# nv-tlabs/LION

Measured on AMD Instinct MI355X. Metric: shapes/sec @1000-step DDIM, Bx2048pts, higher is better.
Workload: dtype f32 (operands of the 3x3x3 voxel convolutions and of the long 1x1 convolutions cut into fp16 hi/lo pairs on the 16-bi...

## Files before the change

### include/lion_hip.h

```cpp
#ifndef LION_HIP_H_
#define LION_HIP_H_

#include <stddef.h>
#include <stdint.h>

#ifdef __cplusplus
extern "C" {
#endif

typedef void *lionStream_t;

#define LION_OK 0
#define LION_EINVAL (-1)
#define LION_EUNSUPPORTED (-2)
#define LION_EWORKSPACE (-3)

int lion_abi_version(void);

size_t lion_avg_voxelize_workspace_bytes(int B, int C, int N, int r);
int lion_avg_voxelize_forward(const float *feat, const int32_t *coords, int B, int C, int N,
                              int r, float *out, int32_t *ind, int32_t *cnt, void *ws,
                              size_t ws_bytes, lionStream_t stream);

int lion_voxelize_points_forward(const float *feat, const float *coords, int B, int C, int N,
                                 int r, int normalize, float eps, float *out,
                                 float *norm_coords, int32_t *ind, int32_t *cnt, void *ws,
                                 size_t ws_bytes, lionStream_t stream);

size_t lion_voxel_plan_bytes(int B, int N, int r);
int lion_voxel_index(const float *coords, int B, int N, int r, int normalize, float eps,
                     float *norm_coords, int32_t *ind, int32_t *cnt, void *plan, size_t plan_bytes,
                     lionStream_t stream);
int lion_voxel_scatter(const float *feat, const void *plan, size_t plan_bytes, int B, int C, int N,
                       int r, float *out, lionStream_t stream);
int lion_voxel_scatter_read(const float *feat, const void *plan, size_t plan_bytes, int B, int C, int N, int r,
                            const int32_t *occ_m1, float *out, lionStream_t stream);

int lion_avg_voxelize_backward(const float *gy, const int32_t *ind, const int32_t *cnt, int B,
                               int C, int N, int r3, float *gx, lionStream_t stream);

int lion_trilinear_devoxelize_forward(const float *coords, const float *feat, int B, int C,
                                      int N, int r, int training, float *out, int32_t *inds,
                                      float *wgts, lionStream_t stream);

int lion_trilinear_devoxelize_backward(const float *gy, const int32_t *inds, const float *wgts,
                                       int B, int C, int N, int r3, float *gx,
                                       lionStream_t stream);

int lion_ball_query(const float *centers, const float *points, int B, int M, int N,
                    float radius, int U, int32_t *idx, lionStream_t stream);

int lion_grouping_forward(const float *feat, const int32_t *idx, int B, int C, int N, int M,
                          int U, float *out, lionStream_t stream);
int lion_group_points_forward(const float *coords, const float *centers, const float *feat, const int32_t *idx,
                              int B, int C, int N, int M, int U, float *out, lionStream_t stream);
int lion_grouping_backward(const float *gy, const int32_t *idx, int B, int C, int N, int M,
                           int U, float *gx, lionStream_t stream);

int lion_furthest_point_sampling(const float *coords, int B, int N, int M, int32_t *idx,
                                 lionStream_t stream);

int lion_gather_features_forward(const float *feat, const int32_t *idx, int B, int C, int N,
                                 int M, float *out, lionStream_t stream);
int lion_gather_features_backward(const float *gy, const int32_t *idx, int B, int C, int N,
                                  int M, float *gx, lionStream_t stream);

int lion_three_nn_interpolate_forward(const float *points, const float *centers,
                                      const float *cfeat, int B, int C, int N, int M,
                                      float *out, int32_t *idx, float *wgt,
                                      lionStream_t stream);
int lion_three_nn_interpolate_cat_forward(const float *points, const float *centers, const float *cfeat, const float *temb,
                                          int ld_t, const float *skip, int B, int C1, int C2, int C3, int N, int M,
                                          float *out, int32_t *idx, float *wgt, lionStream_t stream);
int lion_three_nn_interpolate_backward(const float *gy, const int32_t *idx, const float *wgt,
                                       int B, int C, int N, int M, float *gx,
                                       lionStream_t stream);

int lion_chamfer_forward(const float *xyz1, const float *xyz2, int B, int N, int M,
                         float *dist1, float *dist2, int32_t *idx1, int32_t *idx2,
                         lionStream_t stream);
int lion_chamfer_backward(const float *xyz1, const float *xyz2, const float *gdist1,
                          const float *gdist2, const int32_t *idx1, const int32_t *idx2, int B,
                          int N, int M, float *gxyz1, float *gxyz2, lionStream_t stream);

size_t lion_emd_workspace_bytes(int B, int N, int M);
int lion_emd_approxmatch(const float *xyz1, const float *xyz2, int B, int N, int M,
                         float *match, void *ws, size_t ws_bytes, lionStream_t stream);
int lion_emd_cost(const float *xyz1, const float *xyz2, int B, int N, int M, float *cost, void *ws,
                  size_t ws_bytes, lionStream_t stream);
int lion_emd_matchcost(const float *xyz1, const float *xyz2, const float *match, int B, int N,
                       int M, float *cost, void *ws, size_t ws_bytes, lionStream_t stream);
int lion_emd_matchcost_backward(const float *grad_cost, const float *xyz1, const float *xyz2,
                                const float *match, int B, int N, int M, float *grad1,
                                float *grad2, lionStream_t stream);

int lion_ddim_update(const float *x, const float *eps, const float *z, size_t numel, float s,
                     float c, float sigma, float *out, lionStream_t stream);
int lion_ddpm_update(const float *x, const float *eps, const float *z, size_t numel,
                     int t_is_zero, float k_outer, float k_a, float k_b, float scale,
                     float temp, float *out, lionStream_t stream);
int lion_chain_begin_step(const float *table, int n_steps, int32_t *counter, float *t_out, int B, float *cur,
                          lionStream_t stream);
int lion_chain_update_noise(int mode, const float *x, const float *eps, size_t numel, const float *cur,
                            const uint32_t *seed , uint32_t stream_id, float *out,
                            float *z_out, lionStream_t stream);
int lion_chain_begin_step_temb(const float *table, int n_steps, int32_t *counter, float *t_out, int B, float *cur,
                               const float *temb_table, int temb_width, float *temb_out, lionStream_t stream);
int lion_chain_update_noise_cm(int mode, const float *x, const float *eps_cm, int B, int N, const float *cur,
                               const uint32_t *seed, uint32_t stream_id, float *out, float *z_out, lionStream_t stream);
int lion_latent_unpack(const float *x, int B, int N, int D, float *all, float *coords, float *rest, lionStream_t stream);
int lion_concat_broadcast(const float *a, const float *t, int B, int Ca, int Ct, int N, int ld_t, float *out,
                          lionStream_t stream);

size_t lion_conv3d_packed_floats(int Cout, int Cin);
int lion_conv3d_pack_weights(const float *w, int Cout, int Cin, float *wp, lionStream_t stream);
int lion_conv3d_k3_forward(const float *x, const float *wp, const float *bias, int B, int Cin,
                           int Cout, int r, float *y, lionStream_t stream);
size_t lion_conv3d_wgrad_workspace_floats(int B, int Cin, int Cout, int r);
int lion_conv3d_k3_wgrad(const float *x, const float *gy, int B, int Cin, int Cout, int r, float *gw, float *ws,
                         size_t ws_floats, lionStream_t stream);
int lion_conv3d_k3_wgrad_split(const float *x, const float *gy, int B, int Cin, int Cout, int r, float *gw, float *ws,
                               size_t ws_floats, lionStream_t stream);
size_t lion_conv3d_wgrad_sparse_workspace_floats(int B, int Cin, int Cout, int r);
int lion_conv3d_k3_wgrad_split_sparse(const float *x, const float *gy, const int32_t *cnt, int B, int Cin, int Cout, int r,
                                      float *gw, float *ws, size_t ws_floats, lionStream_t stream);

int lion_conv3d_stat_tiles(int r, int Cout, int B, int sparse);
int lion_conv3d_k3_fused_forward(const float *x, const float *wp, const float *bias, int B, int Cin,
                                 int Cout, int r, const float *pro_a, const float *pro_b, const float *pro_bias,
                                 const float *tconst, float *y, float *stats, int32_t *occ, lionStream_t stream);
size_t lion_conv3d_occupancy_ints(int r, int Cout, int B);
int lion_conv3d_const_response(const float *wsum, const float *bias2, const float *bias1, const float *pro_a,
                               const float *pro_b, int B, int Cin, int Cout, float *tconst, lionStream_t stream);
int lion_conv3d_tile_occupancy(const int32_t *cnt, int B, int r, int Cout, int32_t *occ_m1, int32_t *occ_m2,
                               lionStream_t stream);
int lion_conv3d_tile_occupancy_aware(const int32_t *cnt, int B, int r, int Cout, int32_t *occ_m1, int32_t *occ_m2,
                                     int consumer_aware, lionStream_t stream);
int lion_groupnorm_fold(const float *stats, int B, int C, int T, int G, int voxels, const float *gamma,
                        const float *beta, const float *fac, const float *gbias, int ld_fg, float eps,
                        float *A, float *Bs, float *chmean, lionStream_t stream);
size_t lion_conv3d_split_packed_halfs(int Cout, int Cin);
int lion_conv3d_split_pack_weights(const float *w, int Cout, int Cin, uint16_t *wp, lionStream_t stream);
int lion_conv3d_split_stat_tiles(int r, int Cout);
int lion_conv3d_k3_split_forward(const float *x, const uint16_t *wp, const float *bias, int B, int Cin, int Cout,
                                 int r, const float *pro_a, const float *pro_b, const float *pro_bias,
                                 const float *tconst, float *y, float *stats, int32_t *occ, lionStream_t stream);
size_t lion_skinny_packed_floats(int Cout, int Cin);
int lion_skinny_pack_weights(const float *w, int Cout, int Cin, float *wp, lionStream_t stream);
int lion_skinny_splits(int Cin, int Cout);
int lion_skinny_gemm(const float *pin, int ks_in, const float *bias_in, int act_in, const float *addT,
                     const float *wp, int nb, int Cin, int Cout, float *pout, lionStream_t stream);
int lion_skinny_finish(const float *A, int ks_a, const float *bias_a, const float *Bp, int ks_b, const float *resid,
                       int nb, int C, int mode, float *y, lionStream_t stream);
int lion_skinny_gemm_se_finish(const float *pin, int ks_in, const float *bias_in, int act_in, const float *wp, int nb, int Cin,
                               int Cout, const float *A, int ks_a, const float *bias_a, const float *resid, float *y,
                               lionStream_t stream);
int lion_to_channel_major(const float *a, int lda, int Ca, float *oa, const float *b, int ldb, int Cb, float *ob, int B,
                          lionStream_t stream);
int lion_from_channel_major(const float *x, int B, int C, float *y, lionStream_t stream);
int lion_groupnorm_fold_se(const float *stats, int B, int C, int T, int G, int voxels, const float *gamma,
                           const float *beta, const float *fac, const float *gbias, int ld_fg, float eps, const float *w1,
                           const float *w2, int H, float *A, float *Bs, lionStream_t stream);
int lion_se_gate(const float *chmean, const float *w1, const float *w2, int B, int C, int H, float *A,
                 float *Bs, lionStream_t stream);
int lion_trilinear_devoxelize_affine_forward(const float *coords, const float *feat, const float *scale,
                                             const float *shift, int B, int C, int N, int r, float *out,
                                             lionStream_t stream);
size_t lion_devoxelize_plan_bytes(int B, int N, int r);
int lion_trilinear_devoxelize_plan(const float *coords, int B, int N, int r, void *plan, size_t plan_bytes,
                                   lionStream_t stream);
int lion_trilinear_devoxelize_planned_forward(const void *plan, size_t plan_bytes, const float *coords, const float *feat,
                                              const float *scale, const float *shift, int B, int C, int N, int r,
                                              float *out, lionStream_t stream);

int lion_row_stats(const float *x, int rows, int L, float *stats, lionStream_t stream);
size_t lion_pwconv_packed_floats(int Cout, int Cin);
int lion_pwconv_pack_weights(const float *w, int Cout, int Cin, float *wp, lionStream_t stream);
int lion_pwconv_stat_tiles(int Cout, int Cin, int L);
int lion_pwconv_forward(const float *x, const float *wp, const float *bias, int B, int Cin, int Cout, int L,
                        const float *pro_a, const float *pro_b, float *y, float *stats, lionStream_t stream);
int lion_pwconv_forward_max(const float *x, const float *wp, const float *bias, int B, int Cin, int Cout, int L,
                            const float *pro_a, const float *pro_b, const float *out_a, const float *out_b,
                            float *stats, float *ymax, lionStream_t stream);
size_t lion_pwconv_split_packed_halfs(int Cout, int Cin);
int lion_pwconv_split_pack_weights(const float *w, int Cout, int Cin, uint16_t *wp, lionStream_t stream);
int lion_pwconv_split_pack_weights_t(const float *w, int Cout, int Cin, const uint16_t *wp, uint16_t *wpt, lionStream_t stream);
int lion_pwconv_split_stat_tiles(int Cout, int Cin, int L);
int lion_pwconv_split_forward(const float *x, const uint16_t *wp, const float *bias, int B, int Cin, int Cout, int L,
                              const float *pro_a, const float *pro_b, float *y, float *stats, lionStream_t stream);
int lion_linear_attention_core(const float *qkv, int B, int H, int D, int N, float *out, lionStream_t stream);
int lion_linear_attention_core_backward(const float *qkv, const float *gout, int B, int H, int D, int N, float *gqkv,
                                        lionStream_t stream);
int lion_linear_forward(const float *x, const float *wp, const float *bias, int B, int K, int O, int act, float slope,
                        float *y, lionStream_t stream);
int lion_affine_swish(const float *x, const float *A, const float *Bs, int rows, int L, float *y,
                      lionStream_t stream);
int lion_affine_swish_max(const float *x, const float *A, const float *Bs, int rows, int M, int U,
                          float *y, lionStream_t stream);
int lion_timestep_embedding(const float *t, const float *row, float scale, int B, int half, int D, float *emb,
                            lionStream_t stream);
int lion_affine_swish_add(const float *x, const float *A, const float *Bs, const float *addend, int rows, int L, float *y,
                          lionStream_t stream);

size_t lion_scatter_csr_workspace_bytes(int B, int E, int bins);
int lion_scatter_csr(const float *gy, const int32_t *idx, const float *w, int B, int C, int S, int E, int bins, void *ws,
                     size_t ws_bytes, float *gx, lionStream_t stream);

size_t lion_pwconv_wgrad_workspace_bytes(int B, int Cin, int Cout, int L);
int lion_pwconv_wgrad(const float *x, const float *gy, int B, int Cin, int Cout, int L, void *ws, size_t ws_bytes,
                      float *gw, float *gb, lionStream_t stream);

int lion_gn_train_fold(const float *stats, const float *gw, const float *gb, const float *fac, int fac_stride,
                       const float *bias, int bias_stride, int B, int C, int G, int L, float eps, float *A, float *Bs,
                       float *mean, float *rstd, lionStream_t stream);
int lion_row_stats64(const float *x, int rows, int L, double *stats, lionStream_t stream);
int lion_gn_train_fold64(const double *stats, const float *gw, const float *gb, const float *fac, int fac_stride,
                         const float *bias, int bias_stride, int B, int C, int G, int L, float eps, float *A,
                         float *Bs, float *mean, float *rstd, lionStream_t stream);
int lion_gn_train_bwd_fold(const float *S, const float *mean, const float *rstd, const float *gw, const float *gb,
                           const float *fac, int fac_stride, int B, int C, int G, int L, float *Q, float *R, float *dfac,
                           float *dbias, int d_stride, float *pw, const float *A, const double *xstats, const float *gate,
                           const float *qse, float *Aout, lionStream_t stream);
int lion_gn_train_param_grads(const float *pw, int B, int C, float *dgw, float *dgb, float *dxs, lionStream_t stream);
int lion_se_gate_fwd(const float *stats, const float *w1, const float *w2, int B, int C, int Cr, int L, float *mean, float *h,
                     float *g, float *zero, lionStream_t stream);
int lion_se_gate_bwd(const float *S, const float *g, const float *h, const float *mean, const float *w1, const float *w2, int B,
                     int C, int Cr, int L, float *dpre2, float *dpre1, float *Q, float *dw1, float *dw2, lionStream_t stream);
int lion_rows_dot2(const float *g, const float *v, const float *ws, int B, int C, int N, float *S, lionStream_t stream);
int lion_trilinear_devoxelize_backward_affine(const float *gy, const int32_t *inds, const float *wgts, const float *x,
                                              const float *Ap, const float *Q, const float *R, int B, int C, int N, int r3,
                                              float *dx, lionStream_t stream);
int lion_gn_se_gate_fwd(const double *xstats, const float *A, const float *Bs, const float *w1, const float *w2, int B, int C, int Cr,
                        int L, float *mean, float *h, float *g, float *A2, float *B2, lionStream_t stream);
int lion_gn_se_gate_bwd(const float *S, const double *xstats, const float *A, const float *Bs, const float *g, const float *h,
                        const float *mean, const float *w1, const float *w2, int B, int C, int Cr, int L, float *Sp, float *dpre2,
                        float *dpre1, float *Qse, float *dw1, float *dw2, lionStream_t stream);
int lion_affine_act(const float *x, const float *A, const float *Bs, int rows, int L, int act, float *y,
                    lionStream_t stream);
int lion_affine_act_bwd_stats(const float *x, const float *gy, const float *A, const float *Bs, int rows, int L, int act,
                              float *S, lionStream_t stream);
int lion_affine_act_bwd_apply(const float *x, const float *gy, const float *A, const float *Bs, const float *Q,
                              const float *R, int rows, int L, int act, float *dx, lionStream_t stream);
int lion_affine_act_dropout(const float *x, const float *A, const float *Bs, int rows, int L, int act, const uint64_t *seed,
                            float keep, float *y, lionStream_t stream);
int lion_affine_act_dropout_bwd_stats(const float *x, const float *gy, const float *A, const float *Bs, int rows, int L, int act,
                                      const uint64_t *seed, float keep, float *S, lionStream_t stream);
int lion_affine_act_dropout_bwd_apply(const float *x, const float *gy, const float *A, const float *Bs, const float *Q,
                                      const float *R, int rows, int L, int act, const uint64_t *seed, float keep, float *dx,
                                      lionStream_t stream);
int lion_affine_act_max(const float *x, const float *A, const float *Bs, int rows, int M, int U, int act, float *y,
                        lionStream_t stream);
int lion_affine_act_max_bwd_stats(const float *x, const float *gy, const float *A, const float *Bs, int rows, int M, int U,
                                  int act, float *S, lionStream_t stream);
int lion_affine_act_max_bwd_apply(const float *x, const float *gy, const float *A, const float *Bs, const float *Q,
                                  const float *R, int rows, int M, int U, int act, float *dx, lionStream_t stream);

int lion_adam_chunk(void);
int lion_adam_row(void);
int lion_adam_step(const uint64_t *table, const int32_t *numel, const int32_t *blockmap, int blocks, int tensors, const float *lr,
                   float beta1, float beta2, float eps, float weight_decay, float ema_decay, lionStream_t stream);

#define LION_ODE_RUNNING 0
#define LION_ODE_FINISHED 1
#define LION_ODE_TOO_SMALL_STEP (-1)
typedef struct lion_ode_ctrl {
  double t, h_abs, t_bound, direction, rtol, atol;
  double h, t_new, err_norm, h0, d1, sign;
  int32_t stage, cur, status, step_rejected;
  int32_t yslot, fslot, nfe, n_accepted;
  int32_t n_rejected, accepted, pad0, pad1;
} lion_ode_ctrl;
size_t lion_ode_partials_bytes(size_t n);
int lion_ode_stage(double *Y, const double *K, size_t n, lion_ode_ctrl *ctrl, float *x32, float *t_model, int B,
                   lionStream_t stream);
int lion_ode_drift(const float *eps, int cm_points, const float *x32, size_t n, const float *t_model, float beta_start,
                   float beta_delta, float neg_beta_start, float half_beta_delta, float one_minus_sigma2_0,
                   const float *mix_a, const float *mix_b, int mix_len, double *K, lion_ode_ctrl *ctrl,
                   lionStream_t stream);
int lion_ode_error_partials(const double *Y, const double *K, size_t n, const lion_ode_ctrl *ctrl, double *partials,
                            lionStream_t stream);
int lion_ode_control(const double *partials, size_t n, lion_ode_ctrl *ctrl, lionStream_t stream);

#ifdef __cplusplus
}
#endif
#endif
```

### lion_amd/_lib.py

```python
from __future__ import annotations

import ctypes as C
import os

_HERE = os.path.dirname(os.path.abspath(__file__))
SO_PATH = os.environ.get("LION_HIP_SO") or os.path.join(_HERE, "csrc", "liblion_hip.so")

_vp, _i, _f, _sz = C.c_void_p, C.c_int, C.c_float, C.c_size_t

SIGNATURES = {
    "lion_abi_version": (_i, []),
    "lion_avg_voxelize_workspace_bytes": (_sz, [_i, _i, _i, _i]),
    "lion_avg_voxelize_forward": (_i, [_vp, _vp, _i, _i, _i, _i, _vp, _vp, _vp, _vp, _sz, _vp]),
    "lion_voxelize_points_forward": (_i, [_vp, _vp, _i, _i, _i, _i, _i, _f, _vp, _vp, _vp, _vp,
                                          _vp, _sz, _vp]),
    "lion_voxel_plan_bytes": (_sz, [_i, _i, _i]),
    "lion_voxel_index": (_i, [_vp, _i, _i, _i, _i, _f, _vp, _vp, _vp, _vp, _sz, _vp]),
    "lion_voxel_scatter": (_i, [_vp, _vp, _sz, _i, _i, _i, _i, _vp, _vp]),
    "lion_voxel_scatter_read": (_i, [_vp, _vp, _sz, _i, _i, _i, _i, _vp, _vp, _vp]),
    "lion_avg_voxelize_backward": (_i, [_vp, _vp, _vp, _i, _i, _i, _i, _vp, _vp]),
    "lion_trilinear_devoxelize_forward": (_i, [_vp, _vp, _i, _i, _i, _i, _i, _vp, _vp, _vp, _vp]),
    "lion_trilinear_devoxelize_backward": (_i, [_vp, _vp, _vp, _i, _i, _i, _i, _vp, _vp]),
    "lion_ball_query": (_i, [_vp, _vp, _i, _i, _i, _f, _i, _vp, _vp]),
    "lion_grouping_forward": (_i, [_vp, _vp, _i, _i, _i, _i, _i, _vp, _vp]),
    "lion_group_points_forward": (_i, [_vp, _vp, _vp, _vp, _i, _i, _i, _i, _i, _vp, _vp]),
    "lion_grouping_backward": (_i, [_vp, _vp, _i, _i, _i, _i, _i, _vp, _vp]),
    "lion_furthest_point_sampling": (_i, [_vp, _i, _i, _i, _vp, _vp]),
    "lion_gather_features_forward": (_i, [_vp, _vp, _i, _i, _i, _i, _vp, _vp]),
    "lion_gather_features_backward": (_i, [_vp, _vp, _i, _i, _i, _i, _vp, _vp]),
    "lion_three_nn_interpolate_forward": (_i, [_vp, _vp, _vp, _i, _i, _i, _i, _vp, _vp, _vp, _vp]),
    "lion_three_nn_interpolate_backward": (_i, [_vp, _vp, _vp, _i, _i, _i, _i, _vp, _vp]),
    "lion_chamfer_forward": (_i, [_vp, _vp, _i, _i, _i, _vp, _vp, _vp, _vp, _vp]),
    "lion_chamfer_backward": (_i, [_vp, _vp, _vp, _vp, _vp, _vp, _i, _i, _i, _vp, _vp, _vp]),
    "lion_emd_workspace_bytes": (_sz, [_i, _i, _i]),
    "lion_emd_approxmatch": (_i, [_vp, _vp, _i, _i, _i, _vp, _vp, _sz, _vp]),
    "lion_emd_cost": (_i, [_vp, _vp, _i, _i, _i, _vp, _vp, _sz, _vp]),
    "lion_emd_matchcost": (_i, [_vp, _vp, _vp, _i, _i, _i, _vp, _vp, _sz, _vp]),
    "lion_emd_matchcost_backward": (_i, [_vp, _vp, _vp, _vp, _i, _i, _i, _vp, _vp, _vp]),
    "lion_conv3d_packed_floats": (_sz, [_i, _i]),
    "lion_conv3d_pack_weights": (_i, [_vp, _i, _i, _vp, _vp]),
    "lion_conv3d_k3_forward": (_i, [_vp, _vp, _vp, _i, _i, _i, _i, _vp, _vp]),
    "lion_conv3d_wgrad_workspace_floats": (_sz, [_i, _i, _i, _i]),
    "lion_conv3d_k3_wgrad": (_i, [_vp, _vp, _i, _i, _i, _i, _vp, _vp, _sz, _vp]),
    "lion_conv3d_k3_wgrad_split": (_i, [_vp, _vp, _i, _i, _i, _i, _vp, _vp, _sz, _vp]),
    "lion_conv3d_wgrad_sparse_workspace_floats": (_sz, [_i, _i, _i, _i]),
    "lion_conv3d_k3_wgrad_split_sparse": (_i, [_vp, _vp, _vp, _i, _i, _i, _i, _vp, _vp, _sz, _vp]),
    "lion_conv3d_stat_tiles": (_i, [_i, _i, _i, _i]),
    "lion_conv3d_k3_fused_forward": (_i, [_vp, _vp, _vp, _i, _i, _i, _i, _vp, _vp, _vp, _vp, _vp, _vp, _vp, _vp]),
    "lion_conv3d_const_response": (_i, [_vp, _vp, _vp, _vp, _vp, _i, _i, _i, _vp, _vp]),
    "lion_conv3d_occupancy_ints": (_sz, [_i, _i, _i]),
    "lion_conv3d_tile_occupancy": (_i, [_vp, _i, _i, _i, _vp, _vp, _vp]),
    "lion_conv3d_tile_occupancy_aware": (_i, [_vp, _i, _i, _i, _vp, _vp, _i, _vp]),
    "lion_conv3d_split_packed_halfs": (_sz, [_i, _i]),
    "lion_conv3d_split_pack_weights": (_i, [_vp, _i, _i, _vp, _vp]),
    "lion_conv3d_split_stat_tiles": (_i, [_i, _i]),
    "lion_conv3d_k3_split_forward": (_i, [_vp, _vp, _vp, _i, _i, _i, _i, _vp, _vp, _vp, _vp, _vp, _vp, _vp, _vp]),
    "lion_groupnorm_fold": (_i, [_vp, _i, _i, _i, _i, _i, _vp, _vp, _vp, _vp, _i, _f, _vp, _vp, _vp, _vp]),
    "lion_groupnorm_fold_se": (_i, [_vp, _i, _i, _i, _i, _i, _vp, _vp, _vp, _vp, _i, _f, _vp, _vp, _i, _vp, _vp, _vp]),
    "lion_skinny_packed_floats": (_sz, [_i, _i]),
    "lion_skinny_pack_weights": (_i, [_vp, _i, _i, _vp, _vp]),
    "lion_skinny_splits": (_i, [_i, _i]),
    "lion_skinny_gemm": (_i, [_vp, _i, _vp, _i, _vp, _vp, _i, _i, _i, _vp, _vp]),
    "lion_skinny_gemm_se_finish": (_i, [_vp, _i, _vp, _i, _vp, _i, _i, _i, _vp, _i, _vp, _vp, _vp, _vp]),
    "lion_skinny_finish": (_i, [_vp, _i, _vp, _vp, _i, _vp, _i, _i, _i, _vp, _vp]),
    "lion_to_channel_major": (_i, [_vp, _i, _i, _vp, _vp, _i, _i, _vp, _i, _vp]),
    "lion_from_channel_major": (_i, [_vp, _i, _i, _vp, _vp]),
    "lion_se_gate": (_i, [_vp, _vp, _vp, _i, _i, _i, _vp, _vp, _vp]),
    "lion_trilinear_devoxelize_affine_forward": (_i, [_vp, _vp, _vp, _vp, _i, _i, _i, _i, _vp, _vp]),
    "lion_devoxelize_plan_bytes": (_sz, [_i, _i, _i]),
    "lion_trilinear_devoxelize_plan": (_i, [_vp, _i, _i, _i, _vp, _sz, _vp]),
    "lion_trilinear_devoxelize_planned_forward": (_i, [_vp, _sz, _vp, _vp, _vp, _vp, _i, _i, _i, _i, _vp, _vp]),
    "lion_row_stats": (_i, [_vp, _i, _i, _vp, _vp]),
    "lion_pwconv_packed_floats": (_sz, [_i, _i]),
    "lion_pwconv_pack_weights": (_i, [_vp, _i, _i, _vp, _vp]),
    "lion_pwconv_stat_tiles": (_i, [_i, _i, _i]),
    "lion_pwconv_forward": (_i, [_vp, _vp, _vp, _i, _i, _i, _i, _vp, _vp, _vp, _vp, _vp]),
    "lion_pwconv_forward_max": (_i, [_vp, _vp, _vp, _i, _i, _i, _i, _vp, _vp, _vp, _vp, _vp, _vp, _vp]),
    "lion_pwconv_split_packed_halfs": (_sz, [_i, _i]),
    "lion_pwconv_split_pack_weights": (_i, [_vp, _i, _i, _vp, _vp]),
    "lion_pwconv_split_pack_weights_t": (_i, [_vp, _i, _i, _vp, _vp, _vp]),
    "lion_pwconv_split_stat_tiles": (_i, [_i, _i, _i]),
    "lion_pwconv_split_forward": (_i, [_vp, _vp, _vp, _i, _i, _i, _i, _vp, _vp, _vp, _vp, _vp]),
    "lion_linear_attention_core": (_i, [_vp, _i, _i, _i, _i, _vp, _vp]),
    "lion_linear_attention_core_backward": (_i, [_vp, _vp, _i, _i, _i, _i, _vp, _vp]),
    "lion_linear_forward": (_i, [_vp, _vp, _vp, _i, _i, _i, _i, _f, _vp, _vp]),
    "lion_affine_swish": (_i, [_vp, _vp, _vp, _i, _i, _vp, _vp]),
    "lion_affine_swish_max": (_i, [_vp, _vp, _vp, _i, _i, _i, _vp, _vp]),
    "lion_timestep_embedding": (_i, [_vp, _vp, _f, _i, _i, _i, _vp, _vp]),
    "lion_affine_swish_add": (_i, [_vp, _vp, _vp, _vp, _i, _i, _vp, _vp]),
    "lion_scatter_csr_workspace_bytes": (_sz, [_i, _i, _i]),
    "lion_scatter_csr": (_i, [_vp, _vp, _vp, _i, _i, _i, _i, _i, _vp, _sz, _vp, _vp]),
    "lion_pwconv_wgrad_workspace_bytes": (_sz, [_i, _i, _i, _i]),
    "lion_pwconv_wgrad": (_i, [_vp, _vp, _i, _i, _i, _i, _vp, _sz, _vp, _vp, _vp]),
    "lion_gn_train_fold": (_i, [_vp, _vp, _vp, _vp, _i, _vp, _i, _i, _i, _i, _i, _f, _vp, _vp, _vp, _vp, _vp]),
    "lion_row_stats64": (_i, [_vp, _i, _i, _vp, _vp]),
    "lion_gn_train_fold64": (_i, [_vp, _vp, _vp, _vp, _i, _vp, _i, _i, _i, _i, _i, _f, _vp, _vp, _vp, _vp, _vp]),
    "lion_gn_train_bwd_fold": (_i, [_vp, _vp, _vp, _vp, _vp, _vp, _i, _i, _i, _i, _i, _vp, _vp, _vp, _vp, _i, _vp, _vp, _vp, _vp, _vp,
                                    _vp, _vp]),
    "lion_gn_train_param_grads": (_i, [_vp, _i, _i, _vp, _vp, _vp, _vp]),
    "lion_adam_chunk": (_i, []),
    "lion_adam_row": (_i, []),
    "lion_adam_step": (_i, [_vp, _vp, _vp, _i, _i, _vp, _f, _f, _f, _f, _f, _vp]),
    "lion_se_gate_fwd": (_i, [_vp, _vp, _vp, _i, _i, _i, _i, _vp, _vp, _vp, _vp, _vp]),
    "lion_se_gate_bwd": (_i, [_vp, _vp, _vp, _vp, _vp, _vp, _i, _i, _i, _i, _vp, _vp, _vp, _vp, _vp, _vp]),
    "lion_rows_dot2": (_i, [_vp, _vp, _vp, _i, _i, _i, _vp, _vp]),
    "lion_trilinear_devoxelize_backward_affine": (_i, [_vp, _vp, _vp, _vp, _vp, _vp, _vp, _i, _i, _i, _i, _vp, _vp]),
    "lion_gn_se_gate_fwd": (_i, [_vp, _vp, _vp, _vp, _vp, _i, _i, _i, _i, _vp, _vp, _vp, _vp, _vp, _vp]),
    "lion_gn_se_gate_bwd": (_i, [_vp, _vp, _vp, _vp, _vp, _vp, _vp, _vp, _vp, _i, _i, _i, _i, _vp, _vp, _vp, _vp, _vp, _vp, _vp]),
    "lion_affine_act": (_i, [_vp, _vp, _vp, _i, _i, _i, _vp, _vp]),
    "lion_affine_act_bwd_stats": (_i, [_vp, _vp, _vp, _vp, _i, _i, _i, _vp, _vp]),
    "lion_affine_act_bwd_apply": (_i, [_vp, _vp, _vp, _vp, _vp, _vp, _i, _i, _i, _vp, _vp]),
    "lion_affine_act_dropout": (_i, [_vp, _vp, _vp, _i, _i, _i, _vp, _f, _vp, _vp]),
    "lion_affine_act_dropout_bwd_stats": (_i, [_vp, _vp, _vp, _vp, _i, _i, _i, _vp, _f, _vp, _vp]),
    "lion_affine_act_dropout_bwd_apply": (_i, [_vp, _vp, _vp, _vp, _vp, _vp, _i, _i, _i, _vp, _f, _vp, _vp]),
    "lion_affine_act_max": (_i, [_vp, _vp, _vp, _i, _i, _i, _i, _vp, _vp]),
    "lion_affine_act_max_bwd_stats": (_i, [_vp, _vp, _vp, _vp, _i, _i, _i, _i, _vp, _vp]),
    "lion_affine_act_max_bwd_apply": (_i, [_vp, _vp, _vp, _vp, _vp, _vp, _i, _i, _i, _i, _vp, _vp]),
    "lion_ddim_update": (_i, [_vp, _vp, _vp, _sz, _f, _f, _f, _vp, _vp]),
    "lion_ddpm_update": (_i, [_vp, _vp, _vp, _sz, _i, _f, _f, _f, _f, _f, _vp, _vp]),
    "lion_chain_begin_step": (_i, [_vp, _i, _vp, _vp, _i, _vp, _vp]),
    "lion_chain_update_noise": (_i, [_i, _vp, _vp, _sz, _vp, _vp, C.c_uint32, _vp, _vp, _vp]),
    "lion_chain_begin_step_temb": (_i, [_vp, _i, _vp, _vp, _i, _vp, _vp, _i, _vp, _vp]),
    "lion_chain_update_noise_cm": (_i, [_i, _vp, _vp, _i, _i, _vp, _vp, C.c_uint32, _vp, _vp, _vp]),
    "lion_latent_unpack": (_i, [_vp, _i, _i, _i, _vp, _vp, _vp, _vp]),
    "lion_concat_broadcast": (_i, [_vp, _vp, _i, _i, _i, _i, _i, _vp, _vp]),
    "lion_three_nn_interpolate_cat_forward": (_i, [_vp, _vp, _vp, _vp, _i, _vp, _i, _i, _i, _i, _i, _i, _vp, _vp, _vp, _vp]),
    "lion_ode_partials_bytes": (_sz, [_sz]),
    "lion_ode_stage": (_i, [_vp, _vp, _sz, _vp, _vp, _vp, _i, _vp]),
    "lion_ode_drift": (_i, [_vp, _i, _vp, _sz, _vp, _f, _f, _f, _f, _f, _vp, _vp, _i, _vp, _vp, _vp]),
    "lion_ode_error_partials": (_i, [_vp, _vp, _sz, _vp, _vp, _vp]),
    "lion_ode_control": (_i, [_vp, _sz, _vp, _vp]),
}



_ERR = {-1: "LION_EINVAL (bad shape / null pointer)",
        -2: "LION_EUNSUPPORTED (shape outside what the kernels implement)",
        -3: "LION_EWORKSPACE (workspace too small)"}

_lib = None


def load() -> C.CDLL:
    global _lib
    if _lib is not None:
        return _lib
    if not os.path.exists(SO_PATH):
        raise RuntimeError(
            f"lion_amd: HIP extension not built: {SO_PATH} is missing. Run "
            f"`python -c 'import __graft_entry__ as g; g.build()'` or lion_amd/csrc/build.sh. "
            f"There is no CPU fallback.")
    lib = C.CDLL(SO_PATH)
    for name, (res, args) in SIGNATURES.items():
        try:
            fn = getattr(lib, name)
        except AttributeError as e:
            raise RuntimeError(f"lion_amd: {SO_PATH} does not export {name}") from e
        fn.restype = res
        fn.argtypes = args
    _lib = lib
    return lib


def check(code: int, what: str) -> None:
    if code != 0:
        msg = _ERR.get(code, f"hipError {code}" if code > 0 else f"error {code}")
        raise RuntimeError(f"lion_amd: {what} failed: {msg}")


def call(name: str, *args, unsupported_ok: bool = False) -> bool:
    import torch
    if len(args) + 1 != len(SIGNATURES[name][1]):
        raise TypeError(f"lion_amd: {name} takes {len(SIGNATURES[name][1]) - 1} arguments before the stream, got {len(args)}")
    dev, argv = None, list(args)
    for i, a in enumerate(args):
        if isinstance(a, torch.Tensor):
            d = a.get_device()
            if d != dev:
                if d < 0:
                    raise RuntimeError("lion_amd: expected a CUDA(HIP) tensor; there is no CPU path")
                if dev is not None:
                    raise RuntimeError(f"lion_amd: {name}: operands on different devices (cuda:{dev} and cuda:{d})")
                dev = d
            argv[i] = a.data_ptr()
    rc = getattr(load(), name)(*argv, torch._C._cuda_getCurrentRawStream(torch.cuda.current_device() if dev is None else dev))
    if rc == -2 and unsupported_ok:
        return False
    check(rc, name)
    return True


def ptr(t):
    return None if t is None else C.c_void_p(t.data_ptr())


def stream_ptr(device=None):
    import torch
    return C.c_void_p(torch.cuda.current_stream(device).cuda_stream)


def require_cuda(*tensors):
    for t in tensors:
        if t is None:
            continue
        if not t.is_cuda:
            raise RuntimeError("lion_amd: expected a CUDA(HIP) tensor; there is no CPU path")
        if not t.is_contiguous():
            raise RuntimeError("lion_amd: expected a contiguous tensor")
```

### lion_amd/chain.py

```python
from __future__ import annotations

import numpy as np
import torch

from . import _lib, _wcache

DDIM, DDPM = 0, 1
RECORD = None
TEMB_TABLE = __import__("os").environ.get("LION_TEMB_TABLE", "1") != "0"
CHANNEL_MAJOR_EPS = __import__("os").environ.get("LION_CHAIN_CM_EPS", "1") != "0"

def policy_key() -> tuple:
    from . import conv_ops, fused_ops, geometry
    from .models import pvcnn2_ada
    return (pvcnn2_ada.SPARSE_CONV1, pvcnn2_ada.FUSE_INFERENCE, pvcnn2_ada.OVERLAP_POINT_BRANCH, geometry.ENABLED,
            geometry.SPLIT_GRAPH, conv_ops.SPLIT, fused_ops.PW_SPLIT, pvcnn2_ada.VOX_PLAN, TEMB_TABLE, fused_ops.MAX_RECOMPUTE,
            pvcnn2_ada.SKIP_UNREAD, pvcnn2_ada.SKIP_UNREAD_LEVEL2, CHANNEL_MAJOR_EPS)


class GraphedChain:
    def __init__(self, model, num_samples, shape, condition_input, clip_feat, device, mode, capacity, warmup=2,
                 record_noise=False, step_fn=None):
        self.model, self.mode, self.capacity = model, mode, int(capacity)
        self.fingerprint = _wcache.fingerprint(model)
        dev = torch.device(device)
        size = [num_samples] + list(shape)
        self.x = torch.zeros(size, device=dev)
        self.t = torch.zeros(num_samples, device=dev)
        self.cond = None if condition_input is None else condition_input.detach().clone().contiguous()
        self.clip = None if clip_feat is None else clip_feat.detach().clone().contiguous()
        self.table = torch.zeros(self.capacity, 8, device=dev)
        self.counter = torch.zeros(1, dtype=torch.int32, device=dev)
        self.seed = torch.zeros(2, dtype=torch.int32, device=dev)
        self.cur = torch.zeros(8, device=dev)
        self.z = torch.zeros(size, device=dev) if record_noise else None
        self.table[:, 0] = 1.0
        self.table[:, 1] = 1.0
        self.table[:, 3] = 1.0
        self.temb_table = None
        self.use_temb_table = step_fn is None and TEMB_TABLE and hasattr(model, "time_embedding") and not getattr(model, "embed_dim", 1) == 0
        self.policy = policy_key()
        self.pinned = []

        n_pts, n_cls = getattr(model, "num_points", 0), getattr(model, "num_classes", 0)
        self.cm_out = (CHANNEL_MAJOR_EPS and hasattr(model, "geometry_source") and n_cls == 4
                       and int(np.prod(shape)) == n_pts * n_cls and not getattr(model, "mixed_prediction", False))

        def step():
            if step_fn is not None:
                step_fn(self)
                return
            extra = {}
            if self.temb_table is not None:
                _lib.call("lion_chain_begin_step_temb", self.table, self.capacity, self.counter, self.t, num_samples, self.cur,
                          self.temb_table, self.temb_row.numel(), self.temb_row)
                extra["temb"] = self.temb_row
            else:
                _lib.call("lion_chain_begin_step", self.table, self.capacity, self.counter, self.t, num_samples, self.cur)
            if self.cm_out:
                pred = model(x=self.x, t=self.t, condition_input=self.cond, clip_feat=self.clip, channel_major_out=True,
                             **extra)
                eps = pred.float().contiguous()
                assert tuple(eps.shape) == (num_samples, n_cls, n_pts)
                _lib.call("lion_chain_update_noise_cm", mode, self.x, eps, num_samples, n_pts, self.cur, self.seed, 0, self.x,
                          self.z)
                return
            pred = model(x=self.x, t=self.t, condition_input=self.cond, clip_feat=self.clip, **extra)
            eps = pred.float().contiguous()
            _lib.call("lion_chain_update_noise", mode, self.x, eps, self.x.numel(), self.cur, self.seed, 0, self.x, self.z)

        from . import geometry
        src = getattr(model, "geometry_source", None)
        self.geo_graphs = self.graph_b = None
        self.geo_plan = None
        split = geometry.SPLIT_GRAPH and src is not None and not geometry.ENABLED
        if self.use_temb_table:
            with torch.no_grad():
                row = model.time_embedding(torch.ones(1, device=dev))
            self.temb_table = torch.zeros((self.capacity,) + tuple(row.shape[1:]), device=dev)
            self.temb_row = torch.zeros((1,) + tuple(row.shape[1:]), device=dev)
        main = torch.cuda.current_stream(dev)
        side = torch.cuda.Stream(device=dev)
        side.wait_stream(main)
        with _wcache.pinning(self.pinned):
            with torch.no_grad(), torch.cuda.stream(side):
                for _ in range(warmup):
                    step()
            main.wait_stream(side)
            if split:
                self.geo_stream = torch.cuda.Stream(device=dev)
                self.ev_step = torch.cuda.Event()

                def geo(boundary=None):
                    mods, coords = src(self.x)
                    return geometry.compute_chain(mods, coords, boundary=boundary)
                self.geo_stream.wait_stream(main)
                with torch.no_grad(), torch.cuda.stream(self.geo_stream):
                    geo()
                main.wait_stream(self.geo_stream)
                torch.cuda.synchronize(dev)
                self.geo_graphs = [torch.cuda.CUDAGraph()]
                gs = torch.cuda.Stream(device=dev)
                gs.wait_stream(main)

                def geo_cut(i):
                    if i == 1:
                        self.geo_graphs[-1].capture_end()
                        self.geo_graphs.append(torch.cuda.CUDAGraph())
                        self.geo_graphs[-1].capture_begin(pool=self.geo_graphs[0].pool())
                with torch.no_grad(), torch.cuda.stream(gs):
                    self.geo_graphs[0].capture_begin()
                    try:
                        self.geo_plan = geo(geo_cut)
                    finally:
                        self.geo_graphs[-1].capture_end()
                main.wait_stream(gs)
                torch.cuda.synchronize(dev)
                self.geo_stage_of_graph = [0, self.geo_plan["stages"] - 1][:len(self.geo_graphs)]
                self.ev_geo = [torch.cuda.Event() for _ in self.geo_graphs]
                graphs, waits = [torch.cuda.CUDAGraph()], []

                def on_use(first, last):
                    need = [g for g, st_ in enumerate(self.geo_stage_of_graph)
                            if st_ >= first and (g == 0 or self.geo_stage_of_graph[g - 1] < last)]
                    need = [g for g in need if not any(g in w for w in waits)]
                    if not need:
                        return
                    graphs[-1].capture_end()
                    waits.append(need)
                    graphs.append(torch.cuda.CUDAGraph())
                    graphs[-1].capture_begin(pool=graphs[0].pool())
                cap = torch.cuda.Stream(device=dev)
                cap.wait_stream(main)
                with torch.no_grad(), torch.cuda.stream(cap), geometry.external(self.geo_plan, on_use):
                    graphs[0].capture_begin()
                    try:
                        step()
                    finally:
                        graphs[-1].capture_end()
                main.wait_stream(cap)
                self.graph = graphs[0]
                if waits:
                    self.graphs, self.waits = graphs, waits
                    self.graph_b = graphs[1]
                else:
                    self.geo_graphs = self.geo_plan = None
            else:
                self.graph = torch.cuda.CUDAGraph()
                with torch.no_grad(), torch.cuda.graph(self.graph):
                    step()
        self.pinned = list({id(v): v for v in self.pinned}.values())

    def replay(self):
        if self.graph_b is None:
            self.graph.replay()
            return
        main = torch.cuda.current_stream(self.x.device)
        self.ev_step.record(main)
        self.geo_stream.wait_event(self.ev_step)
        with torch.cuda.stream(self.geo_stream):
            for g, ev in zip(self.geo_graphs, self.ev_geo):
                g.replay()
                ev.record(self.geo_stream)
        self.graphs[0].replay()
        for k, need in enumerate(self.waits):
            for g in need:
                main.wait_event(self.ev_geo[g])
            self.graphs[k + 1].replay()

    def matches(self, condition_input, clip_feat):
# ... 84 lines not shown
```

### lion_amd/csrc/common.h

```cpp
#pragma once
#include <hip/hip_runtime.h>
#include <stdint.h>
#include <stddef.h>

#include "lion_hip.h"

#define LION_WAVE 64

#define LION_LAUNCH_CHECK()                         \
  do {                                              \
    hipError_t e__ = hipGetLastError();             \
    if (e__ != hipSuccess) return (int)e__;         \
  } while (0)

static inline int lion_cdiv(int a, int b) { return (a + b - 1) / b; }

__attribute__((visibility("hidden"))) int lion_internal_sparse_tile_dims(int r, int *td, int *th);

#define LION_MAX_DEVICES 32
struct LionLdsLimit {
  size_t bytes[LION_MAX_DEVICES];
};
static inline int lion_current_device(int *dev) {
  if (hipGetDevice(dev) != hipSuccess || *dev < 0 || *dev >= LION_MAX_DEVICES) return LION_EINVAL;
  return 0;
}
template <typename K>
static inline int lion_dynamic_lds(K kernel, size_t bytes, LionLdsLimit &limit) {
  int dev = 0;
  if (int e = lion_current_device(&dev)) return e;
  if (bytes > limit.bytes[dev]) {
    hipError_t e = hipFuncSetAttribute(reinterpret_cast<const void *>(kernel),
                                       hipFuncAttributeMaxDynamicSharedMemorySize, (int)bytes);
    if (e != hipSuccess) return (int)e;
    limit.bytes[dev] = bytes;
  }
  return 0;
}

__device__ __forceinline__ float mul_rn(float a, float b) { return __fmul_rn(a, b); }
__device__ __forceinline__ float add_rn(float a, float b) { return __fadd_rn(a, b); }
__device__ __forceinline__ float sub_rn(float a, float b) { return __fsub_rn(a, b); }
__device__ __forceinline__ float div_rn(float a, float b) { return __fdiv_rn(a, b); }
__device__ __forceinline__ float sqrt_rn(float a) { return sqrtf(a); }
__device__ __forceinline__ void philox4x32_10(uint32_t c0, uint32_t c1, uint32_t c2, uint32_t c3, uint32_t k0,
                                              uint32_t k1, uint32_t out[4]) {
#pragma unroll
  for (int r = 0; r < 10; ++r) {
    const uint64_t p0 = (uint64_t)0xD2511F53u * c0, p1 = (uint64_t)0xCD9E8D57u * c2;
    const uint32_t n0 = (uint32_t)(p1 >> 32) ^ c1 ^ k0, n2 = (uint32_t)(p0 >> 32) ^ c3 ^ k1;
    c1 = (uint32_t)p1; c3 = (uint32_t)p0; c0 = n0; c2 = n2;
    k0 += 0x9E3779B9u; k1 += 0xBB67AE85u;
  }
  out[0] = c0; out[1] = c1; out[2] = c2; out[3] = c3;
}

__device__ __forceinline__ float swish_fast(float t) { return t * __builtin_amdgcn_rcpf(1.0f + __expf(-t)); }

__device__ __forceinline__ float sqdist3(float ax, float ay, float az, float bx, float by,
                                         float bz) {
  const float dx = sub_rn(ax, bx), dy = sub_rn(ay, by), dz = sub_rn(az, bz);
  return add_rn(add_rn(mul_rn(dx, dx), mul_rn(dy, dy)), mul_rn(dz, dz));
}

#define LION_DPP_F32(v, ctrl) __builtin_bit_cast(float, __builtin_amdgcn_update_dpp(0, __builtin_bit_cast(int, (v)), (ctrl), 0xf, 0xf, true))
__device__ __forceinline__ float row16_sum_rn(float v) {
  v = __fadd_rn(v, LION_DPP_F32(v, 0xB1));
  v = __fadd_rn(v, LION_DPP_F32(v, 0x4E));
  v = __fadd_rn(v, LION_DPP_F32(v, 0x141));
  v = __fadd_rn(v, LION_DPP_F32(v, 0x140));
  return v;
}
__device__ __forceinline__ unsigned wave_max_u32_lane63(unsigned v) {
#define LION_DPP_U32(x, ctrl, rmask) ((unsigned)__builtin_amdgcn_update_dpp(0, (int)(x), (ctrl), (rmask), 0xf, true))
  unsigned o;
  o = LION_DPP_U32(v, 0xB1, 0xf); v = o > v ? o : v;
  o = LION_DPP_U32(v, 0x4E, 0xf); v = o > v ? o : v;
  o = LION_DPP_U32(v, 0x141, 0xf); v = o > v ? o : v;
  o = LION_DPP_U32(v, 0x140, 0xf); v = o > v ? o : v;
  o = LION_DPP_U32(v, 0x142, 0xa); v = o > v ? o : v;
  o = LION_DPP_U32(v, 0x143, 0xc); v = o > v ? o : v;
#undef LION_DPP_U32
  return v;
}
__device__ __forceinline__ float row_pair_sum_odd_rows(float v) {
  return __fadd_rn(v, __builtin_bit_cast(float, __builtin_amdgcn_update_dpp(0, __builtin_bit_cast(int, v), 0x142, 0xa, 0xf, true)));
}
#define LION_DPP_F32_ROWS(x, ctrl, rmask) \
  __builtin_bit_cast(float, __builtin_amdgcn_update_dpp(0, __builtin_bit_cast(int, (x)), (ctrl), (rmask), 0xf, true))
__device__ __forceinline__ float row16_max(float v) {
  float o;
  o = LION_DPP_F32(v, 0xB1); v = o > v ? o : v;
  o = LION_DPP_F32(v, 0x4E); v = o > v ? o : v;
  o = LION_DPP_F32(v, 0x141); v = o > v ? o : v;
  o = LION_DPP_F32(v, 0x140); v = o > v ? o : v;
  return v;
}

__device__ __forceinline__ int wave_incl_scan(int v, int lane) {
#pragma unroll
  for (int d = 1; d < LION_WAVE; d <<= 1) {
    const int t = __shfl_up(v, d, LION_WAVE);
    if (lane >= d) v += t;
  }
  return v;
}
```

### lion_amd/csrc/conv3d.hip

```cpp
#include "common.h"

namespace {

typedef float f32x16 __attribute__((ext_vector_type(16)));
#ifndef LION_CONV_KC
#define LION_CONV_KC 4
#endif
#ifndef LION_CONV_WAVES
#define LION_CONV_WAVES 2
#endif
constexpr int KC = LION_CONV_KC;

__device__ __forceinline__ float pro_act(float v, float pa, float pb) {
  const float t = v * pa + pb;
  return swish_fast(t);
}

template <int TD, int TH, int TW, int COT, int VB, bool PRO, bool STATS>
__global__ __launch_bounds__(256, LION_CONV_WAVES) void conv3d_k3_kernel(const float *__restrict__ x,
                                                                const float *__restrict__ wp,
                                                                const float *__restrict__ bias,
                                                                float *__restrict__ y, int Cin,
                                                                int Cout, int r,
                                                                const float *__restrict__ pro_a,
// ... 72 lines not shown
  for (int vb = 0; vb < VB; ++vb) {
    const int v = (wave * VB + vb) * 32 + (lane & 31);
    const int d = v / (TH * TW), h = (v / TW) % TH, w = v % TW;
    boff[vb] = (lane >> 5) * HALO + (d * HH + h) * HW + w;
  }
  const int aoff = (lane >> 5) * 27 * COT + (lane & 31);

  f32x16 acc[CB][VB];
#pragma unroll
  for (int cb = 0; cb < CB; ++cb)
#pragma unroll
    for (int vb = 0; vb < VB; ++vb)
#pragma unroll
      for (int i = 0; i < 16; ++i) acc[cb][vb][i] = 0.f;

  const __amdgpu_buffer_rsrc_t xrs = __builtin_amdgcn_make_buffer_rsrc(
      const_cast<float *>(x + (size_t)b * Cin * r3), 0, Cin * r3 * 4, 0x00020000);
  float rx[KC][NJ];
  typedef __attribute__((address_space(3))) float lds_float;
  const uint32_t sw_lds = (uint32_t)(uintptr_t)(lds_float *)sw;
  auto load_chunk = [&](int q) {
#pragma unroll
    for (int i = 0; i < NWV; ++i) {
      const int e0 = wave * 64 + i * TM;
      if (e0 < WV4) {
        const int e = min(e0 + lane, WV4 - 1);
        const int row = e / (COT / 4), j4 = e - row * (COT / 4);
        const float *g = wp + ((size_t)q * KC * 27 + row) * Cout + co0 + j4 * 4;
        const uint32_t dst = __builtin_amdgcn_readfirstlane(sw_lds + (uint32_t)(((q & 1) * SWS + e0 * 4) * 4));
        unsigned keep;
        asm volatile("s_mov_b32 %0, m0\n\ts_mov_b32 m0, %2\n\ts_nop 0\n\tglobal_load_lds_dwordx4 %1, off\n\ts_mov_b32 m0, %0"
                     : "=&s"(keep) : "v"(g), "s"(dst) : "memory");
      }
    }
#pragma unroll
    for (int c = 0; c < KC; ++c)
#pragma unroll
      for (int j = 0; j < NJ; ++j)
        rx[c][j] = __builtin_bit_cast(float, __builtin_amdgcn_raw_buffer_load_b32(xrs, goff[j], (q * KC + c) * r3 * 4, 0));
  };
  const int wmask = queued ? (occ[b * ntiles + tile] & 0xf) : 0xf;
  const bool empty = wmask == 0;
  const bool wave_on = (wmask >> wave) & 1;
  const int nchunks = empty ? 0 : Cin / KC;
  if (!empty) load_chunk(0);
  for (int q = 0; q < nchunks; ++q) {
    __syncthreads();
#pragma unroll
    for (int c = 0; c < KC; ++c) {
      float pa = 1.f, pb = 0.f, pc = 0.f;
      if (PRO) { pa = spa[q * KC + c]; pb = spb[q * KC + c]; pc = spc[q * KC + c]; }
#pragma unroll
      for (int j = 0; j < NJ; ++j) {
        const int p = tid + j * TM;
        float v = rx[c][j];
        if (PRO) v = pro_act(v, pa, pb) - pc;
        if (p < HALO) sx[c * HALO + p] = (!PRO || gok[j]) ? v : 0.f;
      }
    }
    asm volatile("s_waitcnt vmcnt(0)" ::: "memory");
    __syncthreads();
    if (q + 1 < nchunks) load_chunk(q + 1);

    constexpr int NS = (KC / 2) * 27;
    const float *swq = sw + (q & 1) * SWS;
    float av[2][CB], bv[2][VB];
    auto lds_step = [&](int st, int buf) {
      const int cp = st / 27, tap = st % 27;
      const int kd = tap / 9, kh = (tap / 3) % 3, kw = tap % 3;
      const int toff = (kd * HH + kh) * HW + kw + cp * 2 * HALO;
#pragma unroll
      for (int vb = 0; vb < VB; ++vb) bv[buf][vb] = sx[boff[vb] + toff];
      const float *ap = swq + aoff + (cp * 2 * 27 + tap) * COT;
#pragma unroll
      for (int cb = 0; cb < CB; ++cb) av[buf][cb] = ap[cb * 32];
    };
    if (wave_on) {
    lds_step(0, 0);
#pragma unroll
    for (int st = 0; st < NS; ++st) {
      if (st + 1 < NS) lds_step(st + 1, (st + 1) & 1);
      __builtin_amdgcn_sched_barrier(0);
#pragma unroll
      for (int cb = 0; cb < CB; ++cb)
#pragma unroll
        for (int vb = 0; vb < VB; ++vb)
          acc[cb][vb] = __builtin_amdgcn_mfma_f32_32x32x2f32(av[st & 1][cb], bv[st & 1][vb], acc[cb][vb], 0, 0, 0);
      __builtin_amdgcn_sched_barrier(0);
    }
    }
  }

  if (delta) {
    __syncthreads();
    for (int e = tid; e < 27 * COT; e += TM) sT[e] = tconst[((size_t)b * 27 + e / COT) * Cout + co0 + e % COT];
    __syncthreads();
  } else if (empty) {
    __syncthreads();
  }
  float *yb = y + ((size_t)b * Cout + co0) * r3;
#pragma unroll
  for (int vb = 0; vb < VB; ++vb) {
    const int v = (wave * VB + vb) * 32 + (lane & 31);
    const int d = v / (TH * TW), h = (v / TW) % TH, w = v % TW;
    const int gv = ((d0 + d) * r + (h0 + h)) * r + (w0 + w);
    const int gd = d0 + d, gh = h0 + h, gw = w0 + w;
    const int cfg = (((gd == 0 ? 0 : gd == r - 1 ? 2 : 1) * 3 + (gh == 0 ? 0 : gh == r - 1 ? 2 : 1)) * 3 +
                     (gw == 0 ? 0 : gw == r - 1 ? 2 : 1));
    const float *addv = delta ? sT + cfg * COT : sbias;
#pragma unroll
    for (int cb = 0; cb < CB; ++cb)
#pragma unroll
      for (int i = 0; i < 16; ++i) {
        const int co = cb * 32 + (i & 3) + 8 * (i >> 2) + 4 * (lane >> 5);
        const float o = acc[cb][vb][i] + addv[co];
        acc[cb][vb][i] = o;
        yb[(size_t)co * r3 + gv] = o;
      }
  }
  if (STATS) {
    constexpr int NWAVE = 4;
#pragma unroll
    for (int cb = 0; cb < CB; ++cb)
#pragma unroll
      for (int i = 0; i < 16; ++i) {
        float s1 = acc[cb][0][i], s2 = acc[cb][0][i] * acc[cb][0][i];
#pragma unroll
        for (int vb = 1; vb < VB; ++vb) { s1 += acc[cb][vb][i]; s2 += acc[cb][vb][i] * acc[cb][vb][i]; }
        s1 = row16_sum_rn(s1); s2 = row16_sum_rn(s2);
        s1 = row_pair_sum_odd_rows(s1); s2 = row_pair_sum_odd_rows(s2);
        if ((lane & 31) == 16) {
          const int co = cb * 32 + (i & 3) + 8 * (i >> 2) + 4 * (lane >> 5);
          sred[(wave * COT + co) * 2] = s1;
          sred[(wave * COT + co) * 2 + 1] = s2;
        }
      }
    __syncthreads();
    if (tid < COT) {
      float s1 = 0.f, s2 = 0.f;
#pragma unroll
      for (int w = 0; w < NWAVE; ++w) { s1 += sred[(w * COT + tid) * 2]; s2 += sred[(w * COT + tid) * 2 + 1]; }
      float *o = stats + (((size_t)b * Cout + co0 + tid) * ntiles + tile) * 2;
      o[0] = s1;
      o[1] = s2;
    }
  }
  }
  if (queued && tid == 0) {
    int32_t *q = occ + 2 * B * ntiles;
    if (atomicAdd(q + 1, 1) == (int)gridDim.x - 1) { q[0] = 0; q[1] = 0; }
  }
}

__global__ void gn_fold_kernel(const float *__restrict__ stats, int C, int T, int G, float count,
                               const float *__restrict__ gamma, const float *__restrict__ beta,
                               const float *__restrict__ fac, const float *__restrict__ gbias, int ld_fg, float eps,
                               float *__restrict__ A, float *__restrict__ Bs, float *__restrict__ chmean) {
  __shared__ double cs[64][2];
  __shared__ double gs[2];
  const int b = blockIdx.y, g = blockIdx.x, cpg = C / G, tid = threadIdx.x;
  int cp2 = 1;
  while (cp2 < cpg) cp2 <<= 1;
  const int LPC = 256 / cp2, ch = tid / LPC, sub = tid % LPC;
  double s1 = 0.0, s2 = 0.0;
  if (ch < cpg) {
    const float2 *p = reinterpret_cast<const float2 *>(stats + (((size_t)b * C + g * cpg + ch) * T) * 2);
    for (int t = sub; t < T; t += LPC) { const float2 v = p[t]; s1 += (double)v.x; s2 += (double)v.y; }
  }
  for (int m = 1; m < LPC && m < 64; m <<= 1) { s1 += __shfl_xor(s1, m, 64); s2 += __shfl_xor(s2, m, 64); }
  if (LPC > 64) {
    __shared__ double ws[4][2];
    if ((tid & 63) == 0) { ws[tid >> 6][0] = s1; ws[tid >> 6][1] = s2; }
    __syncthreads();
    if (sub == 0) {
      s1 = 0.0; s2 = 0.0;
      for (int w = 0; w < LPC / 64; ++w) { s1 += ws[(tid >> 6) + w][0]; s2 += ws[(tid >> 6) + w][1]; }
    }
  }
  if (ch < cpg && sub == 0) {
    cs[ch][0] = s1;
    cs[ch][1] = s2;
    chmean[(size_t)b * C + g * cpg + ch] = (float)(s1 / count);
  }
  __syncthreads();
  if (tid == 0) {
    double g1 = 0.0, g2 = 0.0;
    for (int c = 0; c < cpg; ++c) { g1 += cs[c][0]; g2 += cs[c][1]; }
    gs[0] = g1;
    gs[1] = g2;
  }
  __syncthreads();
  if (tid < cpg) {
    const double n = (double)count * cpg;
    const double mean = gs[0] / n;
    double var = gs[1] / n - mean * mean;
    var = var > 0.0 ? var : 0.0;
    const float rstd = (float)(1.0 / sqrt(var + (double)eps));
    const int c = g * cpg + tid;
    const float f = fac[(size_t)b * ld_fg + c], gb = gbias[(size_t)b * ld_fg + c];
    const float a0 = rstd * gamma[c];
    A[(size_t)b * C + c] = a0 * f;
    Bs[(size_t)b * C + c] = (beta[c] - (float)mean * a0) * f + gb;
  }
}

__global__ __launch_bounds__(256) void gn_fold_se_kernel(const float *__restrict__ stats, int C, int T, int G, float count,
                                                         const float *__restrict__ gamma, const float *__restrict__ beta,
                                                         const float *__restrict__ fac, const float *__restrict__ gbias,
                                                         int ld_fg, float eps, const float *__restrict__ w1,
                                                         const float *__restrict__ w2, int H, float *__restrict__ A,
                                                         float *__restrict__ Bs) {
  __shared__ double cs[256][2];
  __shared__ float sA[256], sB[256], sm[256], sh[128];
  const int b = blockIdx.x, tid = threadIdx.x, lane = tid & 63, wave = tid >> 6, cpg = C / G;
  int cp2 = 1;
  while (cp2 < C) cp2 <<= 1;
  const int LPC = 256 / cp2, ch = tid / LPC, sub = tid % LPC;
  double s1 = 0.0, s2 = 0.0;
  if (ch < C) {
    const float2 *p = reinterpret_cast<const float2 *>(stats + (((size_t)b * C + ch) * T) * 2);
    for (int t = sub; t < T; t += LPC) { const float2 v = p[t]; s1 += (double)v.x; s2 += (double)v.y; }
  }
  for (int m = 1; m < LPC; m <<= 1) { s1 += __shfl_xor(s1, m, 64); s2 += __shfl_xor(s2, m, 64); }
  if (ch < C && sub == 0) { cs[ch][0] = s1; cs[ch][1] = s2; }
  __syncthreads();
  if (tid < C) {
    const int g0 = (tid / cpg) * cpg;
    double g1 = 0.0, g2 = 0.0;
    for (int k = 0; k < cpg; ++k) { g1 += cs[g0 + k][0]; g2 += cs[g0 + k][1]; }
    const double n = (double)count * cpg, mean = g1 / n;
    double var = g2 / n - mean * mean;
    var = var > 0.0 ? var : 0.0;
    const float rstd = (float)(1.0 / sqrt(var + (double)eps));
    const float f = fac[(size_t)b * ld_fg + tid], gb = gbias[(size_t)b * ld_fg + tid];
    const float a0 = rstd * gamma[tid];
    const float a = a0 * f, bb = (beta[tid] - (float)mean * a0) * f + gb;
    sA[tid] = a;
    sB[tid] = bb;
    sm[tid] = a * (float)(cs[tid][0] / count) + bb;
  }
  __syncthreads();
  for (int j = wave; j < H; j += 4) {
    float acc = 0.f;
    for (int c = lane; c < C; c += 64) acc += w1[(size_t)j * C + c] * sm[c];
#pragma unroll
    for (int m = 32; m >= 1; m >>= 1) acc += __shfl_xor(acc, m, 64);
    if (lane == 0) sh[j] = acc > 0.f ? acc : 0.f;
  }
  __syncthreads();
  if (tid < C) {
    float acc = 0.f;
    for (int j = 0; j < H; ++j) acc += w2[(size_t)tid * H + j] * sh[j];
    const float g = 1.0f / (1.0f + expf(-acc));
    A[(size_t)b * C + tid] = sA[tid] * g;
    Bs[(size_t)b * C + tid] = sB[tid] * g;
  }
}

__global__ __launch_bounds__(1024) void conv_tile_occ_kernel(const int32_t *__restrict__ cnt, int r, int TD, int TH,
                                                             int32_t *__restrict__ occ1, int32_t *__restrict__ occ2,
                                                             int aware) {
  __shared__ unsigned col[32 * 32];
  __shared__ int flag[2][256];
  const int b = blockIdx.x, B = gridDim.x, tid = threadIdx.x;
  const int nth = r / TH, ntiles = (r / TD) * nth, total = B * ntiles;
  for (int i = tid; i < r * r; i += 1024) col[i] = 0u;
  __syncthreads();
  const int4 *c4 = reinterpret_cast<const int4 *>(cnt + (size_t)b * r * r * r);
  for (int i = tid; i < (r * r * r) >> 2; i += 1024) {
    const int4 v = c4[i];
    if (v.x | v.y | v.z | v.w) {
      const unsigned m4 = (v.x ? 1u : 0u) | (v.y ? 2u : 0u) | (v.z ? 4u : 0u) | (v.w ? 8u : 0u);
      atomicOr(&col[(i << 2) / r], m4 << ((i << 2) % r));
    }
  }
  __syncthreads();
  const int RW = 64 / r;
  for (int e = tid; e < 2 * ntiles; e += 1024) {
    const int t = e % ntiles, margin = 1 + e / ntiles;
    const int dt = (t / nth) * TD, ht = (t % nth) * TH;
    int mask = 0;
    for (int w = 0; w < 4; ++w) {
      const int dl = dt + (w * RW) / TH, hl = ht + (w * RW) % TH;
      unsigned any = 0u;
      for (int d = max(dl - margin, 0); d <= min(dl + margin, r - 1); ++d)
        for (int h = max(hl - margin, 0); h <= min(hl + RW - 1 + margin, r - 1); ++h) any |= col[d * r + h];
      mask |= (any ? 1 : 0) << w;
    }
    flag[margin - 1][t] = mask;
  }
  __syncthreads();
  __shared__ unsigned long long bal[2][4];
  const int m = tid >> 8, t = tid & 255, lane = tid & 63, w = (tid >> 6) & 3;
  const bool live = tid < 512 && t < ntiles;
  const int f = live ? flag[m][t] : 0;
  const unsigned long long bl = __ballot(f != 0);
  if (tid < 512 && lane == 0) bal[m][w] = bl;
  __syncthreads();
  if (live) {
    int32_t *occ = m == 0 ? occ1 : occ2;
    if (occ) {
      int before = __popcll(bal[m][w] & ((1ull << lane) - 1ull)), occupied = 0;
      for (int ww = 0; ww < 4; ++ww) {
        const int c = __popcll(bal[m][ww]);
        if (ww < w) before += c;
        occupied += c;
      }
      int32_t *fl = occ + (size_t)b * ntiles, *list = occ + total + (size_t)b * ntiles;
      int need = flag[1][t] != 0;
      if (m == 0) {
        if (aware == 2) {
          need = 0;
        } else {
          const int td = t / nth, th = t % nth;
          for (int dd = max(td - 1, 0); dd <= min(td + 1, r / TD - 1); ++dd)
            for (int hh = max(th - 1, 0); hh <= min(th + 1, nth - 1); ++hh) need |= flag[1][dd * nth + hh] != 0;
        }
      }
      fl[t] = f | (need << 8) | ((m == 1 && flag[0][t] != 0) ? (1 << 9) : 0);
      list[f ? before : occupied + (t - before)] = t;
      if (b == 0 && t == 0) { occ[2 * total] = 0; occ[2 * total + 1] = 0; occ[2 * total + 2] = aware; }
    }
  }
}

__global__ __launch_bounds__(256) void conv_tconst_kernel(const float *__restrict__ wsum, const float *__restrict__ bias2,
                                                          const float *__restrict__ bias1, const float *__restrict__ pro_a,
                                                          const float *__restrict__ pro_b, int Cin, int Cout,
                                                          float *__restrict__ tconst) {
  __shared__ float sc[256];
  const int cfg = blockIdx.x, b = blockIdx.y, tid = threadIdx.x;
  for (int c = tid; c < Cin; c += 256)
    sc[c] = pro_act(bias1 ? bias1[c] : 0.f, pro_a[(size_t)b * Cin + c], pro_b[(size_t)b * Cin + c]);
  __syncthreads();
  for (int co = tid; co < Cout; co += 256) {
    double acc = bias2 ? (double)bias2[co] : 0.0;
    const float *w = wsum + (size_t)cfg * Cin * Cout + co;
    for (int c = 0; c < Cin; ++c) acc += (double)w[(size_t)c * Cout] * (double)sc[c];
    tconst[((size_t)b * 27 + cfg) * Cout + co] = (float)acc;
  }
}

__global__ void conv3d_pack_kernel(const float *__restrict__ w, int Cout, int Cin, int Cin_pad,
                                   float *__restrict__ wp) {
  const int i = blockIdx.x * blockDim.x + threadIdx.x;
  const int total = Cin_pad * 27 * Cout;
  if (i >= total) return;
  const int co = i % Cout, t = (i / Cout) % 27, ci = i / (Cout * 27);
  wp[i] = ci < Cin ? w[((size_t)co * Cin + ci) * 27 + t] : 0.f;
}

template <int TD, int TH, int TW, int COT, int VB>
static int launch_conv_t(const float *x, const float *wp, const float *bias, float *y, int B, int Cin,
                         int Cout, int r, const float *pa, const float *pb, const float *pbias, const float *tconst,
                         float *stats, int32_t *occ, hipStream_t st) {
  const int tiles = (r / TD) * (r / TH) * (r / TW);
  static int cu_count[LION_MAX_DEVICES] = {0};
  int dev = 0;
  if (int e = lion_current_device(&dev)) return e;
  if (!cu_count[dev]) {
    hipDeviceProp_t prop;
    if (hipGetDeviceProperties(&prop, dev) != hipSuccess) return LION_EINVAL;
    cu_count[dev] = prop.multiProcessorCount;
  }
  const int n_cu = cu_count[dev];
  const long items = (long)B * tiles * (Cout / COT);
  const dim3 grid = occ ? dim3((unsigned)(items < 2L * n_cu ? items : 2L * n_cu)) : dim3(B, tiles, Cout / COT);
  constexpr int NT = 256;
  constexpr int HALO = (TD + 2) * (TH + 2) * (TW + 2);
  constexpr int SWS = ((KC * 27 * COT + 255) / 256) * 256 + 256;
  static_assert(KC * HALO >= 27 * COT, "the response table must fit the input tile buffer");
  const size_t LDS = (size_t)(((KC * HALO + 3) & ~3) + 2 * SWS + COT + (pa ? 3 * ((Cin + 63) & ~63) : 0) +
                              (NT / 64) * COT * 2) * 4;
#define LION_CONV_GO(PRO_, ST_)                                                                           \
  {                                                                                                       \
    static LionLdsLimit cfg = {};                                                                         \
    if (int e = lion_dynamic_lds(&conv3d_k3_kernel<TD, TH, TW, COT, VB, PRO_, ST_>, LDS, cfg)) return e;  \
    conv3d_k3_kernel<TD, TH, TW, COT, VB, PRO_, ST_><<<grid, NT, LDS, st>>>(x, wp, bias, y, Cin, Cout, r, \
                                                                            pa, pb, pbias, tconst, stats, occ, B, \
                                                                            tiles);                      \
  }
  if (pa && stats) LION_CONV_GO(true, true)
  else if (pa) LION_CONV_GO(true, false)
  else if (stats) LION_CONV_GO(false, true)
  else LION_CONV_GO(false, false)
#undef LION_CONV_GO
  LION_LAUNCH_CHECK();
  return 0;
}

struct ConvPlan { int vb, cot, tiles; };
static ConvPlan conv_plan(int r, int Cout, int B, bool sparse) {
  const int r3 = r * r * r;
  if (!sparse && Cout % 64 == 0 && r >= 16 && (long)(r3 / 512) * (Cout / 64) * B >= 512) return {4, 64, r3 / 512};
  if (Cout % 64 == 0 && (long)(r3 / 256) * (Cout / 64) * B >= 512) return {2, 64, r3 / 256};
  if (Cout % 32 == 0 && r >= 16 && !sparse) return {4, 32, r3 / 512};
  if (Cout % 32 == 0 && r >= 16) return {2, 32, r3 / 256};
  if (Cout % 32 == 0) return {1, 32, r3 / 128};
  return {0, 0, 0};
}

static void conv_tile_dims(int r, int vb, int *td, int *th, int *tw) {
  *tw = r;
  if (r == 32) { *td = vb == 2 ? 2 : 4; *th = 4; }
  else if (r == 16) { *td = vb == 2 ? 4 : 8; *th = 4; }
  else { *td = vb == 2 ? 4 : 2; *th = 8; }
}

static int launch_conv(const float *x, const float *wp, const float *bias, float *y, int B, int Cin, int Cout,
                       int r, const float *pa, const float *pb, const float *pbias, const float *tconst, float *stats,
                       int32_t *occ, hipStream_t st) {
  const ConvPlan p = conv_plan(r, Cout, B, occ != nullptr);
#define LION_CONV_TILE(R_, VB_, COT_, TD_, TH_, TW_)                                                       \
  if (r == R_ && p.vb == VB_ && p.cot == COT_)                                                             \
    return launch_conv_t<TD_, TH_, TW_, COT_, VB_>(x, wp, bias, y, B, Cin, Cout, r, pa, pb, pbias, tconst, stats, occ, st);
  LION_CONV_TILE(32, 2, 64, 2, 4, 32)
  LION_CONV_TILE(32, 4, 64, 4, 4, 32)
  LION_CONV_TILE(16, 4, 64, 8, 4, 16)
  LION_CONV_TILE(32, 4, 32, 4, 4, 32)
  LION_CONV_TILE(32, 2, 32, 2, 4, 32)
  LION_CONV_TILE(16, 2, 32, 4, 4, 16)
  LION_CONV_TILE(16, 2, 64, 4, 4, 16)
  LION_CONV_TILE(16, 4, 32, 8, 4, 16)
  LION_CONV_TILE(8, 2, 64, 4, 8, 8)
  LION_CONV_TILE(8, 1, 32, 2, 8, 8)
#undef LION_CONV_TILE
  return LION_EUNSUPPORTED;
}

}

int lion_internal_sparse_tile_dims(int r, int *td, int *th) {
  if (r != 16 && r != 32) return LION_EUNSUPPORTED;
  const ConvPlan a = conv_plan(r, 64, 32, true), b = conv_plan(r, 32, 32, true), c = conv_plan(r, 64, 1, true);
  if (!a.vb || a.vb != b.vb || a.vb != c.vb) return LION_EUNSUPPORTED;
  int tw;
  conv_tile_dims(r, a.vb, td, th, &tw);
  return 0;
}

extern "C" {

size_t lion_conv3d_packed_floats(int Cout, int Cin) {
  return (size_t)((Cin + KC - 1) / KC * KC) * 27 * Cout;
}

int lion_conv3d_pack_weights(const float *w, int Cout, int Cin, float *wp, lionStream_t stream) {
  if (!w || !wp || Cout <= 0 || Cin <= 0) return LION_EINVAL;
  const int Cin_pad = (Cin + KC - 1) / KC * KC;
  const int total = Cin_pad * 27 * Cout;
  conv3d_pack_kernel<<<lion_cdiv(total, 256), 256, 0, static_cast<hipStream_t>(stream)>>>(w, Cout, Cin, Cin_pad, wp);
  LION_LAUNCH_CHECK();
  return 0;
}

int lion_conv3d_k3_fused_forward(const float *x, const float *wp, const float *bias, int B, int Cin,
                                 int Cout, int r, const float *pro_a, const float *pro_b, const float *pro_bias,
                                 const float *tconst, float *y, float *stats, int32_t *occ, lionStream_t stream) {
  if (!x || !wp || !y || B <= 0 || Cin <= 0 || Cout <= 0) return LION_EINVAL;
  if ((pro_a == nullptr) != (pro_b == nullptr)) return LION_EINVAL;
  if (tconst && !pro_a) return LION_EINVAL;
  if (occ && pro_a && !tconst) return LION_EINVAL;
  if (Cin % KC != 0 || (pro_a && Cin > 256)) return LION_EUNSUPPORTED;
  hipStream_t st = static_cast<hipStream_t>(stream);
  if (r != 8 && r != 16 && r != 32) return LION_EUNSUPPORTED;
  return launch_conv(x, wp, bias, y, B, Cin, Cout, r, pro_a, pro_b, pro_bias, tconst, stats, occ, st);
}

int lion_conv3d_k3_forward(const float *x, const float *wp, const float *bias, int B, int Cin,
                           int Cout, int r, float *y, lionStream_t stream) {
  return lion_conv3d_k3_fused_forward(x, wp, bias, B, Cin, Cout, r, nullptr, nullptr, nullptr, nullptr, y, nullptr,
                                      nullptr, stream);
}

int lion_conv3d_const_response(const float *wsum, const float *bias2, const float *bias1, const float *pro_a,
                               const float *pro_b, int B, int Cin, int Cout, float *tconst, lionStream_t stream) {
  if (!wsum || !pro_a || !pro_b || !tconst || B <= 0 || Cin <= 0 || Cout <= 0) return LION_EINVAL;
  if (Cin > 256) return LION_EUNSUPPORTED;
  conv_tconst_kernel<<<dim3(27, B), 256, 0, static_cast<hipStream_t>(stream)>>>(wsum, bias2, bias1, pro_a, pro_b, Cin,
                                                                                 Cout, tconst);
  LION_LAUNCH_CHECK();
  return 0;
}

size_t lion_conv3d_occupancy_ints(int r, int Cout, int B) {
  if (r != 16 && r != 32) return 0;
  return (size_t)2 * B * conv_plan(r, Cout, B, true).tiles + 4;
}

int lion_conv3d_tile_occupancy(const int32_t *cnt, int B, int r, int Cout, int32_t *occ_m1, int32_t *occ_m2,
                               lionStream_t stream) {
  return lion_conv3d_tile_occupancy_aware(cnt, B, r, Cout, occ_m1, occ_m2, 0, stream);
}

int lion_conv3d_tile_occupancy_aware(const int32_t *cnt, int B, int r, int Cout, int32_t *occ_m1, int32_t *occ_m2,
                                     int consumer_aware, lionStream_t stream) {
  if (!cnt || (!occ_m1 && !occ_m2) || B <= 0 || Cout <= 0) return LION_EINVAL;
  if (r != 16 && r != 32) return LION_EUNSUPPORTED;
  const ConvPlan p = conv_plan(r, Cout, B, true);
  if (!p.vb || p.tiles > 256 || (((uintptr_t)cnt) & 15) != 0) return LION_EUNSUPPORTED;
  int td, th, tw;
  conv_tile_dims(r, p.vb, &td, &th, &tw);
  conv_tile_occ_kernel<<<B, 1024, 0, static_cast<hipStream_t>(stream)>>>(cnt, r, td, th, occ_m1, occ_m2,
                                                                         consumer_aware == 2 ? 2 : consumer_aware ? 1 : 0);
  LION_LAUNCH_CHECK();
  return 0;
}

int lion_conv3d_stat_tiles(int r, int Cout, int B, int sparse) {
  if (r != 8 && r != 16 && r != 32) return 0;
  return conv_plan(r, Cout, B, sparse != 0).tiles;
}

int lion_groupnorm_fold_se(const float *stats, int B, int C, int T, int G, int voxels, const float *gamma,
                           const float *beta, const float *fac, const float *gbias, int ld_fg, float eps, const float *w1,
                           const float *w2, int H, float *A, float *Bs, lionStream_t stream) {
  if (!stats || !gamma || !beta || !fac || !gbias || !w1 || !w2 || !A || !Bs) return LION_EINVAL;
  if (B <= 0 || C <= 0 || T <= 0 || G <= 0 || C % G != 0 || ld_fg < C || H <= 0) return LION_EINVAL;
  if (C > 256 || C < 4 || H > 128) return LION_EUNSUPPORTED;
  gn_fold_se_kernel<<<B, 256, 0, static_cast<hipStream_t>(stream)>>>(stats, C, T, G, (float)voxels, gamma, beta, fac, gbias,
                                                                     ld_fg, eps, w1, w2, H, A, Bs);
  LION_LAUNCH_CHECK();
  return 0;
}

int lion_groupnorm_fold(const float *stats, int B, int C, int T, int G, int voxels, const float *gamma,
                        const float *beta, const float *fac, const float *gbias, int ld_fg, float eps,
                        float *A, float *Bs, float *chmean, lionStream_t stream) {
  if (!stats || !gamma || !beta || !fac || !gbias || !A || !Bs || !chmean) return LION_EINVAL;
  if (B <= 0 || C <= 0 || T <= 0 || G <= 0 || C % G != 0 || C / G > 64 || ld_fg < C) return LION_EINVAL;
  gn_fold_kernel<<<dim3(G, B), 256, 0, static_cast<hipStream_t>(stream)>>>(stats, C, T, G, (float)voxels, gamma,
                                                                         beta, fac, gbias, ld_fg, eps, A, Bs, chmean);
  LION_LAUNCH_CHECK();
  return 0;
}

}
```

### lion_amd/csrc/devoxelize.hip

```cpp
#include "common.h"

namespace {

template <bool V> struct BoolT { static constexpr bool value = V; };

struct Corners {
  int ix[8];
  float w[8];
};

__device__ __forceinline__ Corners corners_of(float x, float y, float z, int r, int r2) {
  Corners k;
  const float xl = floorf(x), yl = floorf(y), zl = floorf(z);
  const float xd1 = sub_rn(x, xl), yd1 = sub_rn(y, yl), zd1 = sub_rn(z, zl);
  const float xd0 = sub_rn(1.0f, xd1), yd0 = sub_rn(1.0f, yd1), zd0 = sub_rn(1.0f, zd1);
  k.w[0] = mul_rn(mul_rn(xd0, yd0), zd0);
  k.w[1] = mul_rn(mul_rn(xd0, yd0), zd1);
  k.w[2] = mul_rn(mul_rn(xd0, yd1), zd0);
  k.w[3] = mul_rn(mul_rn(xd0, yd1), zd1);
  k.w[4] = mul_rn(mul_rn(xd1, yd0), zd0);
  k.w[5] = mul_rn(mul_rn(xd1, yd0), zd1);
  k.w[6] = mul_rn(mul_rn(xd1, yd1), zd0);
  k.w[7] = mul_rn(mul_rn(xd1, yd1), zd1);
  const int xlo = (int)xl, ylo = (int)yl, zlo = (int)zl;
  const int xs = (xd1 > 0.0f) ? r2 : 0;
  const int ys = (yd1 > 0.0f) ? r : 0;
  const int zs = (zd1 > 0.0f) ? 1 : 0;
  k.ix[0] = xlo * r2 + ylo * r + zlo;
  k.ix[1] = k.ix[0] + zs;
  k.ix[2] = k.ix[0] + ys;
  k.ix[3] = k.ix[2] + zs;
  k.ix[4] = k.ix[0] + xs;
  k.ix[5] = k.ix[4] + zs;
  k.ix[6] = k.ix[4] + ys;
  k.ix[7] = k.ix[6] + zs;
  return k;
}

template <int CT, bool AFF>
__global__ __launch_bounds__(256) void devox_fwd_kernel(const float *__restrict__ coords,
                                                        const float *__restrict__ feat, int C,
                                                        int N, int r, int training,
                                                        float *__restrict__ out,
                                                        int32_t *__restrict__ inds,
                                                        float *__restrict__ wgts,
                                                        const float *__restrict__ scale,
                                                        const float *__restrict__ shift) {
  const int b = blockIdx.z, i = blockIdx.x * blockDim.x + threadIdx.x;
  if (i >= N) return;
  const int r2 = r * r, r3 = r2 * r;
  const float *co = coords + (size_t)b * 3 * N;
  Corners k = corners_of(co[i], co[i + N], co[i + 2 * N], r, r2);
  if (training && blockIdx.y == 0) {
#pragma unroll
    for (int q = 0; q < 8; ++q) {
      wgts[((size_t)b * 8 + q) * N + i] = k.w[q];
      inds[((size_t)b * 8 + q) * N + i] = k.ix[q];
    }
  }
#pragma unroll
  for (int q = 0; q < 8; ++q) k.ix[q] = min(max(k.ix[q], 0), r3 - 1);
  const int c0 = blockIdx.y * CT, c1 = min(C, c0 + CT);
  const float *f = feat + ((size_t)b * C + c0) * r3;
  float *o = out + ((size_t)b * C + c0) * N + i;
  float wsum = 0.f;
  if (AFF) {
    wsum = k.w[0];
#pragma unroll
    for (int q = 1; q < 8; ++q) wsum += k.w[q];
  }
#pragma unroll 4
  for (int c = c0; c < c1; ++c, f += r3, o += N) {
    float v[8];
#pragma unroll
    for (int q = 0; q < 8; ++q) v[q] = f[k.ix[q]];
    float acc = mul_rn(k.w[0], v[0]);
#pragma unroll
    for (int q = 1; q < 8; ++q) acc = add_rn(acc, mul_rn(k.w[q], v[q]));
    if (AFF) acc = acc * scale[(size_t)b * C + c] + shift[(size_t)b * C + c] * wsum;
    *o = acc;
  }
}


template <int LD, bool AFF>
__global__ __launch_bounds__(256) void devox_slab_kernel(
    const float *__restrict__ coords, const float *__restrict__ feat, int C, int N, int r, int PX,
    int XS, int CT, int CI, int slab_floats, int training, float *__restrict__ out,
    int32_t *__restrict__ inds, float *__restrict__ wgts, const float *__restrict__ scale,
    const float *__restrict__ shift) {
  extern __shared__ __attribute__((aligned(16))) unsigned char smem[];
  float *lds = reinterpret_cast<float *>(smem);
  constexpr int PP = 8;
  const int tid = threadIdx.x, b = blockIdx.y, c0 = blockIdx.x * CT;
  const int nch = min(CT, C - c0);
  const int r2 = r * r, r3 = r2 * r;
  const float *co = coords + (size_t)b * 3 * N;
  uint16_t *sorted = reinterpret_cast<uint16_t *>(lds + 2 * slab_floats);
  int *scnt = reinterpret_cast<int *>(sorted + ((N + 1) & ~1));
  unsigned *need = reinterpret_cast<unsigned *>(scnt + XS);

  const int ngrp = (nch + CI - 1) / CI;
  const int nit = ngrp * XS;
  auto slab_count4 = [&](int g, int xs) {
    return XS == 1 ? (min(CI, nch - g * CI) * r3) >> 2 : ((min(r, xs * PX + PX + 1) - xs * PX) * r2) >> 2;
  };
  typedef __attribute__((address_space(3))) float lds_float;
  const uint32_t lds_base = (uint32_t)(uintptr_t)(lds_float *)lds;
  const int wave = __builtin_amdgcn_readfirstlane(tid >> 6);
  auto issue = [&](int it) {
    const int g = it / XS, xs = it - g * XS;
    const float4 *src = reinterpret_cast<const float4 *>(feat + ((size_t)b * C + c0 + g * CI) * r3 + (size_t)xs * PX * r2);
    const int n4 = slab_count4(g, xs);
    const uint32_t dst0 = lds_base + (uint32_t)((it & 1) * slab_floats * 4 + wave * 1024);
    const int row0 = XS == 1 ? 0 : xs * PX * r;
#pragma unroll
    for (int j = 0; j < LD; ++j) {
      const int f = tid + j * 256;
      const float4 *gp = src + f;
      const uint32_t dst = __builtin_amdgcn_readfirstlane(dst0 + j * 4096);
      int row = (4 * f) / r;
      if (XS == 1) row %= r2;
      else row += row0;
      const bool want = f < n4 && ((need[row >> 5] >> (row & 31)) & 1u);
      if (want) {
        unsigned keep;
        asm volatile("s_mov_b32 %0, m0\n\ts_mov_b32 m0, %2\n\ts_nop 0\n\tglobal_load_lds_dwordx4 %1, off\n\ts_mov_b32 m0, %0"
                     : "=&s"(keep) : "v"(gp), "s"(dst) : "memory");
      }
    }
  };
  const int nwords = (r2 + 31) >> 5;
  for (int w = tid; w < nwords; w += 256) need[w] = 0u;
  __syncthreads();
  for (int i = tid; i < N; i += 256) {
    const float x = co[i], y = co[i + N];
    const float xl = floorf(x), yl = floorf(y);
    if (xl >= 0.f && yl >= 0.f && xl < (float)r && yl < (float)r) {
      const int x0 = (int)xl, y0 = (int)yl;
      const int x1 = min(x0 + (sub_rn(x, xl) > 0.0f ? 1 : 0), r - 1), y1 = min(y0 + (sub_rn(y, yl) > 0.0f ? 1 : 0), r - 1);
      const int ra = x0 * r + y0, rb = x0 * r + y1, rc = x1 * r + y0, rd = x1 * r + y1;
      atomicOr(&need[ra >> 5], 1u << (ra & 31));
      atomicOr(&need[rb >> 5], 1u << (rb & 31));
      atomicOr(&need[rc >> 5], 1u << (rc & 31));
      atomicOr(&need[rd >> 5], 1u << (rd & 31));
    }
  }
  __syncthreads();
  issue(0);

  for (int s2 = tid; s2 < XS; s2 += 256) scnt[s2] = 0;
  __syncthreads();
  int sl0[PP];
#pragma unroll
  for (int p = 0; p < PP; ++p) {
    const int i = tid + p * 256;
    sl0[p] = -1;
    if (i < N) {
      sl0[p] = min(max((int)floorf(co[i]) / PX, 0), XS - 1);
      if (XS > 1) atomicAdd(&scnt[sl0[p]], 1);
    }
  }
  __syncthreads();
  if (tid == 0) {
    int run = 0;
    for (int s2 = 0; s2 < XS; ++s2) { const int c = scnt[s2]; scnt[s2] = run; run += c; }
  }
  __syncthreads();
#pragma unroll
  for (int p = 0; p < PP; ++p) {
    const int i = tid + p * 256;
    if (i < N) sorted[XS > 1 ? atomicAdd(&scnt[sl0[p]], 1) : i] = (uint16_t)i;
  }
  __syncthreads();

  int ix0[PP], xsl[PP], pid[PP];
  float xd1[PP], yd1[PP], zd1[PP];
#pragma unroll
  for (int p = 0; p < PP; ++p) {
    const int k = tid + p * 256;
    xsl[p] = -1;
    ix0[p] = 0;
    pid[p] = 0;
    xd1[p] = yd1[p] = zd1[p] = 0.f;
    if (k < N) {
      const int i = sorted[k];
      pid[p] = i;
      const float x = co[i], y = co[i + N], z = co[i + 2 * N];
      const Corners kk = corners_of(x, y, z, r, r2);
      if (training && blockIdx.x == 0) {
#pragma unroll
        for (int q = 0; q < 8; ++q) {
          wgts[((size_t)b * 8 + q) * N + i] = kk.w[q];
          inds[((size_t)b * 8 + q) * N + i] = kk.ix[q];
        }
      }
      const float xl = floorf(x), yl = floorf(y), zl = floorf(z);
      xd1[p] = sub_rn(x, xl);
      yd1[p] = sub_rn(y, yl);
      zd1[p] = sub_rn(z, zl);
      ix0[p] = kk.ix[0];
      xsl[p] = min(max((int)xl / PX, 0), XS - 1);
      const int xin = (int)xl - xsl[p] * PX;
      const bool ok = xl >= 0.f && yl >= 0.f && zl >= 0.f && xl < (float)r && yl < (float)r && zl < (float)r &&
                      kk.ix[7] < r3 && xin >= 0 && xin < PX;
      if (!ok) xsl[p] = -2;
    }
  }

  for (int it = 0; it < nit; ++it) {
    const int g = it / XS, xs = it - g * XS;
    const int cg = c0 + g * CI, cin = min(CI, nch - g * CI);
    float *buf = lds + (it & 1) * slab_floats;
    asm volatile("s_waitcnt vmcnt(0)" ::: "memory");
    __syncthreads();
    if (it + 1 < nit) issue(it + 1);
    const int base = xs * PX * r2;
    float *o = out + ((size_t)b * C + cg) * N;
#pragma unroll
    for (int p = 0; p < PP; ++p) {
      if (xsl[p] == xs) {
        const float xd0 = sub_rn(1.0f, xd1[p]), yd0 = sub_rn(1.0f, yd1[p]), zd0 = sub_rn(1.0f, zd1[p]);
        const int xo = (xd1[p] > 0.0f) ? r2 : 0, yo = (yd1[p] > 0.0f) ? r : 0, zo = (zd1[p] > 0.0f) ? 1 : 0;
        const float w0 = mul_rn(mul_rn(xd0, yd0), zd0), w1 = mul_rn(mul_rn(xd0, yd0), zd1[p]);
        const float w2 = mul_rn(mul_rn(xd0, yd1[p]), zd0), w3 = mul_rn(mul_rn(xd0, yd1[p]), zd1[p]);
        const float w4 = mul_rn(mul_rn(xd1[p], yd0), zd0), w5 = mul_rn(mul_rn(xd1[p], yd0), zd1[p]);
        const float w6 = mul_rn(mul_rn(xd1[p], yd1[p]), zd0), w7 = mul_rn(mul_rn(xd1[p], yd1[p]), zd1[p]);
        float wsum = w0;
        if (AFF) { wsum += w1; wsum += w2; wsum += w3; wsum += w4; wsum += w5; wsum += w6; wsum += w7; }
        const float *f0 = buf + (ix0[p] - base);
        for (int ci = 0; ci < cin; ++ci, f0 += r3) {
          const float *f1 = f0 + xo;
          const float v0 = f0[0], v1 = f0[zo], v2 = f0[yo], v3 = f0[yo + zo];
          const float v4 = f1[0], v5 = f1[zo], v6 = f1[yo], v7 = f1[yo + zo];
          float a = mul_rn(w0, v0);
          a = add_rn(a, mul_rn(w1, v1));
          a = add_rn(a, mul_rn(w2, v2));
          a = add_rn(a, mul_rn(w3, v3));
          a = add_rn(a, mul_rn(w4, v4));
          a = add_rn(a, mul_rn(w5, v5));
          a = add_rn(a, mul_rn(w6, v6));
          a = add_rn(a, mul_rn(w7, v7));
          if (AFF) a = a * scale[(size_t)b * C + cg + ci] + shift[(size_t)b * C + cg + ci] * wsum;
          o[(size_t)ci * N + pid[p]] = a;
        }
      } else if (xsl[p] == -2 && xs == 0) {
        for (int ci = 0; ci < cin; ++ci) o[(size_t)ci * N + pid[p]] = 0.f;
      }
    }
  }
}

constexpr int DVR_R = 32, DVR_NT = 512, DVR_PP = 2048 / DVR_NT;
constexpr int DVR_RING_BYTES = 144 * 1024;
constexpr int DVR_NJ = 9;

__device__ __forceinline__ void wait_vm_uniform(int n) {
  n = __builtin_amdgcn_readfirstlane(n);
#define LION_WVM(k) case k: asm volatile("s_waitcnt vmcnt(" #k ")" ::: "memory"); break;
  switch (n < 0 ? 0 : n) {
    LION_WVM(0) LION_WVM(1) LION_WVM(2) LION_WVM(3) LION_WVM(4) LION_WVM(5) LION_WVM(6) LION_WVM(7) LION_WVM(8) LION_WVM(9)
    LION_WVM(10) LION_WVM(11) LION_WVM(12) LION_WVM(13) LION_WVM(14) LION_WVM(15) LION_WVM(16) LION_WVM(17) LION_WVM(18)
    LION_WVM(19) LION_WVM(20) LION_WVM(21) LION_WVM(22) LION_WVM(23) LION_WVM(24) LION_WVM(25) LION_WVM(26) LION_WVM(27)
    LION_WVM(28) LION_WVM(29) LION_WVM(30) LION_WVM(31) LION_WVM(32) LION_WVM(33) LION_WVM(34) LION_WVM(35) LION_WVM(36)
    LION_WVM(37) LION_WVM(38) LION_WVM(39)
  default: asm volatile("s_waitcnt vmcnt(40)" ::: "memory"); break;
  }
#undef LION_WVM
}

template <int G> constexpr int devox_plan_stride() { return 16 + (DVR_NJ * DVR_NT / (G / 4)) * 2 + 2048 * 16 + 2048; }

template <bool AFF, int G, int MODE>
__global__ __launch_bounds__(DVR_NT) void devox_ring_kernel(const float *__restrict__ coords,
                                                            const float *__restrict__ feat, int C, int N, int CT,
                                                            int training, float *__restrict__ out,
                                                            int32_t *__restrict__ inds, float *__restrict__ wgts,
                                                            const float *__restrict__ scale,
                                                            const float *__restrict__ shift, int dmax,
                                                            unsigned char *__restrict__ plan) {
  extern __shared__ __attribute__((aligned(16))) unsigned char smem[];
  constexpr int PP = DVR_PP, r = DVR_R, r2 = r * r, r3 = r2 * r, NT = DVR_NT;
  constexpr int PPR = r / G, NP = r2 * PPR, nwords = NP / 32, LP = G / 4;
  constexpr int NPMAX = DVR_NJ * NT / LP;
  static_assert(nwords <= 128, "two bitmap words per lane of the ranking wave");
  float *lds = reinterpret_cast<float *>(smem);
  const int tid = threadIdx.x, b = blockIdx.y, c0 = blockIdx.x * CT;
  const int nch = min(CT, C - c0);
  unsigned *need = reinterpret_cast<unsigned *>(smem + DVR_RING_BYTES);
  unsigned *base = need + nwords;
  uint16_t *plist = reinterpret_cast<uint16_t *>(base + nwords);
  float *s_sc = reinterpret_cast<float *>(plist + NPMAX);
  int *s_np = reinterpret_cast<int *>(s_sc + 32);
  const float *co = coords + (size_t)b * 3 * N;
  unsigned char *pl_b = (MODE != 0) ? plan + (size_t)b * devox_plan_stride<G>() : nullptr;
  const uint16_t *pl_list = reinterpret_cast<const uint16_t *>(pl_b + 16);
  uint16_t *pl_off = reinterpret_cast<uint16_t *>(pl_b + 16 + NPMAX * 2);
  signed char *pl_st = reinterpret_cast<signed char *>(pl_b + 16 + NPMAX * 2 + 2048 * 16);

  if (tid < nwords) need[tid] = 0u;
  if (AFF && tid < 2 * 16) {
    const int ci = tid & 15;
    s_sc[tid] = ci < nch ? (tid < 16 ? scale : shift)[(size_t)b * C + c0 + ci] : 0.f;
  }
  __syncthreads();
  int np = 0, nj = 0, buf_bytes = 0, D = 2;
  bool fits = false;
  int goff[DVR_NJ];
  typedef __attribute__((address_space(3))) float lds_float;
  const uint32_t lds_base = (uint32_t)(uintptr_t)(lds_float *)lds;
  const int wave = __builtin_amdgcn_readfirstlane(tid >> 6);
  int ops = 0;
  int mark[4] = {0, 0, 0, 0};
  auto ring_shape = [&]() {
    nj = (np * LP + NT - 1) / NT;
    buf_bytes = nj * NT * 16;
    D = nj == 0 ? 2 : min(min(dmax, 4), DVR_RING_BYTES / (nj ? buf_bytes : 1));
    fits = nj <= DVR_NJ && D >= 2;
  };
  auto issue = [&](int ci) {
    const float *src = feat + ((size_t)b * C + c0 + ci) * r3;
    const uint32_t dst0 = lds_base + (uint32_t)((ci % D) * buf_bytes + wave * 1024);
#pragma unroll
    for (int j = 0; j < DVR_NJ; ++j) {
      if (j < nj) {
        const uint32_t dst = __builtin_amdgcn_readfirstlane(dst0 + j * (NT * 16));
        const float *gp = src + goff[j];
        unsigned keep;
        asm volatile("s_mov_b32 %0, m0\n\ts_mov_b32 m0, %2\n\ts_nop 0\n\tglobal_load_lds_dwordx4 %1, off nt\n\ts_mov_b32 m0, %0"
                     : "=&s"(keep) : "v"(gp), "s"(dst) : "memory");
      }
    }
    ops += nj;
    mark[ci % D] = ops;
  };
  if (MODE == 1) {
    const int *hdr = reinterpret_cast<const int *>(pl_b);
    unsigned pl[DVR_NJ];
#pragma unroll
    for (int j = 0; j < DVR_NJ; ++j) pl[j] = pl_list[(tid + j * NT) / LP];
    np = __builtin_amdgcn_readfirstlane(hdr[0]);
    ring_shape();
    fits = fits && hdr[1] != 0;
    const int n4 = fits ? np * LP : 0;
#pragma unroll
    for (int j = 0; j < DVR_NJ; ++j) {
      const int f = tid + j * NT;
      goff[j] = f < n4 ? (int)pl[j] * G + (f % LP) * 4 : 0;
    }
    if (fits)
      for (int k = 0; k < D - 1 && k < nch; ++k) issue(k);
  }
  float xd1[PP], yd1[PP], zd1[PP];
  int row4[PP][4], zl_[PP], st[PP];
#pragma unroll
  for (int p = 0; p < PP; ++p) {
    const int i = tid + p * NT;
    st[p] = 0;
    xd1[p] = yd1[p] = zd1[p] = 0.f;
    row4[p][0] = row4[p][1] = row4[p][2] = row4[p][3] = zl_[p] = 0;
    if (i < N) {
      const float x = co[i], y = co[i + N], z = co[i + 2 * N];
      const Corners kk = corners_of(x, y, z, r, r2);
      if (training && blockIdx.x == 0) {
#pragma unroll
        for (int q = 0; q < 8; ++q) {
          wgts[((size_t)b * 8 + q) * N + i] = kk.w[q];
          inds[((size_t)b * 8 + q) * N + i] = kk.ix[q];
        }
      }
      const float xl = floorf(x), yl = floorf(y), zl = floorf(z);
      xd1[p] = sub_rn(x, xl);
      yd1[p] = sub_rn(y, yl);
      zd1[p] = sub_rn(z, zl);
      const bool ok = xl >= 0.f && yl >= 0.f && zl >= 0.f && xl < (float)r && yl < (float)r && zl < (float)r &&
                      kk.ix[7] < r3;
      st[p] = ok ? 1 : -2;
      if (ok) {
        const int x0 = (int)xl, y0 = (int)yl;
        const int x1 = x0 + (xd1[p] > 0.0f ? 1 : 0), y1 = y0 + (yd1[p] > 0.0f ? 1 : 0);
        zl_[p] = (int)zl;
        row4[p][0] = x0 * r + y0; row4[p][1] = x0 * r + y1; row4[p][2] = x1 * r + y0; row4[p][3] = x1 * r + y1;
        if (zl_[p] == r - 1 && zd1[p] > 0.0f) st[p] = 2;
      }
      if (MODE != 1 && st[p] == 1) {
        const int zh = zl_[p] + (zd1[p] > 0.0f ? 1 : 0);
#pragma unroll
        for (int k = 0; k < 4; ++k) {
          const int pl = row4[p][k] * PPR + zl_[p] / G, ph = row4[p][k] * PPR + zh / G;
          atomicOr(&need[pl >> 5], 1u << (pl & 31));
          if (ph != pl) atomicOr(&need[ph >> 5], 1u << (ph & 31));
        }
      }
    }
  }
  auto slot_of = [&](int pc) { return (int)(base[pc >> 5] + __popc(need[pc >> 5] & ((1u << (pc & 31)) - 1u))); };
  if (MODE != 1) {
    __syncthreads();
    if (tid < 64) {
      const int w0 = 2 * tid, w1 = 2 * tid + 1;
      const int c0_ = w0 < nwords ? __popc(need[w0]) : 0, c1_ = w1 < nwords ? __popc(need[w1]) : 0;
      const int inc = wave_incl_scan(c0_ + c1_, tid);
      if (w0 < nwords) base[w0] = (unsigned)(inc - c0_ - c1_);
      if (w1 < nwords) base[w1] = (unsigned)(inc - c1_);
      if (tid == 63) *s_np = inc;
    }
    __syncthreads();
    np = *s_np;
    ring_shape();
    if (fits)
      for (int pc = tid; pc < NP; pc += NT)
        if ((need[pc >> 5] >> (pc & 31)) & 1u) plist[slot_of(pc)] = (uint16_t)pc;
    __syncthreads();
    const int n4 = fits ? np * LP : 0;
#pragma unroll
    for (int j = 0; j < DVR_NJ; ++j) {
      const int f = tid + j * NT;
      goff[j] = f < n4 ? (int)plist[f / LP] * G + (f % LP) * 4 : 0;
    }
    if (MODE == 0 && fits)
      for (int k = 0; k < D - 1 && k < nch; ++k) issue(k);
  }
  unsigned boff[PP][8];
  float wq[PP][8], wsum4[PP];
#pragma unroll
  for (int p = 0; p < PP; ++p) {
    const int zh = zl_[p] + (zd1[p] > 0.0f ? 1 : 0);
#pragma unroll
    for (int k = 0; k < 4; ++k) {
      boff[p][2 * k] = boff[p][2 * k + 1] = 0u;
      if (MODE != 1 && fits && st[p] == 1) {
        boff[p][2 * k] = (unsigned)(slot_of(row4[p][k] * PPR + zl_[p] / G) * G + zl_[p] % G) * 4u;
        boff[p][2 * k + 1] = (unsigned)(slot_of(row4[p][k] * PPR + zh / G) * G + zh % G) * 4u;
      }
      row4[p][k] = row4[p][k] * r + zl_[p];
    }
    const float xd0 = sub_rn(1.0f, xd1[p]), yd0 = sub_rn(1.0f, yd1[p]), zd0 = sub_rn(1.0f, zd1[p]);
    wq[p][0] = mul_rn(mul_rn(xd0, yd0), zd0); wq[p][1] = mul_rn(mul_rn(xd0, yd0), zd1[p]);
    wq[p][2] = mul_rn(mul_rn(xd0, yd1[p]), zd0); wq[p][3] = mul_rn(mul_rn(xd0, yd1[p]), zd1[p]);
    wq[p][4] = mul_rn(mul_rn(xd1[p], yd0), zd0); wq[p][5] = mul_rn(mul_rn(xd1[p], yd0), zd1[p]);
    wq[p][6] = mul_rn(mul_rn(xd1[p], yd1[p]), zd0); wq[p][7] = mul_rn(mul_rn(xd1[p], yd1[p]), zd1[p]);
    float ws = wq[p][0];
#pragma unroll
    for (int q = 1; q < 8; ++q) ws += wq[p][q];
    wsum4[p] = ws;
  }
  if (MODE == 1) {
#pragma unroll
    for (int p = 0; p < PP; ++p) {
      const int i = tid + p * NT;
      const uint4 o4 = *reinterpret_cast<const uint4 *>(pl_off + (size_t)(i < 2048 ? i : 0) * 8);
      boff[p][0] = (o4.x & 0xffffu) * 4u; boff[p][1] = (o4.x >> 16) * 4u; boff[p][2] = (o4.y & 0xffffu) * 4u; boff[p][3] = (o4.y >> 16) * 4u;
      boff[p][4] = (o4.z & 0xffffu) * 4u; boff[p][5] = (o4.z >> 16) * 4u; boff[p][6] = (o4.w & 0xffffu) * 4u; boff[p][7] = (o4.w >> 16) * 4u;
    }
  }
  if (MODE == 2) {
    if (tid == 0) { int *hdr = reinterpret_cast<int *>(pl_b); hdr[0] = np; hdr[1] = fits ? 1 : 0; }
    uint16_t *wl = reinterpret_cast<uint16_t *>(pl_b + 16);
    for (int s_ = tid; s_ < NPMAX; s_ += NT) wl[s_] = (fits && s_ < np) ? plist[s_] : (uint16_t)0;
#pragma unroll
    for (int p = 0; p < PP; ++p) {
      const int i = tid + p * NT;
      if (i < 2048) {
        uint4 o4;
        o4.x = (boff[p][0] >> 2) | ((boff[p][1] >> 2) << 16); o4.y = (boff[p][2] >> 2) | ((boff[p][3] >> 2) << 16);
        o4.z = (boff[p][4] >> 2) | ((boff[p][5] >> 2) << 16); o4.w = (boff[p][6] >> 2) | ((boff[p][7] >> 2) << 16);
        *reinterpret_cast<uint4 *>(pl_off + (size_t)i * 8) = o4;
        pl_st[i] = (signed char)st[p];
      }
    }
    return;
  }
  bool any2 = false;
#pragma unroll
  for (int p = 0; p < PP; ++p) any2 |= st[p] == 2;
  const bool wave_generic = !fits || __ballot(any2) != 0ull;
  float *ob = out + ((size_t)b * C + c0) * N;
  const __amdgpu_buffer_rsrc_t ors = __builtin_amdgcn_make_buffer_rsrc(ob, 0, nch * N * 4, 0x00020000);
  for (int ci = 0; ci < nch; ++ci) {
    const float *gsrc = feat + ((size_t)b * C + c0 + ci) * r3;
    typedef __attribute__((address_space(3))) const float lds_cfloat;
    const uint32_t lbase = lds_base + (uint32_t)((ci % D) * buf_bytes);
    if (fits) {
      wait_vm_uniform(ops - mark[ci % D]);
      asm volatile("s_waitcnt lgkmcnt(0)\n\ts_barrier" ::: "memory");
      if (ci + D - 1 < nch) issue(ci + D - 1);
    }
    float sc = 1.f, sh = 0.f;
    if (AFF) { sc = s_sc[ci]; sh = s_sc[16 + ci]; }
    float a4[PP];
    auto gather = [&](auto generic_c) {
      constexpr bool GENERIC = decltype(generic_c)::value;
#pragma unroll
      for (int p = 0; p < PP; ++p) {
        float a = 0.f;
        if (st[p] > 0) {
          float v[8];
          if (!GENERIC || (fits && st[p] == 1)) {
#pragma unroll
            for (int q = 0; q < 8; ++q) v[q] = *(lds_cfloat *)(uintptr_t)(lbase + boff[p][q]);
          } else {
            const int zo = (zd1[p] > 0.0f) ? 1 : 0;
#pragma unroll
            for (int k = 0; k < 4; ++k) { v[2 * k] = gsrc[row4[p][k]]; v[2 * k + 1] = gsrc[row4[p][k] + zo]; }
          }
          a = mul_rn(wq[p][0], v[0]);
#pragma unroll
          for (int q = 1; q < 8; ++q) a = add_rn(a, mul_rn(wq[p][q], v[q]));
          if (AFF) a = a * sc + sh * wsum4[p];
        }
        a4[p] = a;
      }
    };
    if (wave_generic) gather(BoolT<true>{}); else gather(BoolT<false>{});
#pragma unroll
    for (int p = 0; p < PP; ++p) {
      const int i = tid + p * NT;
      __builtin_amdgcn_raw_buffer_store_b32(__float_as_uint(a4[p]), ors, i < N ? (ci * N + i) * 4 : 0x7fffff00, 0, 0);
    }
    ops += PP;
  }
}

__global__ __launch_bounds__(1024) void devox_bwd_lds_kernel(const float *__restrict__ gy,
                                                             const int32_t *__restrict__ inds,
                                                             const float *__restrict__ wgts, int C,
                                                             int N, int r3,
                                                             float *__restrict__ gx) {
  extern __shared__ __attribute__((aligned(16))) unsigned char smem[];
  float *slab = reinterpret_cast<float *>(smem);
  const int tid = threadIdx.x, nt = blockDim.x;
  const int c = blockIdx.x, b = blockIdx.y;
  const int part = r3 / gridDim.z, lo = blockIdx.z * part;
  for (int v = tid * 4; v < part; v += nt * 4)
    *reinterpret_cast<float4 *>(slab + v) = make_float4(0.f, 0.f, 0.f, 0.f);
  __syncthreads();
  const float *g = gy + ((size_t)b * C + c) * N;
  const int32_t *id = inds + (size_t)b * 8 * N;
  const float *wg = wgts + (size_t)b * 8 * N;
  for (int i = tid; i < N; i += nt) {
    const float gv = g[i];
#pragma unroll
    for (int q = 0; q < 8; ++q) {
      const int ix = min(max(id[(size_t)q * N + i], 0), r3 - 1) - lo;
      if (ix >= 0 && ix < part) atomicAdd(slab + ix, mul_rn(wg[(size_t)q * N + i], gv));
    }
  }
  __syncthreads();
  float *o = gx + ((size_t)b * C + c) * r3 + lo;
  for (int v = tid * 4; v < part; v += nt * 4)
    *reinterpret_cast<float4 *>(o + v) = *reinterpret_cast<const float4 *>(slab + v);
}

__global__ __launch_bounds__(1024) void devox_bwd_affine_kernel(const float *__restrict__ gy, const int32_t *__restrict__ inds,
                                                                const float *__restrict__ wgts, const float *__restrict__ x,
                                                                const float *__restrict__ Ap, const float *__restrict__ Q,
                                                                const float *__restrict__ R, int C, int N, int r3,
                                                                float *__restrict__ dx) {
  extern __shared__ __attribute__((aligned(16))) unsigned char smem[];
  float *slab = reinterpret_cast<float *>(smem);
  const int tid = threadIdx.x, nt = blockDim.x;
  const int c = blockIdx.x, b = blockIdx.y;
  const int part = r3 / gridDim.z, lo = blockIdx.z * part;
  const size_t row = (size_t)b * C + c;
  const float a = Ap[row], q = Q[row], rr = R[row];
  const float *xr = x + row * r3 + lo;
  for (int v = tid * 4; v < part; v += nt * 4) {
    const float4 t = *reinterpret_cast<const float4 *>(xr + v);
    *reinterpret_cast<float4 *>(slab + v) = make_float4(q + rr * t.x, q + rr * t.y, q + rr * t.z, q + rr * t.w);
  }
  __syncthreads();
  const float *g = gy + row * N;
  const int32_t *id = inds + (size_t)b * 8 * N;
  const float *wg = wgts + (size_t)b * 8 * N;
  for (int i = tid; i < N; i += nt) {
    const float gv = a * g[i];
#pragma unroll
    for (int k = 0; k < 8; ++k) {
      const int ix = min(max(id[(size_t)k * N + i], 0), r3 - 1) - lo;
      if (ix >= 0 && ix < part) atomicAdd(slab + ix, mul_rn(wg[(size_t)k * N + i], gv));
    }
  }
  __syncthreads();
  float *o = dx + row * r3 + lo;
  for (int v = tid * 4; v < part; v += nt * 4)
    *reinterpret_cast<float4 *>(o + v) = *reinterpret_cast<const float4 *>(slab + v);
}

__global__ void devox_bwd_atomic_kernel(const float *__restrict__ gy,
                                        const int32_t *__restrict__ inds,
                                        const float *__restrict__ wgts, int C, int N, int r3,
                                        int CT, float *__restrict__ gx) {
  const int b = blockIdx.z, i = blockIdx.x * blockDim.x + threadIdx.x;
  if (i >= N) return;
  int ix[8];
  float w[8];
  for (int q = 0; q < 8; ++q) {
    ix[q] = min(max(inds[((size_t)b * 8 + q) * N + i], 0), r3 - 1);
    w[q] = wgts[((size_t)b * 8 + q) * N + i];
  }
  const int c0 = blockIdx.y * CT, c1 = min(C, c0 + CT);
  for (int c = c0; c < c1; ++c) {
    const float gv = gy[((size_t)b * C + c) * N + i];
    for (int q = 0; q < 8; ++q) atomicAdd(gx + ((size_t)b * C + c) * r3 + ix[q], mul_rn(w[q], gv));
  }
}

}

constexpr int DVR_G = 8;
constexpr size_t DVR_LDS = (size_t)DVR_RING_BYTES + (size_t)2 * (DVR_R * DVR_R * (DVR_R / DVR_G) / 32) * 4 +
                           (size_t)(DVR_NJ * DVR_NT / (DVR_G / 4)) * 2 + 32 * 4 + 16;
static int devox_ring_depth() {
  static const int d = getenv("LION_DEVOX_RING") ? atoi(getenv("LION_DEVOX_RING")) : 4;
  return d < 2 ? 2 : d;
}

extern "C" {

static int devox_launch(const float *coords, const float *feat, int B, int C, int N, int r,
                        int training, float *out, int32_t *inds, float *wgts, const float *scale,
                        const float *shift, hipStream_t st) {
  const int r2 = r * r;
  if (r == DVR_R && N <= 2048 && (((uintptr_t)feat) & 15) == 0) {
    int CT = 8;
    while (CT > 1 && (long)B * lion_cdiv(C, CT) < 256) CT >>= 1;
    dim3 grid(lion_cdiv(C, CT), B);
    static LionLdsLimit cfgr0 = {}, cfgr1 = {};
    if (scale) {
      if (int e = lion_dynamic_lds(&devox_ring_kernel<true, DVR_G, 0>, DVR_LDS, cfgr1)) return e;
      devox_ring_kernel<true, DVR_G, 0><<<grid, DVR_NT, DVR_LDS, st>>>(coords, feat, C, N, CT, training, out, inds, wgts, scale, shift, devox_ring_depth(), nullptr);
    } else {
      if (int e = lion_dynamic_lds(&devox_ring_kernel<false, DVR_G, 0>, DVR_LDS, cfgr0)) return e;
      devox_ring_kernel<false, DVR_G, 0><<<grid, DVR_NT, DVR_LDS, st>>>(coords, feat, C, N, CT, training, out, inds, wgts, scale, shift, devox_ring_depth(), nullptr);
    }
    LION_LAUNCH_CHECK();
    return 0;
  }
  if ((r2 % 4) == 0 && N <= 2048 && r2 <= 4608 && (((uintptr_t)feat) & 15) == 0) {
    const int planes_max = 9216 / r2;
    const int PX = planes_max >= r ? r : planes_max - 1;
    const int XS = lion_cdiv(r, PX);
    const int CI = XS == 1 ? (9216 / (r2 * r) < 16 ? 9216 / (r2 * r) : 16) : 1;
    const int ld0 = lion_cdiv((XS == 1 ? CI * r2 * r : (PX + 1) * r2) / 4, 256);
    const int ld = ld0 <= 1 ? 1 : ld0 <= 2 ? 2 : ld0 <= 4 ? 4 : 9;
    const int slab_floats = ld * 1024;
    const size_t lds = (size_t)2 * slab_floats * 4 + (size_t)((N + 1) & ~1) * 2 + (size_t)XS * 4 +
                       (size_t)((r2 + 31) / 32) * 4;
    int CT = 4 * CI;
    while (CT > CI && (long)B * lion_cdiv(C, CT) < 512) CT >>= 1;
    dim3 grid(lion_cdiv(C, CT), B);
#define DEVOX_SLAB(LD_)                                                                                    \
  {                                                                                                        \
    static LionLdsLimit cfg0 = {}, cfg1 = {};                                                              \
    if (scale) {                                                                                           \
      if (int e = lion_dynamic_lds(&devox_slab_kernel<LD_, true>, lds, cfg1)) return e;                    \
      devox_slab_kernel<LD_, true><<<grid, 256, lds, st>>>(coords, feat, C, N, r, PX, XS, CT, CI, slab_floats, \
                                                           training, out, inds, wgts, scale, shift);       \
    } else {                                                                                               \
      if (int e = lion_dynamic_lds(&devox_slab_kernel<LD_, false>, lds, cfg0)) return e;                   \
      devox_slab_kernel<LD_, false><<<grid, 256, lds, st>>>(coords, feat, C, N, r, PX, XS, CT, CI, slab_floats, \
                                                            training, out, inds, wgts, scale, shift);      \
    }                                                                                                      \
  }
    if (ld <= 1) DEVOX_SLAB(1)
    else if (ld <= 2) DEVOX_SLAB(2)
    else if (ld <= 4) DEVOX_SLAB(4)
    else DEVOX_SLAB(9)
#undef DEVOX_SLAB
    LION_LAUNCH_CHECK();
    return 0;
  }
  const int pt = lion_cdiv(N, 256);
  int ct = 16;
  while (ct > 2 && (long)B * pt * lion_cdiv(C, ct) < 2048) ct >>= 1;
  dim3 grid(pt, lion_cdiv(C, ct), B);
#define DEVOX_CASE(CT_)                                                                                   \
  if (scale) devox_fwd_kernel<CT_, true><<<grid, 256, 0, st>>>(coords, feat, C, N, r, training, out, inds, wgts, scale, shift); \
  else devox_fwd_kernel<CT_, false><<<grid, 256, 0, st>>>(coords, feat, C, N, r, training, out, inds, wgts, scale, shift)
  switch (ct) {
  case 16: DEVOX_CASE(16); break;
  case 8:  DEVOX_CASE(8); break;
  case 4:  DEVOX_CASE(4); break;
  default: DEVOX_CASE(2); break;
  }
#undef DEVOX_CASE
  LION_LAUNCH_CHECK();
  return 0;
}

int lion_trilinear_devoxelize_forward(const float *coords, const float *feat, int B, int C, int N,
                                      int r, int training, float *out, int32_t *inds, float *wgts,
                                      lionStream_t stream) {
  if (!coords || !feat || !out || B <= 0 || C <= 0 || N <= 0 || r <= 0) return LION_EINVAL;
  if (training && (!inds || !wgts)) return LION_EINVAL;
  return devox_launch(coords, feat, B, C, N, r, training, out, inds, wgts, nullptr, nullptr,
                      static_cast<hipStream_t>(stream));
}

int lion_trilinear_devoxelize_affine_forward(const float *coords, const float *feat, const float *scale,
                                             const float *shift, int B, int C, int N, int r, float *out,
                                             lionStream_t stream) {
  if (!coords || !feat || !out || !scale || !shift || B <= 0 || C <= 0 || N <= 0 || r <= 0) return LION_EINVAL;
  return devox_launch(coords, feat, B, C, N, r, 0, out, nullptr, nullptr, scale, shift,
                      static_cast<hipStream_t>(stream));
}

size_t lion_devoxelize_plan_bytes(int B, int N, int r) {
  if (B <= 0 || N <= 0 || N > 2048 || r != DVR_R) return 0;
  return (size_t)B * devox_plan_stride<DVR_G>();
}

int lion_trilinear_devoxelize_plan(const float *coords, int B, int N, int r, void *plan, size_t plan_bytes,
                                   lionStream_t stream) {
  if (!coords || !plan || B <= 0 || N <= 0) return LION_EINVAL;
  const size_t need = lion_devoxelize_plan_bytes(B, N, r);
  if (!need || (((uintptr_t)plan) & 15) != 0) return LION_EUNSUPPORTED;
  if (plan_bytes < need) return LION_EWORKSPACE;
  static LionLdsLimit cfg = {};
  if (int e = lion_dynamic_lds(&devox_ring_kernel<false, DVR_G, 2>, DVR_LDS, cfg)) return e;
  devox_ring_kernel<false, DVR_G, 2><<<dim3(1, B), DVR_NT, DVR_LDS, static_cast<hipStream_t>(stream)>>>(
      coords, nullptr, 1, N, 1, 0, nullptr, nullptr, nullptr, nullptr, nullptr, devox_ring_depth(),
      static_cast<unsigned char *>(plan));
  LION_LAUNCH_CHECK();
  return 0;
}

int lion_trilinear_devoxelize_planned_forward(const void *plan, size_t plan_bytes, const float *coords, const float *feat,
                                              const float *scale, const float *shift, int B, int C, int N, int r,
                                              float *out, lionStream_t stream) {
  if (!plan || !coords || !feat || !out || B <= 0 || C <= 0 || N <= 0) return LION_EINVAL;
  if ((scale == nullptr) != (shift == nullptr)) return LION_EINVAL;
  const size_t need = lion_devoxelize_plan_bytes(B, N, r);
  if (!need || (((uintptr_t)plan) & 15) != 0 || (((uintptr_t)feat) & 15) != 0) return LION_EUNSUPPORTED;
  if (plan_bytes < need) return LION_EWORKSPACE;
  hipStream_t st = static_cast<hipStream_t>(stream);
  int CT = 8;
  while (CT > 1 && (long)B * lion_cdiv(C, CT) < 256) CT >>= 1;
  dim3 grid(lion_cdiv(C, CT), B);
  unsigned char *pl = const_cast<unsigned char *>(static_cast<const unsigned char *>(plan));
  static LionLdsLimit cfg0 = {}, cfg1 = {};
  if (scale) {
    if (int e = lion_dynamic_lds(&devox_ring_kernel<true, DVR_G, 1>, DVR_LDS, cfg1)) return e;
    devox_ring_kernel<true, DVR_G, 1><<<grid, DVR_NT, DVR_LDS, st>>>(coords, feat, C, N, CT, 0, out, nullptr, nullptr, scale, shift, devox_ring_depth(), pl);
  } else {
    if (int e = lion_dynamic_lds(&devox_ring_kernel<false, DVR_G, 1>, DVR_LDS, cfg0)) return e;
    devox_ring_kernel<false, DVR_G, 1><<<grid, DVR_NT, DVR_LDS, st>>>(coords, feat, C, N, CT, 0, out, nullptr, nullptr, nullptr, nullptr, devox_ring_depth(), pl);
  }
  LION_LAUNCH_CHECK();
  return 0;
}

int lion_trilinear_devoxelize_backward(const float *gy, const int32_t *inds, const float *wgts,
                                       int B, int C, int N, int r3, float *gx,
                                       lionStream_t stream) {
  if (!gy || !inds || !wgts || !gx || B <= 0 || C <= 0 || N <= 0 || r3 <= 0) return LION_EINVAL;
  hipStream_t st = static_cast<hipStream_t>(stream);
  if ((size_t)r3 * 4 <= 128 * 1024 && (r3 % 4) == 0) {
    int parts = (size_t)r3 * 4 > 64 * 1024 ? 2 : 1;
    if (r3 % (4 * parts) != 0) parts = 1;
    const size_t lds = (size_t)(r3 / parts) * 4;
    static LionLdsLimit configured = {};
    if (int e = lion_dynamic_lds(&devox_bwd_lds_kernel, lds, configured)) return e;
    const int nt = r3 >= 16384 ? 1024 : 256;
    devox_bwd_lds_kernel<<<dim3(C, B, parts), nt, lds, st>>>(gy, inds, wgts, C, N, r3, gx);
    LION_LAUNCH_CHECK();
    return 0;
  }
  hipError_t e = hipMemsetAsync(gx, 0, (size_t)B * C * r3 * 4, st);
  if (e != hipSuccess) return (int)e;
  const int CT = 8;
  devox_bwd_atomic_kernel<<<dim3(lion_cdiv(N, 256), lion_cdiv(C, CT), B), 256, 0, st>>>(
      gy, inds, wgts, C, N, r3, CT, gx);
  LION_LAUNCH_CHECK();
  return 0;
}

int lion_trilinear_devoxelize_backward_affine(const float *gy, const int32_t *inds, const float *wgts, const float *x,
                                              const float *Ap, const float *Q, const float *R, int B, int C, int N, int r3,
                                              float *dx, lionStream_t stream) {
  if (!gy || !inds || !wgts || !x || !Ap || !Q || !R || !dx || B <= 0 || C <= 0 || N <= 0 || r3 <= 0) return LION_EINVAL;
  if ((size_t)r3 * 4 > 128 * 1024 || (r3 % 8) != 0 || (((uintptr_t)x | (uintptr_t)dx) & 15) != 0) return LION_EUNSUPPORTED;
  hipStream_t st = static_cast<hipStream_t>(stream);
  const int parts = (size_t)r3 * 4 > 64 * 1024 ? 2 : 1;
  const size_t lds = (size_t)(r3 / parts) * 4;
  static LionLdsLimit configured = {};
  if (int e = lion_dynamic_lds(&devox_bwd_affine_kernel, lds, configured)) return e;
  const int nt = r3 >= 16384 ? 1024 : 256;
  devox_bwd_affine_kernel<<<dim3(C, B, parts), nt, lds, st>>>(gy, inds, wgts, x, Ap, Q, R, C, N, r3, dx);
  LION_LAUNCH_CHECK();
  return 0;
}

}
```

### lion_amd/csrc/pointwise.hip

```cpp
#include "common.h"

namespace {

__device__ __forceinline__ float swishf(float t) { return swish_fast(t); }

__global__ __launch_bounds__(256) void row_stats_kernel(const float *__restrict__ x, int L,
                                                        float *__restrict__ stats) {
  __shared__ float r1[4], r2[4];
  const int row = blockIdx.x, tid = threadIdx.x, lane = tid & 63, wave = tid >> 6;
  const float *p = x + (size_t)row * L;
  float s1 = 0.f, s2 = 0.f;
  if ((L & 3) == 0) {
    for (int i = tid * 4; i < L; i += 1024) {
      const float4 v = *reinterpret_cast<const float4 *>(p + i);
      s1 += (v.x + v.y) + (v.z + v.w);
      s2 += (v.x * v.x + v.y * v.y) + (v.z * v.z + v.w * v.w);
    }
  } else {
    for (int i = tid; i < L; i += 256) { const float v = p[i]; s1 += v; s2 += v * v; }
  }
  s1 = row16_sum_rn(s1); s2 = row16_sum_rn(s2);
#pragma unroll
  for (int m = 16; m < 64; m <<= 1) { s1 += __shfl_xor(s1, m, 64); s2 += __shfl_xor(s2, m, 64); }
  if (lane == 0) { r1[wave] = s1; r2[wave] = s2; }
  __syncthreads();
  if (tid == 0) {
    stats[(size_t)row * 2] = (r1[0] + r1[1]) + (r1[2] + r1[3]);
    stats[(size_t)row * 2 + 1] = (r2[0] + r2[1]) + (r2[2] + r2[3]);
  }
}

__global__ __launch_bounds__(256) void affine_swish_kernel(const float *__restrict__ x,
                                                           const float *__restrict__ A,
                                                           const float *__restrict__ Bs, int L,
                                                           float *__restrict__ y) {
  const int row = blockIdx.y;
  const float a = A[row], b = Bs[row];
  const float *p = x + (size_t)row * L;
  float *q = y + (size_t)row * L;
  const int i = (blockIdx.x * 256 + threadIdx.x) * 4;
  if (i + 3 < L && (L & 3) == 0) {
    const float4 v = *reinterpret_cast<const float4 *>(p + i);
    *reinterpret_cast<float4 *>(q + i) =
        make_float4(swishf(v.x * a + b), swishf(v.y * a + b), swishf(v.z * a + b), swishf(v.w * a + b));
  } else {
    for (int j = i; j < L && j < i + 4; ++j) q[j] = swishf(p[j] * a + b);
  }
}

__global__ __launch_bounds__(256) void affine_swish_add_kernel(const float *__restrict__ x, const float *__restrict__ A,
                                                               const float *__restrict__ Bs,
                                                               const float *__restrict__ addend, int L,
                                                               float *__restrict__ y) {
  const int row = blockIdx.y;
  const float a = A[row], b = Bs[row];
  const float *p = x + (size_t)row * L, *ad = addend + (size_t)row * L;
  float *q = y + (size_t)row * L;
  const int i = (blockIdx.x * 256 + threadIdx.x) * 4;
  if (i + 3 < L && (L & 3) == 0) {
    const float4 v = *reinterpret_cast<const float4 *>(p + i), w = *reinterpret_cast<const float4 *>(ad + i);
    *reinterpret_cast<float4 *>(q + i) = make_float4(swishf(v.x * a + b) + w.x, swishf(v.y * a + b) + w.y,
                                                     swishf(v.z * a + b) + w.z, swishf(v.w * a + b) + w.w);
  } else {
    for (int j = i; j < L && j < i + 4; ++j) q[j] = swishf(p[j] * a + b) + ad[j];
  }
}

__global__ void timestep_embedding_kernel(const float *__restrict__ t, const float *__restrict__ row, float scale, int B,
                                          int half, int D, float *__restrict__ emb) {
  const int e = blockIdx.x * blockDim.x + threadIdx.x;
  if (e >= B * D) return;
  const int b = e / D, i = e - b * D;
  float v = 0.f;
  if (i < 2 * half) {
    const float ang = mul_rn(mul_rn(t[b], scale), row[i < half ? i : i - half]);
    v = i < half ? sinf(ang) : cosf(ang);
  }
  emb[e] = v;
}

__global__ __launch_bounds__(256) void affine_swish_max_kernel(const float *__restrict__ x,
                                                               const float *__restrict__ A,
                                                               const float *__restrict__ Bs, int M,
                                                               int U, float *__restrict__ y) {
  const int row = blockIdx.y, m = blockIdx.x * 256 + threadIdx.x;
  if (m >= M) return;
  const float a = A[row], b = Bs[row];
  const float *p = x + ((size_t)row * M + m) * U;
  float best = -INFINITY;
  if ((U & 3) == 0) {
    for (int u = 0; u < U; u += 4) {
      const float4 v = *reinterpret_cast<const float4 *>(p + u);
      best = fmaxf(best, fmaxf(fmaxf(swishf(v.x * a + b), swishf(v.y * a + b)),
                               fmaxf(swishf(v.z * a + b), swishf(v.w * a + b))));
    }
  } else {
    for (int u = 0; u < U; ++u) best = fmaxf(best, swishf(p[u] * a + b));
  }
  y[(size_t)row * M + m] = best;
}

template <int LPM>
__global__ __launch_bounds__(256) void affine_swish_max_coop_kernel(const float *__restrict__ x,
                                                                    const float *__restrict__ A,
                                                                    const float *__restrict__ Bs, int M,
                                                                    float *__restrict__ y) {
  constexpr int MPW = 64 / LPM;
  constexpr int IT = 8;
  const int row = blockIdx.y, lane = threadIdx.x & 63, wave = threadIdx.x >> 6;
  const float a = A[row], b = Bs[row];
  const int m0 = (blockIdx.x * 4 + wave) * MPW * IT;
  const float4 *p = reinterpret_cast<const float4 *>(x + (size_t)row * M * (LPM * 4));
  float4 v[IT];
#pragma unroll
  for (int i = 0; i < IT; ++i) {
    const int m = min(m0 + i * MPW + lane / LPM, M - 1);
    v[i] = p[(size_t)m * LPM + (lane % LPM)];
  }
#pragma unroll
  for (int i = 0; i < IT; ++i) {
    float best = fmaxf(fmaxf(swishf(v[i].x * a + b), swishf(v[i].y * a + b)),
                       fmaxf(swishf(v[i].z * a + b), swishf(v[i].w * a + b)));
    if (LPM >= 2) best = fmaxf(best, LION_DPP_F32(best, 0xB1));
    if (LPM >= 4) best = fmaxf(best, LION_DPP_F32(best, 0x4E));
    if (LPM >= 8) best = fmaxf(best, LION_DPP_F32(best, 0x141));
    if (LPM >= 16) best = fmaxf(best, LION_DPP_F32(best, 0x140));
    const int m = m0 + i * MPW + lane / LPM;
    if ((lane % LPM) == 0 && m < M) y[(size_t)row * M + m] = best;
  }
}

__global__ __launch_bounds__(256) void se_gate_kernel(const float *__restrict__ chmean,
                                                      const float *__restrict__ w1,
                                                      const float *__restrict__ w2, int C, int H,
                                                      float *__restrict__ A, float *__restrict__ Bs) {
  __shared__ float sm[1024], sh[128];
  const int b = blockIdx.x, tid = threadIdx.x, lane = tid & 63, wave = tid >> 6;
  for (int c = tid; c < C; c += 256) sm[c] = A[(size_t)b * C + c] * chmean[(size_t)b * C + c] + Bs[(size_t)b * C + c];
  __syncthreads();
  for (int j = wave; j < H; j += 4) {
    float acc = 0.f;
    for (int c = lane; c < C; c += 64) acc += w1[(size_t)j * C + c] * sm[c];
#pragma unroll
    for (int m = 32; m >= 1; m >>= 1) acc += __shfl_xor(acc, m, 64);
    if (lane == 0) sh[j] = acc > 0.f ? acc : 0.f;
  }
  __syncthreads();
  for (int c = tid; c < C; c += 256) {
    float acc = 0.f;
    for (int j = 0; j < H; ++j) acc += w2[(size_t)c * H + j] * sh[j];
    const float g = 1.0f / (1.0f + expf(-acc));
    A[(size_t)b * C + c] *= g;
    Bs[(size_t)b * C + c] *= g;
  }
}


__global__ __launch_bounds__(256) void latent_unpack_kernel(const float *__restrict__ x, int N, int D,
                                                            float *__restrict__ all, float *__restrict__ coords,
                                                            float *__restrict__ rest) {
  __shared__ float tile[256 * 9];
  const int b = blockIdx.y, n0 = blockIdx.x * 256, tid = threadIdx.x;
  const int np = min(256, N - n0);
  const float *src = x + ((size_t)b * N + n0) * D;
  for (int i = tid; i < np * D; i += 256) tile[(i / D) * (D + 1) + i % D] = src[i];
  __syncthreads();
  if (tid >= np) return;
  for (int d = 0; d < D; ++d) {
    const float v = tile[tid * (D + 1) + d];
    if (all) all[((size_t)b * D + d) * N + n0 + tid] = v;
    if (coords && d < 3) coords[((size_t)b * 3 + d) * N + n0 + tid] = v;
    if (rest && d >= 3) rest[((size_t)b * (D - 3) + d - 3) * N + n0 + tid] = v;
  }
}

__global__ __launch_bounds__(256) void concat_broadcast_kernel(const float *__restrict__ a, const float *__restrict__ t,
                                                               int Ca, int Ct, int N4, int ld_t, float4 *__restrict__ out) {
  const int row = blockIdx.y, C = Ca + Ct, b = row / C, c = row % C;
  float4 *o = out + (size_t)row * N4;
  if (c < Ca) {
    const float4 *s = reinterpret_cast<const float4 *>(a) + ((size_t)b * Ca + c) * N4;
    for (int i = blockIdx.x * 256 + threadIdx.x; i < N4; i += gridDim.x * 256) o[i] = s[i];
  } else {
    const float v = t[(size_t)b * ld_t + c - Ca];
    for (int i = blockIdx.x * 256 + threadIdx.x; i < N4; i += gridDim.x * 256) o[i] = make_float4(v, v, v, v);
  }
}

}

extern "C" {

int lion_row_stats(const float *x, int rows, int L, float *stats, lionStream_t stream) {
  if (!x || !stats || rows <= 0 || L <= 0) return LION_EINVAL;
  row_stats_kernel<<<rows, 256, 0, static_cast<hipStream_t>(stream)>>>(x, L, stats);
  LION_LAUNCH_CHECK();
  return 0;
}

int lion_affine_swish(const float *x, const float *A, const float *Bs, int rows, int L, float *y,
                      lionStream_t stream) {
  if (!x || !A || !Bs || !y || rows <= 0 || L <= 0) return LION_EINVAL;
  affine_swish_kernel<<<dim3(lion_cdiv(lion_cdiv(L, 4), 256), rows), 256, 0, static_cast<hipStream_t>(stream)>>>(
      x, A, Bs, L, y);
  LION_LAUNCH_CHECK();
  return 0;
}

int lion_timestep_embedding(const float *t, const float *row, float scale, int B, int half, int D, float *emb,
                            lionStream_t stream) {
  if (!t || !row || !emb || B <= 0 || half <= 0 || D < 2 * half) return LION_EINVAL;
  timestep_embedding_kernel<<<lion_cdiv(B * D, 256), 256, 0, static_cast<hipStream_t>(stream)>>>(t, row, scale, B, half, D, emb);
  LION_LAUNCH_CHECK();
  return 0;
}

int lion_affine_swish_add(const float *x, const float *A, const float *Bs, const float *addend, int rows, int L, float *y,
// ... 55 lines not shown
```

### lion_amd/fused_ops.py

```python
import os

import torch

from . import _lib
from ._wcache import WeightCache
from . import conv_ops
from .conv_ops import packed_weight, supported


def _border_sums(weight):
    m = torch.tensor([[0., 1., 1.], [1., 1., 1.], [1., 1., 0.]], dtype=torch.float64, device=weight.device)
    ws = torch.einsum("oidhw,ad,bh,cw->abcio", weight.detach().double(), m, m, m)
    return ws.reshape(27, weight.shape[1], weight.shape[0]).float().contiguous()


_WSUM_CACHE = WeightCache(_border_sums)


def border_weight_sums(weight):
    return _WSUM_CACHE.get(weight)


def conv3d_occupancy(counts, r, cout, b, consumer_aware=False):
    lib = _lib.load()
    n = lib.lion_conv3d_occupancy_ints(r, cout, b)
    buf = torch.empty((2, n), device=counts.device, dtype=torch.int32)
    _lib.call("lion_conv3d_tile_occupancy_aware", counts.contiguous(), b, r, cout, buf[0], buf[1], int(consumer_aware))
    return buf[0], buf[1]


class FoldSpec:

    def __init__(self, gn: torch.nn.GroupNorm, fac, gbias, count, se=None):
        self.gn, self.fac, self.gbias, self.count, self.se = gn, fac, gbias, int(count), se

    def apply(self, stats):
        if self.se is not None:
            merged = groupnorm_fold_se(stats, self.gn, self.fac, self.gbias, self.count, self.se)
            if merged is not None:
                return merged
            a, b_, m = groupnorm_fold(stats, self.gn, self.fac, self.gbias, self.count)
            return se_gate_(a, b_, m, self.se)
        a, b_, _ = groupnorm_fold(stats, self.gn, self.fac, self.gbias, self.count)
        return a, b_


def conv3d_fused(x, conv, pro=None, want_stats=True, occ=None, prev_conv=None, split=None, fold=None):
    lib = _lib.load()
    b, cin, r = x.shape[0], x.shape[1], x.shape[2]
    cout = conv.out_channels
    use_split = conv_ops.use_split(split, cin, cout, r)
    if cin % 4:
        assert pro is None
        x = torch.cat([x, x.new_zeros(b, 4 - cin % 4, r, r, r)], dim=1)
        cin = x.shape[1]
    x = x.contiguous()
    wp = conv_ops.split_packed_weight(conv.weight) if use_split else packed_weight(conv.weight)
    y = torch.empty((b, cout, r, r, r), device=x.device, dtype=torch.float32)
    pa = pb = pbias = tconst = None
    if pro is not None:
        pa, pb = pro[0].contiguous(), pro[1].contiguous()
    bias = conv.bias.detach().contiguous() if conv.bias is not None else None
    sparse = occ is not None and r >= 16
    if sparse and pro is not None:
        if prev_conv is None or cin > 256:
            sparse = False
        else:
            ws = border_weight_sums(conv.weight)
            pbias = prev_conv.bias.detach().contiguous() if prev_conv.bias is not None else None
            tconst = torch.empty((b, 27, cout), device=x.device, dtype=torch.float32)
            _lib.call("lion_conv3d_const_response", ws, bias, pbias, pa, pb, b, cin, cout, tconst)
    stats = None
    if want_stats:
        tiles = lib.lion_conv3d_split_stat_tiles(r, cout) if use_split else lib.lion_conv3d_stat_tiles(r, cout, b, int(sparse))
        stats = torch.empty((b, cout, tiles, 2), device=x.device, dtype=torch.float32)
    if not sparse:
        occ = None
    _lib.call("lion_conv3d_k3_split_forward" if use_split else "lion_conv3d_k3_fused_forward",
              x, wp, bias, b, cin, cout, r, pa, pb, pbias, tconst, y, stats, occ)
    if fold is not None:
        return y, fold.apply(stats)
    return y, stats


def groupnorm_fold(stats, gn: torch.nn.GroupNorm, fac, gbias, voxels):
    b, c, t, _ = stats.shape
    A = torch.empty((b, c), device=stats.device, dtype=torch.float32)
    Bs = torch.empty_like(A)
    cm = torch.empty_like(A)
    if not (fac.stride(1) == 1 and gbias.stride(1) == 1 and fac.stride(0) == gbias.stride(0) and fac.stride(0) >= c):
        fac, gbias = fac.contiguous(), gbias.contiguous()
    _lib.call("lion_groupnorm_fold", stats, b, c, t, gn.num_groups, int(voxels), gn.weight, gn.bias, fac, gbias,
              int(fac.stride(0)), float(gn.eps), A, Bs, cm)
    return A, Bs, cm


def groupnorm_fold_se(stats, gn: torch.nn.GroupNorm, fac, gbias, voxels, se):
    b, c, t, _ = stats.shape
    w1, w2 = se.fc[0].weight.detach(), se.fc[2].weight.detach()
    h = w1.shape[0]
    if c > 256 or c < 4 or h > 128 or not (w1.is_contiguous() and w2.is_contiguous()):
        return None
    A = torch.empty((b, c), device=stats.device, dtype=torch.float32)
    Bs = torch.empty_like(A)
    if not (fac.stride(1) == 1 and gbias.stride(1) == 1 and fac.stride(0) == gbias.stride(0) and fac.stride(0) >= c):
        fac, gbias = fac.contiguous(), gbias.contiguous()
    _lib.call("lion_groupnorm_fold_se", stats, b, c, t, gn.num_groups, int(voxels), gn.weight, gn.bias, fac, gbias,
              int(fac.stride(0)), float(gn.eps), w1, w2, h, A, Bs)
    return A, Bs


def se_gate_(A, Bs, chmean, se):
    w1, w2 = se.fc[0].weight.detach(), se.fc[2].weight.detach()
    h, c = w1.shape
    if c > 1024 or h > 128 or not (w1.is_contiguous() and w2.is_contiguous()):
        gate = se.fc(A * chmean + Bs)
        return A * gate, Bs * gate
    _lib.call("lion_se_gate", chmean, w1, w2, A.shape[0], c, h, A, Bs)
    return A, Bs


def devoxelize_plan(coords, r):
    lib = _lib.load()
    b, _, n = coords.shape
    nbytes = lib.lion_devoxelize_plan_bytes(b, n, int(r))
    if nbytes == 0 or not coords.is_contiguous() or coords.dtype != torch.float32:
        return None
    buf = torch.empty((nbytes,), device=coords.device, dtype=torch.uint8)
    _lib.call("lion_trilinear_devoxelize_plan", coords, b, n, int(r), buf, nbytes)
    return {"buf": buf, "coords": coords, "shape": (b, n, int(r))}


def devoxelize_affine(grid, coords, r, scale, shift, plan=None):
    b, c = grid.shape[:2]
    n = coords.shape[2]
    out = torch.empty((b, c, n), device=grid.device, dtype=torch.float32)
    co_c, gr_c, sc_c, sh_c = coords.contiguous(), grid.contiguous(), scale.contiguous(), shift.contiguous()
    if plan is not None and plan["shape"] == (b, n, int(r)) and plan["coords"].data_ptr() == co_c.data_ptr():
        buf = plan["buf"]
        _lib.call("lion_trilinear_devoxelize_planned_forward", buf, buf.numel(), co_c, gr_c, sc_c, sh_c, b, c, n, int(r), out)
        return out
    _lib.call("lion_trilinear_devoxelize_affine_forward", co_c, gr_c, sc_c, sh_c, b, c, n, int(r), out)
    return out


def fusable(conv1, conv2, r, x):
    return (x.is_cuda and x.dtype == torch.float32 and not torch.is_autocast_enabled()
            and supported(conv1.in_channels, conv1.out_channels, r)
            and supported(conv2.in_channels, conv2.out_channels, r)
            and conv2.in_channels % 4 == 0 and conv2.in_channels <= 256)


def _pw_pack(weight):
    return conv_ops.pack_with(weight, "lion_pwconv_packed_floats", "lion_pwconv_pack_weights", torch.float32, as_matrix=True)


_PW_CACHE = WeightCache(_pw_pack)
PW_ALL = os.environ.get("LION_PW_ALL", "1") != "0"


def pw_packed_weight(weight):
    return _PW_CACHE.get(weight)


def _pw_split_pack(weight):
    return conv_ops.pack_with(weight, "lion_pwconv_split_packed_halfs", "lion_pwconv_split_pack_weights", torch.int16,
                              as_matrix=True)


_PW_SPLIT_CACHE = WeightCache(_pw_split_pack)
PW_SPLIT = os.environ.get("LION_PW_SPLIT", "1") != "0"


def pw_use_split(split, b, cin, cout, L):
    can = cin * L < (1 << 29) and cin <= 4096
    if split is None:
        return PW_SPLIT and can and b * L >= 8192 and (L <= 4096 or cin * cout >= 8192)
    return bool(split) and can


def pw_supported(conv, x):
    if not PW_ALL:
        L = x[0, 0].numel()
        if not (conv.out_channels in (32, 64, 128, 256) and L >= 1024 and x.shape[0] * L * conv.out_channels >= (1 << 22)):
            return False
    return (conv.groups == 1 and all(k == 1 for k in conv.kernel_size) and all(s == 1 for s in conv.stride)
            and all(p == 0 for p in conv.padding) and x.is_cuda and x.dtype == torch.float32 and x[0, 0].numel() > 0
            and _lib.load().lion_pwconv_stat_tiles(conv.out_channels, conv.in_channels, x[0, 0].numel()) > 0)


def pwconv_fused(x, conv, pro=None, want_stats=True, split=None):
    lib = _lib.load()
    x = x.contiguous()
    b, cin = x.shape[:2]
    L = x[0, 0].numel()
    cout = conv.out_channels
    use_split = pw_use_split(split, b, cin, cout, L)
    wp = _PW_SPLIT_CACHE.get(conv.weight) if use_split else pw_packed_weight(conv.weight)
    y = torch.empty((b, cout) + tuple(x.shape[2:]), device=x.device, dtype=torch.float32)
    tiles = (lib.lion_pwconv_split_stat_tiles if use_split else lib.lion_pwconv_stat_tiles)(cout, cin, L)
    stats = torch.empty((b, cout, tiles, 2), device=x.device, dtype=torch.float32) if want_stats else None
    pa = pb = None
    if pro is not None:
        pa, pb = pro[0].contiguous(), pro[1].contiguous()
    bias = conv.bias.detach().contiguous() if conv.bias is not None else None
    _lib.call("lion_pwconv_split_forward" if use_split else "lion_pwconv_forward",
              x, wp, bias, b, cin, cout, L, pa, pb, y, stats)
    return y, stats


MAX_RECOMPUTE = os.environ.get("LION_PW_MAX_RECOMPUTE", "0") != "0"


def pwconv_max_recompute(x, conv, gn, style, pro):
    lib = _lib.load()
    x = x.contiguous()
    b, cin, m, u = x.shape
    L = m * u
    cout = conv.out_channels
    wp = pw_packed_weight(conv.weight)
    tiles = lib.lion_pwconv_stat_tiles(cout, cin, L)
    if tiles <= 0:
        return None
    stats = torch.empty((b, cout, tiles, 2), device=x.device, dtype=torch.float32)
    pa = pb = None
    if pro is not None:
        pa, pb = pro[0].contiguous(), pro[1].contiguous()
    bias = conv.bias.detach().contiguous() if conv.bias is not None else None
    if not _lib.call("lion_pwconv_forward_max", x, wp, bias, b, cin, cout, L, pa, pb, None, None, stats, None,
                     unsupported_ok=True):
        return None
    f, g = gn.affine(style)
    A, Bs, _ = groupnorm_fold(stats, gn.norm, f, g, L)
    y = torch.empty((b, cout, m), device=x.device, dtype=torch.float32)
    _lib.call("lion_pwconv_forward_max", x, wp, bias, b, cin, cout, L, pa, pb, A, Bs, None, y)
    return y


def pwconv_raw(x, w2d, bias=None, cached_param=None, transposed=False):
    lib = _lib.load()
    x = x.contiguous()
    b, cin = x.shape[:2]
    cout = w2d.shape[1] if transposed else w2d.shape[0]
    L = x[0, 0].numel()
    if not (x.is_cuda and x.dtype == torch.float32 and L > 0 and lib.lion_pwconv_stat_tiles(cout, cin, L) > 0):
        return None
    use_split = pw_use_split(None, b, cin, cout, L)
    if transposed and use_split and cached_param is not None:
        wf = _PW_SPLIT_CACHE.get(cached_param)
        wp = torch.empty((lib.lion_pwconv_split_packed_halfs(cout, cin),), device=x.device, dtype=torch.int16)
        _lib.call("lion_pwconv_split_pack_weights_t", w2d.detach().contiguous(), cin, cout, wf, wp)
    elif transposed:
        wp = (_pw_split_pack if use_split else _pw_pack)(w2d.detach().t().contiguous())
    elif cached_param is not None:
        wp = _PW_SPLIT_CACHE.get(cached_param) if use_split else _PW_CACHE.get(cached_param)
    else:
        wp = (_pw_split_pack if use_split else _pw_pack)(w2d)
    y = torch.empty((b, cout) + tuple(x.shape[2:]), device=x.device, dtype=torch.float32)
    bias_c = bias.detach().contiguous() if bias is not None else None
    _lib.call("lion_pwconv_split_forward" if use_split else "lion_pwconv_forward",
              x, wp, bias_c, b, cin, cout, L, None, None, y, None)
    return y


def pwconv_wgrad(x, gy, want_bias=False):
    lib = _lib.load()
    x, gy = x.contiguous(), gy.contiguous()
    b, cin = x.shape[:2]
    cout = gy.shape[1]
    L = x[0, 0].numel()
    wsb = lib.lion_pwconv_wgrad_workspace_bytes(b, cin, cout, L)
    ws = torch.empty((wsb,), device=x.device, dtype=torch.uint8)
    gw = torch.empty((cout, cin), device=x.device, dtype=torch.float32)
    gb = torch.empty((cout,), device=x.device, dtype=torch.float32) if want_bias else None
    _lib.call("lion_pwconv_wgrad", x, gy, b, cin, cout, L, ws, wsb, gw, gb)
    return (gw, gb) if want_bias else gw


def group_points(coords, centers, feat, idx):
    b, _, n = coords.shape
    m, u = idx.shape[1], idx.shape[2]
    c = 0 if feat is None else feat.shape[1]
    out = torch.empty((b, 3 + c, m, u), device=coords.device, dtype=torch.float32)
    _lib.call("lion_group_points_forward", coords.contiguous(), centers.contiguous(), None if feat is None else feat.contiguous(),
              idx.contiguous(), b, c, n, m, u, out)
    return out


def linear_rows(x, weight, bias=None, act=0, slope=0.0):
    x = x.contiguous()
    b, k = x.shape
    o = weight.shape[0]
    wp = pw_packed_weight(weight)
    y = torch.empty((b, o), device=x.device, dtype=torch.float32)
    bias_c = bias.detach().contiguous() if bias is not None else None
    _lib.call("lion_linear_forward", x, wp, bias_c, b, k, o, int(act), float(slope), y)
# ... 200 lines not shown
```

### lion_amd/models/pvcnn2_ada.py

```python
import contextlib
import functools
import os

import torch
import torch.nn as nn
from einops import rearrange

from .. import functional as F
from ..conv_ops import conv3d_module
from .. import fused_ops

FUSE_INFERENCE = True
SPARSE_CONV1 = True
OVERLAP_POINT_BRANCH = os.environ.get("LION_OVERLAP_POINT_BRANCH", "0") != "0"
_POINT_STREAMS = {}


_VOX_PLANS = None
VOX_PLAN = os.environ.get("LION_VOX_PLAN", "1") != "0"
OCC_PLAN = os.environ.get("LION_OCC_PLAN", "1") != "0"
SKIP_UNREAD = os.environ.get("LION_CONV_SKIP_UNREAD", "1") != "0"
SKIP_UNREAD_LEVEL2 = os.environ.get("LION_CONV_SKIP_UNREAD_LEVEL2", "1") != "0"
OCC_CLONE = os.environ.get("LION_OCC_CLONE", "0") != "0"
DEVOX_PLAN = os.environ.get("LION_DEVOX_PLAN", "1") != "0"


@contextlib.contextmanager
def voxel_plans():
    global _VOX_PLANS
    prev, _VOX_PLANS = _VOX_PLANS, ({} if VOX_PLAN else None)
    try:
        yield
    finally:
        _VOX_PLANS = prev


def _occupancy(counts, r, cout, b, level=None):
    if level is None:
        level = 1 if SKIP_UNREAD else 0
    if _VOX_PLANS is None or not OCC_PLAN:
        return fused_ops.conv3d_occupancy(counts, r, cout, b, consumer_aware=level)
    key = ("occ", counts.data_ptr(), tuple(counts.shape), int(r), int(b), int(level))
    hit = _VOX_PLANS.get(key)
    if hit is None:
        o1, o2 = fused_ops.conv3d_occupancy(counts, r, cout, b, consumer_aware=level)
        hit = (counts, (o1, o2))
        _VOX_PLANS[key] = hit
    if OCC_CLONE:
        return hit[1][0].clone(), hit[1][1].clone()
    return hit[1]


def _devox_plan(voxel_coords, r):
    if _VOX_PLANS is None or not DEVOX_PLAN or r != 32 or voxel_coords.shape[2] > 2048 or not voxel_coords.is_contiguous():
        return None
    key = ("devox", voxel_coords.data_ptr(), tuple(voxel_coords.shape), int(r))
    hit = _VOX_PLANS.get(key)
    if hit is None:
        plan = fused_ops.devoxelize_plan(voxel_coords, r)
        hit = (voxel_coords, plan)
        _VOX_PLANS[key] = hit
    return hit[1]


def _point_stream(device):
    key = (device.type, device.index)
    if key not in _POINT_STREAMS:
        _POINT_STREAMS[key] = torch.cuda.Stream(device=device)
    return _POINT_STREAMS[key]
from .adagn import AdaGN


class SE3d(nn.Module):

    def __init__(self, channel, reduction=8):
        super().__init__()
        self.fc = nn.Sequential(
            nn.Linear(channel, channel // reduction, bias=False),
            nn.ReLU(inplace=True),
            nn.Linear(channel // reduction, channel, bias=False),
            nn.Sigmoid())
        self.channel = channel

    def __repr__(self):
        return f"SE({self.channel}, {self.channel})"

    def gate(self, inputs):
        return self.fc(inputs.mean(-1).mean(-1).mean(-1))

    def forward(self, inputs):
        return inputs * self.gate(inputs).view(inputs.shape[0], inputs.shape[1], 1, 1, 1)


class LinearAttention(nn.Module):

    def __init__(self, dim, heads=4, dim_head=32, verbose=True):
        super().__init__()
        self.heads = heads
        hidden_dim = dim_head * heads
        self.to_qkv = nn.Conv2d(dim, hidden_dim * 3, 1, bias=False)
        self.to_out = nn.Conv2d(hidden_dim, dim, 1)

    def forward(self, x):
        if own_kernels(x) and self.to_qkv.out_channels == 3 * self.heads * 32 and fused_ops.pw_supported(self.to_qkv, x):
            qkv = fused_ops.pwconv_fused(x, self.to_qkv, None, want_stats=False)[0]
            core = fused_ops.linear_attention_core(qkv, self.heads, 32)
            return fused_ops.pwconv_fused(core, self.to_out, None, want_stats=False)[0]
        x = x.unsqueeze(-1)
        b, c, h, w = x.shape
        qkv = self.to_qkv(x)
        from .. import train_ops
        if w == 1 and self.to_qkv.out_channels == 3 * self.heads * 32 and train_ops.attention_trainable(qkv.squeeze(-1), self.heads, 32):
            out = train_ops.linear_attention_core(qkv.squeeze(-1), self.heads)
            return self.to_out(out.unsqueeze(-1)).squeeze(-1)
        q, k, v = rearrange(qkv, 'b (qkv heads c) h w -> qkv b heads c (h w)', heads=self.heads, qkv=3)
        k = k.softmax(dim=-1)
        context = torch.einsum('bhdn,bhen->bhde', k, v)
        out = torch.einsum('bhde,bhdn->bhen', context, q)
        out = rearrange(out, 'b heads c (h w) -> b (heads c) h w', heads=self.heads, h=h, w=w)
        return self.to_out(out).squeeze(-1)


def swish(input):
    return input * torch.sigmoid(input)


class Swish(nn.Module):
    def forward(self, input):
        return swish(input)


class BallQuery(nn.Module):

    def __init__(self, radius, num_neighbors, include_coordinates=True):
        super().__init__()
        self.radius = radius
        self.num_neighbors = num_neighbors
        self.include_coordinates = include_coordinates

    def forward(self, points_coords, centers_coords, points_features=None):
        with torch.autocast("cuda", enabled=False):
            points_coords = points_coords.float().contiguous()
            centers_coords = centers_coords.float().contiguous()
            neighbor_indices = F.ball_query(centers_coords, points_coords, self.radius, self.num_neighbors)
            if own_kernels(points_coords) and self.include_coordinates and points_coords.shape[1] == 3 \
                    and (points_features is None or points_features.dtype == torch.float32):
                return fused_ops.group_points(points_coords, centers_coords, points_features, neighbor_indices)
            neighbor_coordinates = F.grouping(points_coords, neighbor_indices)
            neighbor_coordinates = neighbor_coordinates - centers_coords.unsqueeze(-1)
            if points_features is None:
                assert self.include_coordinates, 'No Features For Grouping'
                return neighbor_coordinates
            neighbor_features = F.grouping(points_features.float(), neighbor_indices)
            if self.include_coordinates:
                neighbor_features = torch.cat([neighbor_coordinates, neighbor_features], dim=1)
            return neighbor_features

    def extra_repr(self):
        return 'radius={}, num_neighbors={}{}'.format(
            self.radius, self.num_neighbors, ', include coordinates' if self.include_coordinates else '')


def own_kernels(x):
    return (FUSE_INFERENCE and x.is_cuda and x.dtype == torch.float32 and not torch.is_grad_enabled()
            and not torch.is_autocast_enabled())


# ... 34 lines not shown
    return module


def run_layers(layers, x, style, conv, reduce_max=False):
    from .. import train_ops
    i, n = 0, len(layers)
    while i < n:
        layer = layers[i]
        if isinstance(layer, AdaGN):
            if train_ops.usable(x) and layer.n_channel <= 1024:
                fused_act = i + 1 < n and isinstance(layers[i + 1], Swish)
                factor, bias = layer.affine(style)
                if (not fused_act and i + 1 < n and isinstance(layers[i + 1], SE3d) and x.dim() == 5
                        and train_ops.se3d_trainable(layers[i + 1], x)):
                    x = train_ops.adagn_se(x, layer.norm, factor, bias, layers[i + 1])
                    i += 2
                    continue
                if reduce_max and i + (2 if fused_act else 1) == n and train_ops.adagn_act_max_usable(x):
                    return train_ops.adagn_act_max(x, layer.norm, factor, bias, act=fused_act)
                i += 2 if fused_act else 1
                drop_p, used = train_ops.fusable_dropout(layers, i) if fused_act else (0.0, 0)
                x = train_ops.adagn_act(x, layer.norm, factor, bias, act=fused_act, dropout_p=drop_p)
                i += used
                continue
            x = layer(x, style)
        elif isinstance(layer, (nn.Conv1d, nn.Conv2d, nn.Conv3d)):
            x = conv(layer, x)
        elif isinstance(layer, SE3d) and train_ops.se3d_trainable(layer, x):
            x = train_ops.se3d(layer, x)
        else:
            x = layer(x)
        i += 1
    return x.max(dim=-1).values if reduce_max else x


class SharedMLP(nn.Module):

    def __init__(self, in_channels, out_channels, dim=1, cfg={}):
        assert len(cfg) > 0, cfg
        super().__init__()
        conv = nn.Conv1d if dim == 1 else nn.Conv2d
        if not isinstance(out_channels, (list, tuple)):
            out_channels = [out_channels]
        layers = []
        for oc in out_channels:
            layers += [conv(in_channels, oc, 1), AdaGN(dim, cfg, oc), Swish()]
            in_channels = oc
        self.layers = nn.ModuleList(layers)

    def _fusable(self, x):
        return (FUSE_INFERENCE and not self.training and not torch.is_grad_enabled() and x.is_cuda
                and x.dtype == torch.float32 and not torch.is_autocast_enabled())

    def _run(self, x, style, reduce_max=False, add=None):
        if self._fusable(x):
            n = len(self.layers) // 3
            convs, gns = [self.layers[3 * i] for i in range(n)], [self.layers[3 * i + 1] for i in range(n)]
            return fused_ops.shared_mlp(x, convs, gns, style, reduce_max, add=add)
        x = run_layers(list(self.layers), x, style, conv1x1, reduce_max=reduce_max)
        return x if add is None else x + add

    def forward_max(self, x, style):
        return self._run(x, style, reduce_max=True)

    def forward(self, *inputs):
        if len(inputs) == 1 and len(inputs[0]) == 4:
            inputs = inputs[0]
        if len(inputs) == 4:
            x, _, _, style = inputs
            return (self._run(x, style), *inputs[1:])
        if len(inputs) == 2:
            return self._run(*inputs)
        raise NotImplementedError


class Voxelization(nn.Module):

    def __init__(self, resolution, normalize=True, eps=0):
        super().__init__()
        self.r = int(resolution)
        self.normalize = normalize
        self.eps = eps

    def forward(self, features, coords, return_counts=False, sparse_reader=False):
        coords = coords.detach()
        if return_counts:
            from ..functional.backend import _backend
            b, c = features.shape[:2]
            co = coords[:, :3].float().contiguous()
            plan = None
            if _VOX_PLANS is not None and hasattr(_backend, "voxel_index"):
                key = (co.data_ptr(), tuple(co.shape), self.r, bool(self.normalize), float(self.eps))
                hit = _VOX_PLANS.get(key)
                if hit is None:
                    plan = _backend.voxel_index(co, self.r, self.normalize, self.eps)
                    if plan is not None:
                        _VOX_PLANS[key] = (co, plan)
                else:
                    plan = hit[1]
            if plan is not None:
                occ_m1 = None
                if sparse_reader and SKIP_UNREAD and SPARSE_CONV1 and self.r in (16, 32) and hasattr(_backend, "voxel_scatter"):
                    occ_m1 = _occupancy(plan["cnt"], self.r, 64, b, int(sparse_reader))[0]
                out = _backend.voxel_scatter(features.float().contiguous(), plan, occ_m1)
                return out.view(b, c, self.r, self.r, self.r), plan["norm"], plan["cnt"]
            out, norm_coords, _, counts = _backend.voxelize_points_forward(
                features.float().contiguous(), co, self.r, self.normalize, self.eps)
            return out.view(b, c, self.r, self.r, self.r), norm_coords, counts
        if features is None:
            from ..functional.backend import _backend
            _, norm_coords, _, _ = _backend.voxelize_points_forward(
                None, coords[:, :3].float().contiguous(), self.r, self.normalize, self.eps)
            return features, norm_coords
        return F.voxelize_points(features, coords, self.r, self.normalize, self.eps)

    def extra_repr(self):
        return 'resolution={}{}'.format(
            self.r, ', normalized eps = {}'.format(self.eps) if self.normalize else '')


class PVConv(nn.Module):

    def __init__(self, in_channels, out_channels, kernel_size, resolution, normalize=1, eps=0,
                 with_se=False, add_point_feat=True, attention=False, dropout=0.1, verbose=True,
                 cfg={}):
        super().__init__()
        assert len(cfg) > 0, cfg
        self.resolution = resolution
        self.voxelization = Voxelization(resolution, normalize=normalize, eps=eps)
        norm = functools.partial(AdaGN, 3, cfg)
        voxel_layers = [
            nn.Conv3d(in_channels, out_channels, kernel_size, stride=1, padding=kernel_size // 2),
            norm(out_channels),
            Swish(),
            nn.Dropout(dropout),
            nn.Conv3d(out_channels, out_channels, kernel_size, stride=1, padding=kernel_size // 2),
            norm(out_channels),
        ]
        if with_se:
            voxel_layers.append(SE3d(out_channels))
        self.voxel_layers = nn.ModuleList(voxel_layers)
        self.attn = LinearAttention(out_channels, verbose=verbose) if attention else None
        if add_point_feat:
            self.point_features = SharedMLP(in_channels, out_channels, cfg=cfg)
        self.add_point_feat = add_point_feat

    def _aware_level(self):
        if not SKIP_UNREAD:
            return 0
        from .. import conv_ops
        conv2 = self.voxel_layers[4]
        return 2 if (SKIP_UNREAD_LEVEL2 and conv_ops.use_split(None, conv2.in_channels, conv2.out_channels, self.resolution)) else 1

    def _fused_voxel_branch(self, grid, voxel_coords, style, counts=None):
        conv1, gn1, conv2, gn2 = self.voxel_layers[0], self.voxel_layers[1], self.voxel_layers[4], self.voxel_layers[5]
        se = self.voxel_layers[6] if len(self.voxel_layers) > 6 else None
        r = self.resolution
        occ1 = occ2 = None
        if SPARSE_CONV1 and counts is not None and r >= 16:
            occ1, occ2 = _occupancy(counts, r, conv1.out_channels, grid.shape[0], self._aware_level())
        f1, g1 = gn1.affine(style)
        y1, (a1, b1) = fused_ops.conv3d_fused(grid, conv1, None, True, occ1,
                                              fold=fused_ops.FoldSpec(gn1.norm, f1, g1, r ** 3))
        f2, g2 = gn2.affine(style)
        y2, (a2, b2) = fused_ops.conv3d_fused(y1, conv2, (a1, b1), True, occ2, prev_conv=conv1,
                                              fold=fused_ops.FoldSpec(gn2.norm, f2, g2, r ** 3, se))
        return fused_ops.devoxelize_affine(y2, voxel_coords, r, a2, b2, plan=_devox_plan(voxel_coords, r))

    def forward(self, inputs):
        features, coords_input, time_emb, style = inputs
        coords = coords_input[:, :3] if coords_input.shape[1] > 3 else coords_input
        assert features.shape[0] == coords.shape[0] and features.shape[2] == coords.shape[2], \
            f'get feat: {features.shape} and {coords.shape}'
        assert coords.shape[1] == 3, f'expect coords: B,3,Npoint, get: {coords.shape}'
        counts = None
        if (FUSE_INFERENCE and not self.training and not torch.is_grad_enabled() and features.is_cuda
                and not torch.is_autocast_enabled()):
            will_fuse = fused_ops.fusable(self.voxel_layers[0], self.voxel_layers[4], self.resolution, features.float())
            grid, voxel_coords, counts = self.voxelization(features, coords, return_counts=True,
                                                           sparse_reader=self._aware_level() if will_fuse else 0)
        else:
            grid, voxel_coords = self.voxelization(features, coords)
        if (FUSE_INFERENCE and not self.training and not torch.is_grad_enabled()
                and fused_ops.fusable(self.voxel_layers[0], self.voxel_layers[4], self.resolution, grid)):
            pf = None
            if self.add_point_feat and OVERLAP_POINT_BRANCH:
                main, side = torch.cuda.current_stream(features.device), _point_stream(features.device)
                side.wait_stream(main)
                with torch.cuda.stream(side):
                    pf = self.point_features(features, style)
            fused = self._fused_voxel_branch(grid, voxel_coords, style, counts)
            if pf is not None:
                main.wait_stream(side)
                pf.record_stream(main)
                fused = fused + pf
            elif self.add_point_feat:
                fused = self.point_features._run(features, style, add=fused)
            if self.attn is not None:
                fused = self.attn(fused)
            return fused, coords_input, time_emb, style
        layers = list(self.voxel_layers)
        from .. import train_ops
        if (self.training and len(layers) >= 2 and isinstance(layers[-1], SE3d) and isinstance(layers[-2], AdaGN)
                and train_ops.usable(grid) and layers[-2].n_channel <= 1024 and train_ops.adagn_se_devox_usable(grid, layers[-1])):
            grid = run_layers(layers[:-2], grid, style, conv3d_module)
            factor, bias = layers[-2].affine(style)
            fused = train_ops.adagn_se_devox(grid, layers[-2].norm, factor, bias, layers[-1], voxel_coords, self.resolution)
        else:
            grid = run_layers(layers, grid, style, conv3d_module)
            fused = F.trilinear_devoxelize(grid, voxel_coords, self.resolution, self.training)
        if self.add_point_feat:
            fused = fused + self.point_features(features, style)
        if self.attn is not None:
            fused = self.attn(fused)
        return fused, coords_input, time_emb, style


class PointNetAModule(nn.Module):

    def __init__(self, in_channels, out_channels, include_coordinates=True, cfg={}):
        super().__init__()
        if not isinstance(out_channels, (list, tuple)):
            out_channels = [[out_channels]]
        elif not isinstance(out_channels[0], (list, tuple)):
            out_channels = [out_channels]
        mlps, total = [], 0
        for oc in out_channels:
            mlps.append(SharedMLP(in_channels + (3 if include_coordinates else 0), oc, dim=1, cfg=cfg))
            total += oc[-1]
        self.include_coordinates = include_coordinates
        self.out_channels = total
        self.mlps = nn.ModuleList(mlps)

    def forward(self, inputs):
        features, coords, time_emb, style = inputs
        if self.include_coordinates:
            features = torch.cat([features, coords], dim=1)
        coords = torch.zeros((coords.size(0), 3, 1), device=coords.device)
        pooled = [mlp(features, style).max(dim=-1, keepdim=True).values for mlp in self.mlps]
        return (torch.cat(pooled, dim=1) if len(pooled) > 1 else pooled[0]), coords, time_emb

    def extra_repr(self):
        return f'out_channels={self.out_channels}, include_coordinates={self.include_coordinates}'


class PointNetSAModule(nn.Module):

    def __init__(self, num_centers, radius, num_neighbors, in_channels, out_channels,
                 include_coordinates=True, cfg={}):
        super().__init__()
        if not isinstance(radius, (list, tuple)):
            radius = [radius]
        if not isinstance(num_neighbors, (list, tuple)):
            num_neighbors = [num_neighbors] * len(radius)
        assert len(radius) == len(num_neighbors)
        if not isinstance(out_channels, (list, tuple)):
            out_channels = [[out_channels]] * len(radius)
        elif not isinstance(out_channels[0], (list, tuple)):
            out_channels = [out_channels] * len(radius)
        assert len(radius) == len(out_channels)
        groupers, mlps, total = [], [], 0
        for rad, oc, nn_ in zip(radius, out_channels, num_neighbors):
            groupers.append(BallQuery(radius=rad, num_neighbors=nn_, include_coordinates=include_coordinates))
            mlps.append(SharedMLP(in_channels + (3 if include_coordinates else 0), oc, dim=2, cfg=cfg))
            total += oc[-1]
        self.num_centers = num_centers
        self.out_channels = total
        self.groupers = nn.ModuleList(groupers)
        self.mlps = nn.ModuleList(mlps)

    def forward(self, inputs):
        features, coords, time_emb, style = inputs[0], inputs[1], inputs[2], inputs[3]
        if coords.shape[1] > 3:
            coords = coords[:, :3]
        centers_coords = F.furthest_point_sample(coords, self.num_centers)
        S = centers_coords.shape[-1]
        if time_emb is not None and type(time_emb) is not dict:
            time_emb = time_emb[:, :, :S]
        pooled = [mlp.forward_max(grouper(coords, centers_coords, features), style)
                  for grouper, mlp in zip(self.groupers, self.mlps)]
        out = torch.cat(pooled, dim=1) if len(pooled) > 1 else pooled[0]
        return out, centers_coords, time_emb, style

    def extra_repr(self):
        return f'num_centers={self.num_centers}, out_channels={self.out_channels}'


class PointNetFPModule(nn.Module):

    def __init__(self, in_channels, out_channels, cfg={}):
        super().__init__()
        self.mlp = SharedMLP(in_channels=in_channels, out_channels=out_channels, dim=1, cfg=cfg)

    def forward(self, inputs):
        if len(inputs) == 5:
            points_coords, centers_coords, centers_features, time_emb, style = inputs
            points_features = None
        elif len(inputs) == 6:
            points_coords, centers_coords, centers_features, points_features, time_emb, style = inputs
        else:
            raise NotImplementedError
        interpolated = None
        if isinstance(centers_features, tuple):
            cfeat, ctemb = centers_features
            interpolated = fused_ops.three_nn_interpolate_cat(points_coords, centers_coords, cfeat, ctemb, points_features)
            if interpolated is None:
                centers_features = torch.cat([cfeat, ctemb], dim=1)
        if interpolated is None:
            interpolated = F.nearest_neighbor_interpolate(points_coords, centers_coords, centers_features)
            if points_features is not None:
                interpolated = torch.cat([interpolated, points_features], dim=1)
        if time_emb is not None:
            time_emb = time_emb[:, :, 0:1].expand(-1, -1, points_coords.shape[-1])
        return self.mlp(interpolated, style), points_coords, time_emb, style


def _linear_gn_relu(in_channels, out_channels):
    return nn.Sequential(nn.Linear(in_channels, out_channels), nn.GroupNorm(8, out_channels), Swish())


def create_mlp_components(in_channels, out_channels, classifier=False, dim=2, width_multiplier=1, cfg={}):
    r = width_multiplier
    block = _linear_gn_relu if dim == 1 else SharedMLP
    if not isinstance(out_channels, (list, tuple)):
        out_channels = [out_channels]
    if len(out_channels) == 0 or (len(out_channels) == 1 and out_channels[0] is None):
        return nn.Sequential(), in_channels, in_channels
    layers = []
    for oc in out_channels[:-1]:
        if oc < 1:
            layers.append(nn.Dropout(oc))
        else:
            oc = int(r * oc)
            layers.append(block(in_channels, oc, cfg=cfg))
            in_channels = oc
    if dim == 1:
        layers.append(nn.Linear(in_channels, out_channels[-1]) if classifier
                      else _linear_gn_relu(in_channels, int(r * out_channels[-1])))
# ... 85 lines not shown
```

Before: 5.377.

## Fuse point-branch GroupNorm fold and residual add into voxel branch kernels

Adds a short-chain path for PVConv inference. The point-branch 1x1 conv runs before voxelization, and its GroupNorm fold is merged with the conv1 fold in one launch. That same launch also computes the border constant response (tconst) for conv2. The devoxelize kernel then applies the point branch's affine+swish as a fused residual add, removing several small kernel launches and a separate elementwise pass over point features. The trade-off is more complex kernels with shape restrictions, plus fallbacks when they are unsupported.

```diff
diff --git a/include/lion_hip.h b/include/lion_hip.h
--- a/include/lion_hip.h
+++ b/include/lion_hip.h
@@ -139,6 +139,17 @@
 int lion_groupnorm_fold(const float *stats, int B, int C, int T, int G, int voxels, const float *gamma,
                         const float *beta, const float *fac, const float *gbias, int ld_fg, float eps,
                         float *A, float *Bs, float *chmean, lionStream_t stream);
+int lion_groupnorm_fold_pair(int B, const float *stats0, int C0, int T0, int G0, int voxels0, const float *gamma0,
+                             const float *beta0, const float *fac0, const float *gbias0, int ld_fg0, float eps0, float *A0,
+                             float *Bs0, float *chmean0, const float *stats1, int C1, int T1, int G1, int voxels1,
+                             const float *gamma1, const float *beta1, const float *fac1, const float *gbias1, int ld_fg1,
+                             float eps1, float *A1, float *Bs1, float *chmean1, lionStream_t stream);
+int lion_groupnorm_fold_tconst(int B, const float *stats0, int C0, int T0, int G0, int voxels0, const float *gamma0,
+                               const float *beta0, const float *fac0, const float *gbias0, int ld_fg0, float eps0, float *A0,
+                               float *Bs0, float *chmean0, const float *stats1, int C1, int T1, int G1, int voxels1,
+                               const float *gamma1, const float *beta1, const float *fac1, const float *gbias1, int ld_fg1,
+                               float eps1, float *A1, float *Bs1, float *chmean1, const float *wsum, const float *bias2,
+                               const float *bias1, int Cout, float *tconst, lionStream_t stream);
 size_t lion_conv3d_split_packed_halfs(int Cout, int Cin);
 int lion_conv3d_split_pack_weights(const float *w, int Cout, int Cin, uint16_t *wp, lionStream_t stream);
 int lion_conv3d_split_stat_tiles(int r, int Cout);
@@ -166,12 +177,20 @@
 int lion_trilinear_devoxelize_affine_forward(const float *coords, const float *feat, const float *scale,
                                              const float *shift, int B, int C, int N, int r, float *out,
                                              lionStream_t stream);
+int lion_trilinear_devoxelize_affine_residual_forward(const float *coords, const float *feat, const float *scale,
+                                                      const float *shift, const float *res, const float *res_a,
+                                                      const float *res_b, int B, int C, int N, int r, float *out,
+                                                      lionStream_t stream);
 size_t lion_devoxelize_plan_bytes(int B, int N, int r);
 int lion_trilinear_devoxelize_plan(const float *coords, int B, int N, int r, void *plan, size_t plan_bytes,
                                    lionStream_t stream);
 int lion_trilinear_devoxelize_planned_forward(const void *plan, size_t plan_bytes, const float *coords, const float *feat,
                                               const float *scale, const float *shift, int B, int C, int N, int r,
                                               float *out, lionStream_t stream);
+int lion_trilinear_devoxelize_planned_residual_forward(const void *plan, size_t plan_bytes, const float *coords,
+                                                       const float *feat, const float *scale, const float *shift,
+                                                       const float *res, const float *res_a, const float *res_b, int B,
+                                                       int C, int N, int r, float *out, lionStream_t stream);
 
 int lion_row_stats(const float *x, int rows, int L, float *stats, lionStream_t stream);
 size_t lion_pwconv_packed_floats(int Cout, int Cin);
diff --git a/lion_amd/_lib.py b/lion_amd/_lib.py
--- a/lion_amd/_lib.py
+++ b/lion_amd/_lib.py
@@ -56,6 +56,9 @@
     "lion_conv3d_split_stat_tiles": (_i, [_i, _i]),
     "lion_conv3d_k3_split_forward": (_i, [_vp, _vp, _vp, _i, _i, _i, _i, _vp, _vp, _vp, _vp, _vp, _vp, _vp, _vp]),
     "lion_groupnorm_fold": (_i, [_vp, _i, _i, _i, _i, _i, _vp, _vp, _vp, _vp, _i, _f, _vp, _vp, _vp, _vp]),
+    "lion_groupnorm_fold_pair": (_i, [_i] + 2 * [_vp, _i, _i, _i, _i, _vp, _vp, _vp, _vp, _i, _f, _vp, _vp, _vp] + [_vp]),
+    "lion_groupnorm_fold_tconst": (_i, [_i] + 2 * [_vp, _i, _i, _i, _i, _vp, _vp, _vp, _vp, _i, _f, _vp, _vp, _vp]
+                                   + [_vp, _vp, _vp, _i, _vp, _vp]),
     "lion_groupnorm_fold_se": (_i, [_vp, _i, _i, _i, _i, _i, _vp, _vp, _vp, _vp, _i, _f, _vp, _vp, _i, _vp, _vp, _vp]),
     "lion_skinny_packed_floats": (_sz, [_i, _i]),
     "lion_skinny_pack_weights": (_i, [_vp, _i, _i, _vp, _vp]),
@@ -67,9 +70,12 @@
     "lion_from_channel_major": (_i, [_vp, _i, _i, _vp, _vp]),
     "lion_se_gate": (_i, [_vp, _vp, _vp, _i, _i, _i, _vp, _vp, _vp]),
     "lion_trilinear_devoxelize_affine_forward": (_i, [_vp, _vp, _vp, _vp, _i, _i, _i, _i, _vp, _vp]),
+    "lion_trilinear_devoxelize_affine_residual_forward": (_i, [_vp, _vp, _vp, _vp, _vp, _vp, _vp, _i, _i, _i, _i, _vp, _vp]),
     "lion_devoxelize_plan_bytes": (_sz, [_i, _i, _i]),
     "lion_trilinear_devoxelize_plan": (_i, [_vp, _i, _i, _i, _vp, _sz, _vp]),
     "lion_trilinear_devoxelize_planned_forward": (_i, [_vp, _sz, _vp, _vp, _vp, _vp, _i, _i, _i, _i, _vp, _vp]),
+    "lion_trilinear_devoxelize_planned_residual_forward": (_i, [_vp, _sz, _vp, _vp, _vp, _vp, _vp, _vp, _vp, _i, _i, _i, _i,
+                                                                 _vp, _vp]),
     "lion_row_stats": (_i, [_vp, _i, _i, _vp, _vp]),
     "lion_pwconv_packed_floats": (_sz, [_i, _i]),
     "lion_pwconv_pack_weights": (_i, [_vp, _i, _i, _vp, _vp]),
diff --git a/lion_amd/chain.py b/lion_amd/chain.py
--- a/lion_amd/chain.py
+++ b/lion_amd/chain.py
@@ -15,7 +15,7 @@
     from .models import pvcnn2_ada
     return (pvcnn2_ada.SPARSE_CONV1, pvcnn2_ada.FUSE_INFERENCE, pvcnn2_ada.OVERLAP_POINT_BRANCH, geometry.ENABLED,
             geometry.SPLIT_GRAPH, conv_ops.SPLIT, fused_ops.PW_SPLIT, pvcnn2_ada.VOX_PLAN, TEMB_TABLE, fused_ops.MAX_RECOMPUTE,
-            pvcnn2_ada.SKIP_UNREAD, pvcnn2_ada.SKIP_UNREAD_LEVEL2, CHANNEL_MAJOR_EPS)
+            pvcnn2_ada.SKIP_UNREAD, pvcnn2_ada.SKIP_UNREAD_LEVEL2, CHANNEL_MAJOR_EPS, pvcnn2_ada.SHORT_CHAIN, fused_ops.RING_RESIDUAL, fused_ops.FOLD_TCONST)
 
 
 class GraphedChain:
diff --git a/lion_amd/csrc/common.h b/lion_amd/csrc/common.h
--- a/lion_amd/csrc/common.h
+++ b/lion_amd/csrc/common.h
@@ -56,6 +56,7 @@
 }
 
 __device__ __forceinline__ float swish_fast(float t) { return t * __builtin_amdgcn_rcpf(1.0f + __expf(-t)); }
+__device__ __forceinline__ float affine_swish_plus(float x, float a, float b, float w) { return swish_fast(x * a + b) + w; }
 
 __device__ __forceinline__ float sqdist3(float ax, float ay, float az, float bx, float by,
                                          float bz) {
diff --git a/lion_amd/csrc/conv3d.hip b/lion_amd/csrc/conv3d.hip
--- a/lion_amd/csrc/conv3d.hip
+++ b/lion_amd/csrc/conv3d.hip
@@ -248,13 +248,14 @@
   }
 }
 
-__global__ void gn_fold_kernel(const float *__restrict__ stats, int C, int T, int G, float count,
-                               const float *__restrict__ gamma, const float *__restrict__ beta,
-                               const float *__restrict__ fac, const float *__restrict__ gbias, int ld_fg, float eps,
-                               float *__restrict__ A, float *__restrict__ Bs, float *__restrict__ chmean) {
+__device__ __forceinline__ void gn_fold_group(const float *__restrict__ stats, int C, int T, int G, float count,
+                                              const float *__restrict__ gamma, const float *__restrict__ beta,
+                                              const float *__restrict__ fac, const float *__restrict__ gbias, int ld_fg,
+                                              float eps, float *__restrict__ A, float *__restrict__ Bs,
+                                              float *__restrict__ chmean, int b, int g) {
   __shared__ double cs[64][2];
   __shared__ double gs[2];
-  const int b = blockIdx.y, g = blockIdx.x, cpg = C / G, tid = threadIdx.x;
+  const int cpg = C / G, tid = threadIdx.x;
   int cp2 = 1;
   while (cp2 < cpg) cp2 <<= 1;
   const int LPC = 256 / cp2, ch = tid / LPC, sub = tid % LPC;
@@ -298,6 +299,30 @@
     A[(size_t)b * C + c] = a0 * f;
     Bs[(size_t)b * C + c] = (beta[c] - (float)mean * a0) * f + gb;
   }
+}
+
+__global__ void gn_fold_kernel(const float *__restrict__ stats, int C, int T, int G, float count,
+                               const float *__restrict__ gamma, const float *__restrict__ beta,
+                               const float *__restrict__ fac, const float *__restrict__ gbias, int ld_fg, float eps,
+                               float *__restrict__ A, float *__restrict__ Bs, float *__restrict__ chmean) {
+  gn_fold_group(stats, C, T, G, count, gamma, beta, fac, gbias, ld_fg, eps, A, Bs, chmean, blockIdx.y, blockIdx.x);
+}
+
+struct GnFoldProblem {
+  const float *stats, *gamma, *beta, *fac, *gbias;
+  float *A, *Bs, *chmean;
+  int C, T, G, ld_fg;
+  float count, eps;
+};
+
+__global__ void gn_fold_pair_kernel(const GnFoldProblem p0, const GnFoldProblem p1) {
+  const int g = blockIdx.x, b = blockIdx.y;
+  if (g < p0.G)
+    gn_fold_group(p0.stats, p0.C, p0.T, p0.G, p0.count, p0.gamma, p0.beta, p0.fac, p0.gbias, p0.ld_fg, p0.eps, p0.A, p0.Bs,
+                  p0.chmean, b, g);
+  else
+    gn_fold_group(p1.stats, p1.C, p1.T, p1.G, p1.count, p1.gamma, p1.beta, p1.fac, p1.gbias, p1.ld_fg, p1.eps, p1.A, p1.Bs,
+                  p1.chmean, b, g - p0.G);
 }
 
 __global__ __launch_bounds__(256) void gn_fold_se_kernel(const float *__restrict__ stats, int C, int T, int G, float count,
@@ -437,6 +462,85 @@
   }
 }
 
+constexpr int GFT_G = 8;
+__global__ __launch_bounds__(256) void gn_fold_tconst_kernel(const GnFoldProblem p0, const GnFoldProblem p1,
+                                                             const float *__restrict__ wsum,
+                                                             const float *__restrict__ bias2,
+                                                             const float *__restrict__ bias1, int Cout,
+                                                             float *__restrict__ tconst) {
+  const int cfg = blockIdx.x, b = blockIdx.y, tid = threadIdx.x;
+  if (cfg >= 27) {
+    gn_fold_group(p1.stats, p1.C, p1.T, p1.G, p1.count, p1.gamma, p1.beta, p1.fac, p1.gbias, p1.ld_fg, p1.eps, p1.A, p1.Bs,
+                  p1.chmean, b, cfg - 27);
+    return;
+  }
+  __shared__ double cs[256][2];
+  __shared__ double gs[GFT_G][2];
+  __shared__ float sc[256];
+  const int C = p0.C, T = p0.T, G = p0.G, cpg = C / G;
+  const float count = p0.count;
+  int cp2 = 1;
+  while (cp2 < cpg) cp2 <<= 1;
+  const int LPC = 256 / cp2, ch = tid / LPC, sub = tid % LPC;
+  double s1[GFT_G], s2[GFT_G];
+#pragma unroll
+  for (int g = 0; g < GFT_G; ++g) s1[g] = s2[g] = 0.0;
+  if (ch < cpg) {
+    const float2 *p = reinterpret_cast<const float2 *>(p0.stats + (((size_t)b * C + ch) * T) * 2);
+    const size_t gstride = (size_t)cpg * T;
+    for (int t = sub; t < T; t += LPC) {
+      float2 v[GFT_G];
+#pragma unroll
+      for (int g = 0; g < GFT_G; ++g) v[g] = g < G ? p[g * gstride + t] : make_float2(0.f, 0.f);
+#pragma unroll
+      for (int g = 0; g < GFT_G; ++g)
+        if (g < G) { s1[g] += (double)v[g].x; s2[g] += (double)v[g].y; }
+    }
+  }
+#pragma unroll
+  for (int g = 0; g < GFT_G; ++g) {
+    if (g < G) {
+      for (int m = 1; m < LPC; m <<= 1) { s1[g] += __shfl_xor(s1[g], m, 64); s2[g] += __shfl_xor(s2[g], m, 64); }
+      if (ch < cpg && sub == 0) {
+        cs[g * cpg + ch][0] = s1[g];
+        cs[g * cpg + ch][1] = s2[g];
+        if (cfg == 0) p0.chmean[(size_t)b * C + g * cpg + ch] = (float)(s1[g] / count);
+      }
+    }
+  }
+  __syncthreads();
+  if (tid < G) {
+    double g1 = 0.0, g2 = 0.0;
+    for (int c = 0; c < cpg; ++c) { g1 += cs[tid * cpg + c][0]; g2 += cs[tid * cpg + c][1]; }
+    gs[tid][0] = g1;
+    gs[tid][1] = g2;
+  }
+  __syncthreads();
+  if (tid < C) {
+    const int g = tid / cpg;
+    const double n = (double)count * cpg;
+    const double mean = gs[g][0] / n;
+    double var = gs[g][1] / n - mean * mean;
+    var = var > 0.0 ? var : 0.0;
+    const float rstd = (float)(1.0 / sqrt(var + (double)p0.eps));
+    const float f = p0.fac[(size_t)b * p0.ld_fg + tid], gb = p0.gbias[(size_t)b * p0.ld_fg + tid];
+    const float a0 = rstd * p0.gamma[tid];
+    const float a = a0 * f, bs = (p0.beta[tid] - (float)mean * a0) * f + gb;
+    if (cfg == 0) {
+      p0.A[(size_t)b * C + tid] = a;
+      p0.Bs[(size_t)b * C + tid] = bs;
+    }
+    sc[tid] = pro_act(bias1 ? bias1[tid] : 0.f, a, bs);
+  }
+  __syncthreads();
+  for (int co = tid; co < Cout; co += 256) {
+    double acc = bias2 ? (double)bias2[co] : 0.0;
+    const float *w = wsum + (size_t)cfg * C * Cout + co;
+    for (int c = 0; c < C; ++c) acc += (double)w[(size_t)c * Cout] * (double)sc[c];
+    tconst[((size_t)b * 27 + cfg) * Cout + co] = (float)acc;
+  }
+}
+
 __global__ void conv3d_pack_kernel(const float *__restrict__ w, int Cout, int Cin, int Cin_pad,
                                    float *__restrict__ wp) {
   const int i = blockIdx.x * blockDim.x + threadIdx.x;
@@ -631,4 +735,43 @@
   return 0;
 }
 
-}
+int lion_groupnorm_fold_pair(int B, const float *stats0, int C0, int T0, int G0, int voxels0, const float *gamma0,
+                             const float *beta0, const float *fac0, const float *gbias0, int ld_fg0, float eps0, float *A0,
+                             float *Bs0, float *chmean0, const float *stats1, int C1, int T1, int G1, int voxels1,
+                             const float *gamma1, const float *beta1, const float *fac1, const float *gbias1, int ld_fg1,
+                             float eps1, float *A1, float *Bs1, float *chmean1, lionStream_t stream) {
+  if (!stats0 || !gamma0 || !beta0 || !fac0 || !gbias0 || !A0 || !Bs0 || !chmean0) return LION_EINVAL;
+  if (!stats1 || !gamma1 || !beta1 || !fac1 || !gbias1 || !A1 || !Bs1 || !chmean1) return LION_EINVAL;
+  if (B <= 0 || C0 <= 0 || T0 <= 0 || G0 <= 0 || C0 % G0 != 0 || C0 / G0 > 64 || ld_fg0 < C0) return LION_EINVAL;
+  if (C1 <= 0 || T1 <= 0 || G1 <= 0 || C1 % G1 != 0 || C1 / G1 > 64 || ld_fg1 < C1) return LION_EINVAL;
+  const GnFoldProblem p0 = {stats0, gamma0, beta0, fac0, gbias0, A0, Bs0, chmean0, C0, T0, G0, ld_fg0, (float)voxels0, eps0};
+  const GnFoldProblem p1 = {stats1, gamma1, beta1, fac1, gbias1, A1, Bs1, chmean1, C1, T1, G1, ld_fg1, (float)voxels1, eps1};
+  gn_fold_pair_kernel<<<dim3(G0 + G1, B), 256, 0, static_cast<hipStream_t>(stream)>>>(p0, p1);
+  LION_LAUNCH_CHECK();
+  return 0;
+}
+
+int lion_groupnorm_fold_tconst(int B, const float *stats0, int C0, int T0, int G0, int voxels0, const float *gamma0,
+                               const float *beta0, const float *fac0, const float *gbias0, int ld_fg0, float eps0, float *A0,
+                               float *Bs0, float *chmean0, const float *stats1, int C1, int T1, int G1, int voxels1,
+                               const float *gamma1, const float *beta1, const float *fac1, const float *gbias1, int ld_fg1,
+                               float eps1, float *A1, float *Bs1, float *chmean1, const float *wsum, const float *bias2,
+                               const float *bias1, int Cout, float *tconst, lionStream_t stream) {
+  if (!stats0 || !gamma0 || !beta0 || !fac0 || !gbias0 || !A0 || !Bs0 || !chmean0 || !wsum || !tconst) return LION_EINVAL;
+  if (B <= 0 || C0 <= 0 || T0 <= 0 || G0 <= 0 || C0 % G0 != 0 || ld_fg0 < C0 || Cout <= 0) return LION_EINVAL;
+  if (stats1) {
+    if (!gamma1 || !beta1 || !fac1 || !gbias1 || !A1 || !Bs1 || !chmean1) return LION_EINVAL;
+    if (C1 <= 0 || T1 <= 0 || G1 <= 0 || C1 % G1 != 0 || C1 / G1 > 64 || ld_fg1 < C1) return LION_EINVAL;
+  } else {
+    G1 = 0;
+  }
+  if (C0 > 256 || G0 > GFT_G || C0 / G0 > 64 || C0 / G0 < 4) return LION_EUNSUPPORTED;
+  const GnFoldProblem p0 = {stats0, gamma0, beta0, fac0, gbias0, A0, Bs0, chmean0, C0, T0, G0, ld_fg0, (float)voxels0, eps0};
+  const GnFoldProblem p1 = {stats1, gamma1, beta1, fac1, gbias1, A1, Bs1, chmean1, C1, T1, G1, ld_fg1, (float)voxels1, eps1};
+  gn_fold_tconst_kernel<<<dim3(27 + G1, B), 256, 0, static_cast<hipStream_t>(stream)>>>(p0, p1, wsum, bias2, bias1, Cout,
+                                                                                      tconst);
+  LION_LAUNCH_CHECK();
+  return 0;
+}
+
+}
diff --git a/lion_amd/csrc/devoxelize.hip b/lion_amd/csrc/devoxelize.hip
--- a/lion_amd/csrc/devoxelize.hip
+++ b/lion_amd/csrc/devoxelize.hip
@@ -83,12 +83,13 @@
 }
 
 
-template <int LD, bool AFF>
+template <int LD, bool AFF, int RES = 0>
 __global__ __launch_bounds__(256) void devox_slab_kernel(
     const float *__restrict__ coords, const float *__restrict__ feat, int C, int N, int r, int PX,
     int XS, int CT, int CI, int slab_floats, int training, float *__restrict__ out,
     int32_t *__restrict__ inds, float *__restrict__ wgts, const float *__restrict__ scale,
-    const float *__restrict__ shift) {
+    const float *__restrict__ shift, const float *__restrict__ res = nullptr, const float *__restrict__ res_a = nullptr,
+    const float *__restrict__ res_b = nullptr) {
   extern __shared__ __attribute__((aligned(16))) unsigned char smem[];
   float *lds = reinterpret_cast<float *>(smem);
   constexpr int PP = 8;
@@ -217,6 +218,71 @@
     if (it + 1 < nit) issue(it + 1);
     const int base = xs * PX * r2;
     float *o = out + ((size_t)b * C + cg) * N;
+    if constexpr (RES != 0) {
+      constexpr int RES_P = RES == 1 ? 8 : 1, RES_C = RES == 1 ? 2 : 16;
+      const float *rs = res + ((size_t)b * C + cg) * N;
+#pragma unroll
+      for (int p0 = 0; p0 < PP; p0 += RES_P) {
+        float pv[RES_P][RES_C], av[RES_P][RES_C];
+#pragma unroll
+        for (int q = 0; q < RES_P; ++q) {
+          const int p = p0 + q;
+          const bool act = xsl[p] == xs || (xsl[p] == -2 && xs == 0);
+#pragma unroll
+          for (int ci = 0; ci < RES_C; ++ci) {
+            pv[q][ci] = 0.f;
+            if (act && ci < cin) pv[q][ci] = rs[(size_t)ci * N + pid[p]];
+          }
+        }
+#pragma unroll
+        for (int q = 0; q < RES_P; ++q) {
+          const int p = p0 + q;
+#pragma unroll
+          for (int ci = 0; ci < RES_C; ++ci) av[q][ci] = 0.f;
+          if (xsl[p] == xs) {
+            const float xd0 = sub_rn(1.0f, xd1[p]), yd0 = sub_rn(1.0f, yd1[p]), zd0 = sub_rn(1.0f, zd1[p]);
+            const int xo = (xd1[p] > 0.0f) ? r2 : 0, yo = (yd1[p] > 0.0f) ? r : 0, zo = (zd1[p] > 0.0f) ? 1 : 0;
+            const float w0 = mul_rn(mul_rn(xd0, yd0), zd0), w1 = mul_rn(mul_rn(xd0, yd0), zd1[p]);
+            const float w2 = mul_rn(mul_rn(xd0, yd1[p]), zd0), w3 = mul_rn(mul_rn(xd0, yd1[p]), zd1[p]);
+            const float w4 = mul_rn(mul_rn(xd1[p], yd0), zd0), w5 = mul_rn(mul_rn(xd1[p], yd0), zd1[p]);
+            const float w6 = mul_rn(mul_rn(xd1[p], yd1[p]), zd0), w7 = mul_rn(mul_rn(xd1[p], yd1[p]), zd1[p]);
+            float wsum = w0;
+            wsum += w1; wsum += w2; wsum += w3; wsum += w4; wsum += w5; wsum += w6; wsum += w7;
+            const float *f0 = buf + (ix0[p] - base);
+#pragma unroll
+            for (int ci = 0; ci < RES_C; ++ci) {
+              if (ci < cin) {
+                const float *fa = f0 + ci * r3, *f1 = fa + xo;
+                const float v0 = fa[0], v1 = fa[zo], v2 = fa[yo], v3 = fa[yo + zo];
+                const float v4 = f1[0], v5 = f1[zo], v6 = f1[yo], v7 = f1[yo + zo];
+                float a = mul_rn(w0, v0);
+                a = add_rn(a, mul_rn(w1, v1));
+                a = add_rn(a, mul_rn(w2, v2));
+                a = add_rn(a, mul_rn(w3, v3));
+                a = add_rn(a, mul_rn(w4, v4));
+                a = add_rn(a, mul_rn(w5, v5));
+                a = add_rn(a, mul_rn(w6, v6));
+                a = add_rn(a, mul_rn(w7, v7));
+                a = a * scale[(size_t)b * C + cg + ci] + shift[(size_t)b * C + cg + ci] * wsum;
+                av[q][ci] = a;
+              }
+            }
+          }
+        }
+#pragma unroll
+        for (int q = 0; q < RES_P; ++q) {
+          const int p = p0 + q;
+          if (xsl[p] == xs || (xsl[p] == -2 && xs == 0)) {
+#pragma unroll
+            for (int ci = 0; ci < RES_C; ++ci)
+              if (ci < cin)
+                o[(size_t)ci * N + pid[p]] = affine_swish_plus(pv[q][ci], res_a[(size_t)b * C + cg + ci],
+                                                               res_b[(size_t)b * C + cg + ci], av[q][ci]);
+          }
+        }
+      }
+      continue;
+    }
 #pragma unroll
     for (int p = 0; p < PP; ++p) {
       if (xsl[p] == xs) {
@@ -271,14 +337,17 @@
 
 template <int G> constexpr int devox_plan_stride() { return 16 + (DVR_NJ * DVR_NT / (G / 4)) * 2 + 2048 * 16 + 2048; }
 
-template <bool AFF, int G, int MODE>
+template <bool AFF, int G, int MODE, bool RES = false>
 __global__ __launch_bounds__(DVR_NT) void devox_ring_kernel(const float *__restrict__ coords,
                                                             const float *__restrict__ feat, int C, int N, int CT,
                                                             int training, float *__restrict__ out,
                                                             int32_t *__restrict__ inds, float *__restrict__ wgts,
                                                             const float *__restrict__ scale,
                                                             const float *__restrict__ shift, int dmax,
-                                                            unsigned char *__restrict__ plan) {
+                                                            unsigned char *__restrict__ plan,
+                                                            const float *__restrict__ res = nullptr,
+                                                            const float *__restrict__ res_a = nullptr,
+                                                            const float *__restrict__ res_b = nullptr) {
   extern __shared__ __attribute__((aligned(16))) unsigned char smem[];
   constexpr int PP = DVR_PP, r = DVR_R, r2 = r * r, r3 = r2 * r, NT = DVR_NT;
   constexpr int PPR = r / G, NP = r2 * PPR, nwords = NP / 32, LP = G / 4;
@@ -291,7 +360,7 @@
   unsigned *base = need + nwords;
   uint16_t *plist = reinterpret_cast<uint16_t *>(base + nwords);
   float *s_sc = reinterpret_cast<float *>(plist + NPMAX);
-  int *s_np = reinterpret_cast<int *>(s_sc + 32);
+  int *s_np = reinterpret_cast<int *>(s_sc + 64);
   const float *co = coords + (size_t)b * 3 * N;
   unsigned char *pl_b = (MODE != 0) ? plan + (size_t)b * devox_plan_stride<G>() : nullptr;
   const uint16_t *pl_list = reinterpret_cast<const uint16_t *>(pl_b + 16);
@@ -302,6 +371,10 @@
   if (AFF && tid < 2 * 16) {
     const int ci = tid & 15;
     s_sc[tid] = ci < nch ? (tid < 16 ? scale : shift)[(size_t)b * C + c0 + ci] : 0.f;
+  }
+  if (RES && tid >= 32 && tid < 64) {
+    const int ci = tid & 15;
+    s_sc[tid] = ci < nch ? (tid < 48 ? res_a : res_b)[(size_t)b * C + c0 + ci] : 0.f;
   }
   __syncthreads();
   int np = 0, nj = 0, buf_bytes = 0, D = 2;
@@ -314,8 +387,8 @@
   int mark[4] = {0, 0, 0, 0};
   auto ring_shape = [&]() {
     nj = (np * LP + NT - 1) / NT;
-    buf_bytes = nj * NT * 16;
-    D = nj == 0 ? 2 : min(min(dmax, 4), DVR_RING_BYTES / (nj ? buf_bytes : 1));
+    buf_bytes = (nj + (RES ? 1 : 0)) * NT * 16;
+    D = buf_bytes == 0 ? 2 : min(min(dmax, 4), DVR_RING_BYTES / (buf_bytes ? buf_bytes : 1));
     fits = nj <= DVR_NJ && D >= 2;
   };
   auto issue = [&](int ci) {
@@ -331,7 +404,14 @@
                      : "=&s"(keep) : "v"(gp), "s"(dst) : "memory");
       }
     }
-    ops += nj;
+    if (RES) {
+      const uint32_t dst = __builtin_amdgcn_readfirstlane(dst0 + nj * (NT * 16));
+      const float *gp = res + ((size_t)b * C + c0 + ci) * N + (tid * 4 < N ? tid * 4 : 0);
+      unsigned keep;
+      asm volatile("s_mov_b32 %0, m0\n\ts_mov_b32 m0, %2\n\ts_nop 0\n\tglobal_load_lds_dwordx4 %1, off nt\n\ts_mov_b32 m0, %0"
+                   : "=&s"(keep) : "v"(gp), "s"(dst) : "memory");
+    }
+    ops += nj + (RES ? 1 : 0);
     mark[ci % D] = ops;
   };
   if (MODE == 1) {
@@ -513,6 +593,24 @@
       }
     };
     if (wave_generic) gather(BoolT<true>{}); else gather(BoolT<false>{});
+    if (RES) {
+      const float ra = s_sc[32 + ci], rb = s_sc[48 + ci];
+      if (wave_generic) {
+        const float *rs = res + ((size_t)b * C + c0 + ci) * N;
+#pragma unroll
+        for (int p = 0; p < PP; ++p) {
+          const int i = tid + p * NT;
+          a4[p] = affine_swish_plus(i < N ? rs[i] : 0.f, ra, rb, a4[p]);
+        }
+      } else {
+        const uint32_t rbase = lbase + (uint32_t)(nj * (NT * 16));
+#pragma unroll
+        for (int p = 0; p < PP; ++p) {
+          const int i = tid + p * NT;
+          a4[p] = affine_swish_plus(*(lds_cfloat *)(uintptr_t)(rbase + (uint32_t)((i < N ? i : 0) * 4)), ra, rb, a4[p]);
+        }
+      }
+    }
 #pragma unroll
     for (int p = 0; p < PP; ++p) {
       const int i = tid + p * NT;
@@ -610,7 +708,7 @@
 
 constexpr int DVR_G = 8;
 constexpr size_t DVR_LDS = (size_t)DVR_RING_BYTES + (size_t)2 * (DVR_R * DVR_R * (DVR_R / DVR_G) / 32) * 4 +
-                           (size_t)(DVR_NJ * DVR_NT / (DVR_G / 4)) * 2 + 32 * 4 + 16;
+                           (size_t)(DVR_NJ * DVR_NT / (DVR_G / 4)) * 2 + 64 * 4 + 16;
 static int devox_ring_depth() {
   static const int d = getenv("LION_DEVOX_RING") ? atoi(getenv("LION_DEVOX_RING")) : 4;
   return d < 2 ? 2 : d;
@@ -620,14 +718,19 @@
 
 static int devox_launch(const float *coords, const float *feat, int B, int C, int N, int r,
                         int training, float *out, int32_t *inds, float *wgts, const float *scale,
-                        const float *shift, hipStream_t st) {
+                        const float *shift, hipStream_t st, const float *res = nullptr, const float *res_a = nullptr,
+                        const float *res_b = nullptr) {
   const int r2 = r * r;
   if (r == DVR_R && N <= 2048 && (((uintptr_t)feat) & 15) == 0) {
+    if (res && ((N & 3) != 0 || (((uintptr_t)res) & 15) != 0)) return LION_EUNSUPPORTED;
     int CT = 8;
     while (CT > 1 && (long)B * lion_cdiv(C, CT) < 256) CT >>= 1;
     dim3 grid(lion_cdiv(C, CT), B);
-    static LionLdsLimit cfgr0 = {}, cfgr1 = {};
-    if (scale) {
+    static LionLdsLimit cfgr0 = {}, cfgr1 = {}, cfgr2 = {};
+    if (res) {
+      if (int e = lion_dynamic_lds(&devox_ring_kernel<true, DVR_G, 0, true>, DVR_LDS, cfgr2)) return e;
+      devox_ring_kernel<true, DVR_G, 0, true><<<grid, DVR_NT, DVR_LDS, st>>>(coords, feat, C, N, CT, 0, out, inds, wgts, scale, shift, devox_ring_depth(), nullptr, res, res_a, res_b);
+    } else if (scale) {
       if (int e = lion_dynamic_lds(&devox_ring_kernel<true, DVR_G, 0>, DVR_LDS, cfgr1)) return e;
       devox_ring_kernel<true, DVR_G, 0><<<grid, DVR_NT, DVR_LDS, st>>>(coords, feat, C, N, CT, training, out, inds, wgts, scale, shift, devox_ring_depth(), nullptr);
     } else {
@@ -652,8 +755,16 @@
     dim3 grid(lion_cdiv(C, CT), B);
 #define DEVOX_SLAB(LD_)                                                                                    \
   {                                                                                                        \
-    static LionLdsLimit cfg0 = {}, cfg1 = {};                                                              \
-    if (scale) {                                                                                           \
+    static LionLdsLimit cfg0 = {}, cfg1 = {}, cfg2 = {}, cfg3 = {};                                        \
+    if (res && CI <= 2) {                                                                                  \
+      if (int e = lion_dynamic_lds(&devox_slab_kernel<LD_, true, 1>, lds, cfg2)) return e;                 \
+      devox_slab_kernel<LD_, true, 1><<<grid, 256, lds, st>>>(coords, feat, C, N, r, PX, XS, CT, CI, slab_floats, \
+                                                              0, out, inds, wgts, scale, shift, res, res_a, res_b); \
+    } else if (res) {                                                                                      \
+      if (int e = lion_dynamic_lds(&devox_slab_kernel<LD_, true, 2>, lds, cfg3)) return e;                 \
+      devox_slab_kernel<LD_, true, 2><<<grid, 256, lds, st>>>(coords, feat, C, N, r, PX, XS, CT, CI, slab_floats, \
+                                                              0, out, inds, wgts, scale, shift, res, res_a, res_b); \
+    } else if (scale) {                                                                                           \
       if (int e = lion_dynamic_lds(&devox_slab_kernel<LD_, true>, lds, cfg1)) return e;                    \
       devox_slab_kernel<LD_, true><<<grid, 256, lds, st>>>(coords, feat, C, N, r, PX, XS, CT, CI, slab_floats, \
                                                            training, out, inds, wgts, scale, shift);       \
@@ -671,6 +782,7 @@
     LION_LAUNCH_CHECK();
     return 0;
   }
+  if (res) return LION_EUNSUPPORTED;
   const int pt = lion_cdiv(N, 256);
   int ct = 16;
   while (ct > 2 && (long)B * pt * lion_cdiv(C, ct) < 2048) ct >>= 1;
@@ -704,6 +816,17 @@
   if (!coords || !feat || !out || !scale || !shift || B <= 0 || C <= 0 || N <= 0 || r <= 0) return LION_EINVAL;
   return devox_launch(coords, feat, B, C, N, r, 0, out, nullptr, nullptr, scale, shift,
                       static_cast<hipStream_t>(stream));
+}
+
+int lion_trilinear_devoxelize_affine_residual_forward(const float *coords, const float *feat, const float *scale,
+                                                      const float *shift, const float *res, const float *res_a,
+                                                      const float *res_b, int B, int C, int N, int r, float *out,
+                                                      lionStream_t stream) {
+  if (!coords || !feat || !out || !scale || !shift || !res || !res_a || !res_b || B <= 0 || C <= 0 || N <= 0 || r <= 0)
+    return LION_EINVAL;
+  if (out == res) return LION_EINVAL;
+  return devox_launch(coords, feat, B, C, N, r, 0, out, nullptr, nullptr, scale, shift, static_cast<hipStream_t>(stream),
+                      res, res_a, res_b);
 }
 
 size_t lion_devoxelize_plan_bytes(int B, int N, int r) {
@@ -751,6 +874,29 @@
   return 0;
 }
 
+int lion_trilinear_devoxelize_planned_residual_forward(const void *plan, size_t plan_bytes, const float *coords,
+                                                       const float *feat, const float *scale, const float *shift,
+                                                       const float *res, const float *res_a, const float *res_b, int B,
+                                                       int C, int N, int r, float *out, lionStream_t stream) {
+  if (!plan || !coords || !feat || !out || !scale || !shift || !res || !res_a || !res_b || B <= 0 || C <= 0 || N <= 0)
+    return LION_EINVAL;
+  if (out == res) return LION_EINVAL;
+  const size_t need = lion_devoxelize_plan_bytes(B, N, r);
+  if (!need || (((uintptr_t)plan) & 15) != 0 || (((uintptr_t)feat) & 15) != 0) return LION_EUNSUPPORTED;
+  if ((N & 3) != 0 || (((uintptr_t)res) & 15) != 0) return LION_EUNSUPPORTED;
+  if (plan_bytes < need) return LION_EWORKSPACE;
+  int CT = 8;
+  while (CT > 1 && (long)B * lion_cdiv(C, CT) < 256) CT >>= 1;
+  dim3 grid(lion_cdiv(C, CT), B);
+  unsigned char *pl = const_cast<unsigned char *>(static_cast<const unsigned char *>(plan));
+  static LionLdsLimit cfg = {};
+  if (int e = lion_dynamic_lds(&devox_ring_kernel<true, DVR_G, 1, true>, DVR_LDS, cfg)) return e;
+  devox_ring_kernel<true, DVR_G, 1, true><<<grid, DVR_NT, DVR_LDS, static_cast<hipStream_t>(stream)>>>(
+      coords, feat, C, N, CT, 0, out, nullptr, nullptr, scale, shift, devox_ring_depth(), pl, res, res_a, res_b);
+  LION_LAUNCH_CHECK();
+  return 0;
+}
+
 int lion_trilinear_devoxelize_backward(const float *gy, const int32_t *inds, const float *wgts,
                                        int B, int C, int N, int r3, float *gx,
                                        lionStream_t stream) {
diff --git a/lion_amd/csrc/pointwise.hip b/lion_amd/csrc/pointwise.hip
--- a/lion_amd/csrc/pointwise.hip
+++ b/lion_amd/csrc/pointwise.hip
@@ -59,10 +59,10 @@
   const int i = (blockIdx.x * 256 + threadIdx.x) * 4;
   if (i + 3 < L && (L & 3) == 0) {
     const float4 v = *reinterpret_cast<const float4 *>(p + i), w = *reinterpret_cast<const float4 *>(ad + i);
-    *reinterpret_cast<float4 *>(q + i) = make_float4(swishf(v.x * a + b) + w.x, swishf(v.y * a + b) + w.y,
-                                                     swishf(v.z * a + b) + w.z, swishf(v.w * a + b) + w.w);
-  } else {
-    for (int j = i; j < L && j < i + 4; ++j) q[j] = swishf(p[j] * a + b) + ad[j];
+    *reinterpret_cast<float4 *>(q + i) = make_float4(affine_swish_plus(v.x, a, b, w.x), affine_swish_plus(v.y, a, b, w.y),
+                                                     affine_swish_plus(v.z, a, b, w.z), affine_swish_plus(v.w, a, b, w.w));
+  } else {
+    for (int j = i; j < L && j < i + 4; ++j) q[j] = affine_swish_plus(p[j], a, b, ad[j]);
   }
 }
 
diff --git a/lion_amd/fused_ops.py b/lion_amd/fused_ops.py
--- a/lion_amd/fused_ops.py
+++ b/lion_amd/fused_ops.py
@@ -45,7 +45,7 @@
         return a, b_
 
 
-def conv3d_fused(x, conv, pro=None, want_stats=True, occ=None, prev_conv=None, split=None, fold=None):
+def conv3d_fused(x, conv, pro=None, want_stats=True, occ=None, prev_conv=None, split=None, fold=None, tconst=None):
     lib = _lib.load()
     b, cin, r = x.shape[0], x.shape[1], x.shape[2]
     cout = conv.out_channels
@@ -57,7 +57,8 @@
     x = x.contiguous()
     wp = conv_ops.split_packed_weight(conv.weight) if use_split else packed_weight(conv.weight)
     y = torch.empty((b, cout, r, r, r), device=x.device, dtype=torch.float32)
-    pa = pb = pbias = tconst = None
+    pa = pb = pbias = None
+    tconst_in, tconst = tconst, None
     if pro is not None:
         pa, pb = pro[0].contiguous(), pro[1].contiguous()
     bias = conv.bias.detach().contiguous() if conv.bias is not None else None
@@ -68,8 +69,10 @@
         else:
             ws = border_weight_sums(conv.weight)
             pbias = prev_conv.bias.detach().contiguous() if prev_conv.bias is not None else None
-            tconst = torch.empty((b, 27, cout), device=x.device, dtype=torch.float32)
-            _lib.call("lion_conv3d_const_response", ws, bias, pbias, pa, pb, b, cin, cout, tconst)
+            tconst = tconst_in
+            if tconst is None:
+                tconst = torch.empty((b, 27, cout), device=x.device, dtype=torch.float32)
+                _lib.call("lion_conv3d_const_response", ws, bias, pbias, pa, pb, b, cin, cout, tconst)
     stats = None
     if want_stats:
         tiles = lib.lion_conv3d_split_stat_tiles(r, cout) if use_split else lib.lion_conv3d_stat_tiles(r, cout, b, int(sparse))
@@ -95,6 +98,50 @@
     return A, Bs, cm
 
 
+def _fold_args(stats, gn, fac, gbias, voxels):
+    b, c, t, _ = stats.shape
+    A = torch.empty((b, c), device=stats.device, dtype=torch.float32)
+    Bs, cm = torch.empty_like(A), torch.empty_like(A)
+    if not (fac.stride(1) == 1 and gbias.stride(1) == 1 and fac.stride(0) == gbias.stride(0) and fac.stride(0) >= c):
+        fac, gbias = fac.contiguous(), gbias.contiguous()
+    return [stats, c, t, gn.num_groups, int(voxels), gn.weight, gn.bias, fac, gbias, int(fac.stride(0)), float(gn.eps),
+            A, Bs, cm], (A, Bs, cm)
+
+
+def groupnorm_fold_pair(stats0, gn0, fac0, gbias0, voxels0, stats1, gn1, fac1, gbias1, voxels1):
+    assert stats0.shape[0] == stats1.shape[0]
+    a0, out0 = _fold_args(stats0, gn0, fac0, gbias0, voxels0)
+    a1, out1 = _fold_args(stats1, gn1, fac1, gbias1, voxels1)
+    _lib.call("lion_groupnorm_fold_pair", stats0.shape[0], *a0, *a1)
+    return out0, out1
+
+
+FOLD_TCONST = os.environ.get("LION_FOLD_TCONST", "1")
+
+
+def delta_mode(conv, occ, r, prev_conv):
+    return occ is not None and r >= 16 and prev_conv is not None and conv.in_channels % 4 == 0 and conv.in_channels <= 256
+
+
+def groupnorm_fold_tconst(stats0, gn0, fac0, gbias0, voxels0, prev_conv, conv, point=None):
+    b, c = stats0.shape[:2]
+    cout = conv.out_channels
+    if c != conv.in_channels or c > 256 or gn0.num_groups > 8 or not 4 <= c // gn0.num_groups <= 64:
+        return None
+    a0, out0 = _fold_args(stats0, gn0, fac0, gbias0, voxels0)
+    if point is not None:
+        a1, out1 = _fold_args(*point)
+    else:
+        a1, out1 = [None, 0, 0, 0, 0, None, None, None, None, 0, 0.0, None, None, None], None
+    ws = border_weight_sums(conv.weight)
+    bias2 = conv.bias.detach().contiguous() if conv.bias is not None else None
+    bias1 = prev_conv.bias.detach().contiguous() if prev_conv.bias is not None else None
+    tconst = torch.empty((b, 27, cout), device=stats0.device, dtype=torch.float32)
+    if not _lib.call("lion_groupnorm_fold_tconst", b, *a0, *a1, ws, bias2, bias1, cout, tconst, unsupported_ok=True):
+        return None
+    return out0, tconst, out1
+
+
 def groupnorm_fold_se(stats, gn: torch.nn.GroupNorm, fac, gbias, voxels, se):
     b, c, t, _ = stats.shape
     w1, w2 = se.fc[0].weight.detach(), se.fc[2].weight.detach()
@@ -142,6 +189,26 @@
         return out
     _lib.call("lion_trilinear_devoxelize_affine_forward", co_c, gr_c, sc_c, sh_c, b, c, n, int(r), out)
     return out
+
+
+RING_RESIDUAL = os.environ.get("LION_DEVOX_RING_RESIDUAL", "1") != "0"
+
+
+def devoxelize_affine_residual(grid, coords, r, scale, shift, res, res_a, res_b, plan=None):
+    b, c = grid.shape[:2]
+    n = coords.shape[2]
+    if res.shape != (b, c, n) or res.dtype != torch.float32 or not res.is_contiguous() or (int(r) == 32 and not RING_RESIDUAL):
+        return None
+    out = torch.empty((b, c, n), device=grid.device, dtype=torch.float32)
+    co_c, gr_c = coords.contiguous(), grid.contiguous()
+    tail = (scale.contiguous(), shift.contiguous(), res, res_a.contiguous(), res_b.contiguous(), b, c, n, int(r), out)
+    if plan is not None and plan["shape"] == (b, n, int(r)) and plan["coords"].data_ptr() == co_c.data_ptr():
+        buf = plan["buf"]
+        ok = _lib.call("lion_trilinear_devoxelize_planned_residual_forward", buf, buf.numel(), co_c, gr_c, *tail,
+                       unsupported_ok=True)
+    else:
+        ok = _lib.call("lion_trilinear_devoxelize_affine_residual_forward", co_c, gr_c, *tail, unsupported_ok=True)
+    return out if ok else None
 
 
 def fusable(conv1, conv2, r, x):
diff --git a/lion_amd/models/pvcnn2_ada.py b/lion_amd/models/pvcnn2_ada.py
--- a/lion_amd/models/pvcnn2_ada.py
+++ b/lion_amd/models/pvcnn2_ada.py
@@ -13,6 +13,7 @@
 FUSE_INFERENCE = True
 SPARSE_CONV1 = True
 OVERLAP_POINT_BRANCH = os.environ.get("LION_OVERLAP_POINT_BRANCH", "0") != "0"
+SHORT_CHAIN = os.environ.get("LION_PVCONV_SHORT_CHAIN", "1") != "0"
 _POINT_STREAMS = {}
 
 
@@ -353,7 +354,14 @@
         conv2 = self.voxel_layers[4]
         return 2 if (SKIP_UNREAD_LEVEL2 and conv_ops.use_split(None, conv2.in_channels, conv2.out_channels, self.resolution)) else 1
 
-    def _fused_voxel_branch(self, grid, voxel_coords, style, counts=None):
+    def _short_chain_point_conv(self, features, style):
+        pf = self.point_features
+        if len(pf.layers) != 3 or not pf._fusable(features) or not fused_ops.pw_supported(pf.layers[0], features):
+            return None
+        y, st = fused_ops.pwconv_fused(features, pf.layers[0], None)
+        return y, st, pf.layers[1], pf.layers[1].affine(style)
+
+    def _fused_voxel_branch(self, grid, voxel_coords, style, counts=None, point=None):
         conv1, gn1, conv2, gn2 = self.voxel_layers[0], self.voxel_layers[1], self.voxel_layers[4], self.voxel_layers[5]
         se = self.voxel_layers[6] if len(self.voxel_layers) > 6 else None
         r = self.resolution
@@ -361,6 +369,28 @@
         if SPARSE_CONV1 and counts is not None and r >= 16:
             occ1, occ2 = _occupancy(counts, r, conv1.out_channels, grid.shape[0], self._aware_level())
         f1, g1 = gn1.affine(style)
+        if point is not None:
+            yp, stp, gnp, (fp, gp) = point
+            y1, st1 = fused_ops.conv3d_fused(grid, conv1, None, True, occ1)
+            merged = None
+            if (fused_ops.FOLD_TCONST == "1" or fused_ops.FOLD_TCONST == str(r)) and fused_ops.delta_mode(conv2, occ2, r, conv1):
+                merged = fused_ops.groupnorm_fold_tconst(st1, gn1.norm, f1, g1, r ** 3, conv1, conv2,
+                                                         point=(stp, gnp.norm, fp, gp, yp[0, 0].numel()))
+            if merged is not None:
+                (a1, b1, _), tconst, (ap, bp, _) = merged
+            else:
+                tconst = None
+                (a1, b1, _), (ap, bp, _) = fused_ops.groupnorm_fold_pair(st1, gn1.norm, f1, g1, r ** 3,
+                                                                         stp, gnp.norm, fp, gp, yp[0, 0].numel())
+            f2, g2 = gn2.affine(style)
+            y2, (a2, b2) = fused_ops.conv3d_fused(y1, conv2, (a1, b1), True, occ2, prev_conv=conv1, tconst=tconst,
+                                                  fold=fused_ops.FoldSpec(gn2.norm, f2, g2, r ** 3, se))
+            plan = _devox_plan(voxel_coords, r)
+            out = fused_ops.devoxelize_affine_residual(y2, voxel_coords, r, a2, b2, yp, ap, bp, plan=plan)
+            if out is None:
+                out = fused_ops.devoxelize_affine(y2, voxel_coords, r, a2, b2, plan=plan)
+                out = fused_ops.affine_swish(yp, ap, bp, add=out)
+            return out
         y1, (a1, b1) = fused_ops.conv3d_fused(grid, conv1, None, True, occ1,
                                               fold=fused_ops.FoldSpec(gn1.norm, f1, g1, r ** 3))
         f2, g2 = gn2.affine(style)
@@ -375,9 +405,12 @@
             f'get feat: {features.shape} and {coords.shape}'
         assert coords.shape[1] == 3, f'expect coords: B,3,Npoint, get: {coords.shape}'
         counts = None
+        point = None
         if (FUSE_INFERENCE and not self.training and not torch.is_grad_enabled() and features.is_cuda
                 and not torch.is_autocast_enabled()):
             will_fuse = fused_ops.fusable(self.voxel_layers[0], self.voxel_layers[4], self.resolution, features.float())
+            if will_fuse and SHORT_CHAIN and self.add_point_feat and not OVERLAP_POINT_BRANCH:
+                point = self._short_chain_point_conv(features, style)
             grid, voxel_coords, counts = self.voxelization(features, coords, return_counts=True,
                                                            sparse_reader=self._aware_level() if will_fuse else 0)
         else:
@@ -385,6 +418,11 @@
         if (FUSE_INFERENCE and not self.training and not torch.is_grad_enabled()
                 and fused_ops.fusable(self.voxel_layers[0], self.voxel_layers[4], self.resolution, grid)):
             pf = None
+            if point is not None:
+                fused = self._fused_voxel_branch(grid, voxel_coords, style, counts, point=point)
+                if self.attn is not None:
+                    fused = self.attn(fused)
+                return fused, coords_input, time_emb, style
             if self.add_point_feat and OVERLAP_POINT_BRANCH:
                 main, side = torch.cuda.current_stream(features.device), _point_stream(features.device)
                 side.wait_stream(main)
```

Result: no change. 5.361 (-0.3%).
